# Leonhard111/M3L

Hardware: AMD Instinct MI355X
Metric: MAE fwd+bwd samples/sec (image+tactile) (higher is better)
Workload: dtype bf16; 1 GPU; BASELINE configs[1]: VTT vision+tactile MAE, 64x64 RGB + 2x32x32 tactile, ViT-Tiny 192/12/3/768 + decoder 192/4/3/768, mask 0.75; batch_per_gpu=256, global_batch=256, parallelism=dp1, grad_allreduce=none (one rank), rccl_ranks=0, step=zero_grad + mask + fwd + bwd + grad all-reduce + Adam

## Files before the change

### include/m3l_amd.h

```cpp
#ifndef M3L_AMD_H
#define M3L_AMD_H
#include <stddef.h>
#include <stdint.h>

#ifdef __cplusplus
extern "C" {
#endif

#define M3L_MAX_TACTILES 8

typedef struct m3l_geom {
    int image_h, image_w, image_patch, image_channels;
    int tactile_h, tactile_w, tactile_patch, tactile_channels;
    int num_tactiles;
    int use_vision;
    int use_tactile;
} m3l_geom;

typedef struct m3l_tf_cfg {
    int dim, depth, heads, mlp_dim;
    int project_out;
    int dtype;
    int dim_head;
} m3l_tf_cfg;

typedef struct m3l_dropout {
    float p;
    uint64_t seed;
} m3l_dropout;

int m3l_version(void);
int m3l_last_error(char* buf, size_t n);
int m3l_set_rowln(int enable);
int m3l_set_attn_block(int mode);
int m3l_set_enc_mega(int mode);
void m3l_set_attn_phase_buffer(void* dev_buf);
int m3l_set_defer_join(int on);
int m3l_set_wgrad_inline(int on);
int m3l_side_join(void* stream);
int m3l_comm_available(void);
int m3l_comm_unique_id(void* out128);
int m3l_comm_init(const void* id128, int rank, int world);
int m3l_comm_world(void);
int m3l_comm_allreduce(float* buf, size_t count, void* after_stream);
int m3l_comm_destroy(void);
int m3l_side_fork(void* after_stream, void** side_out);
int m3l_side_mark_pending(void);
void* m3l_side_stream(void);
int m3l_side_pending(void);
int m3l_set_drop_h(int on);
int m3l_set_t192(int on);
int m3l_set_t192_tt(int tt);
int m3l_set_residual_bf16(int on);
int m3l_set_t192_stagger(int lead_mask, int prio_mask);

int m3l_mask_counts(const m3l_geom* g, double ratio, int* counts_host);
int m3l_mask_sample(const m3l_geom* g, double ratio, int B, const float* const* noise, int64_t* masked, int64_t* unmasked,
                    void* stream);

int m3l_mask_sample_counts(const m3l_geom* g, int nm_img, int nm_tac, int B, const float* const* noise, int64_t* masked,
                           int64_t* unmasked, void* stream);

size_t m3l_embed_ws_bytes(const m3l_geom* g, int D, int dtype, int B, int L);
int m3l_embed_fwd(const m3l_geom* g, int D, int dtype, int B, int L, int cnt_img, const int64_t* idx, const float* image,
                  const float* const* tactiles, const void* const* tensors, void* ws, float* tokens, void* stream);
int m3l_embed_bwd(const m3l_geom* g, int D, int dtype, int B, int L, int cnt_img, const int64_t* idx, const float* image,
                  const float* const* tactiles, const void* const* tensors, void* ws, const float* dtokens, float* const* grads,
                  void* stream);

size_t m3l_transformer_ws_bytes(const m3l_tf_cfg* c, int B, int n);
int m3l_transformer_fwd(const m3l_tf_cfg* c, int B, int n, const float* x_in, const void* const* tensors, void* ws, void* y_t,
                        float* y32, void* stream);
int m3l_transformer_bwd(const m3l_tf_cfg* c, int B, int n, const float* x_in, const void* const* tensors, void* ws, const void* dy,
                        int dy_dtype, float* dx_in, float* const* grads, void* stream);

int m3l_transformer_bwd_range(const m3l_tf_cfg* c, int B, int n, const float* x_in, const void* const* tensors, void* ws,
                              const void* dy, int dy_dtype, float* dx_in, float* const* grads, int layer_hi, int layer_lo, void* stream);

size_t m3l_transformer_ws_bytes_dropout(const m3l_tf_cfg* c, int B, int n, const m3l_dropout* drop);
int m3l_transformer_fwd_dropout(const m3l_tf_cfg* c, int B, int n, const float* x_in, const void* const* tensors, void* ws, void* y_t,
                                float* y32, const m3l_dropout* drop, void* stream);
int m3l_transformer_bwd_dropout(const m3l_tf_cfg* c, int B, int n, const float* x_in, const void* const* tensors, void* ws, const void* dy,
                                int dy_dtype, float* dx_in, float* const* grads, const m3l_dropout* drop, void* stream);
int m3l_transformer_bwd_range_dropout(const m3l_tf_cfg* c, int B, int n, const float* x_in, const void* const* tensors, void* ws,
                                      const void* dy, int dy_dtype, float* dx_in, float* const* grads, int layer_hi, int layer_lo,
                                      const m3l_dropout* drop, void* stream);

size_t m3l_frozen_vit_ws_bytes(const m3l_tf_cfg* c, int B, int n);
int m3l_frozen_vit_fwd(const m3l_tf_cfg* c, float ln_eps, int B, int n, const float* x, const void* const* tensors, void* ws,
                       float* y32, void* stream);

size_t m3l_unshuffle_ws_bytes(const m3l_geom* g, int D, int dd, int dtype, int B, int nvis, int nmask);
int m3l_unshuffle_fwd(const m3l_geom* g, int D, int dd, int dtype, int B, int nvis, int nmask, const int64_t* unmasked,
                      const int64_t* masked, const float* enc32, const void* enc_t, const void* const* tensors, void* ws,
                      float* dec_in, void* stream);
int m3l_unshuffle_bwd(const m3l_geom* g, int D, int dd, int dtype, int B, int nvis, int nmask, const int64_t* unmasked,
                      const int64_t* masked, const void* enc_t, const void* const* tensors, void* ws, const float* d_dec_in,
                      void* d_enc, int* d_enc_dtype, float* const* grads, void* stream);

size_t m3l_heads_ws_bytes(const m3l_geom* g, int dd, int dtype, int B, int nmask);
int m3l_heads_loss_fwd(const m3l_geom* g, int dd, int dtype, int B, int N, int nmask, int nm_img, const int64_t* masked,
                       const float* image, const float* const* tactiles, const void* dec_t, const void* const* tensors, void* ws,
                       float* loss, float* pred_img, float* tgt_img, float* pred_tac, float* tgt_tac, void* stream);
// ... 137 lines not shown
```

### m3l_amd/_lib.py

```python
import ctypes as C
import os

_HERE = os.path.dirname(os.path.abspath(__file__))
LIB_PATH = os.environ.get("M3L_LIB_PATH") or os.path.join(_HERE, "lib", "libm3l_amd.so")

c_p = C.c_void_p
c_i = C.c_int
c_sz = C.c_size_t


class Geom(C.Structure):
    _fields_ = [(n, c_i) for n in ("image_h", "image_w", "image_patch", "image_channels", "tactile_h", "tactile_w",
                                   "tactile_patch", "tactile_channels", "num_tactiles", "use_vision", "use_tactile")]


class CnnCfg(C.Structure):
    _fields_ = [(n, c_i) for n in ("in_channels", "height", "width", "dim", "tactile", "dtype")]


class TfCfg(C.Structure):
    _fields_ = [(n, c_i) for n in ("dim", "depth", "heads", "mlp_dim", "project_out", "dtype", "dim_head")]


class MaeCfg(C.Structure):
    _fields_ = [("geom", Geom), ("enc", TfCfg), ("dec", TfCfg), ("masking_ratio", C.c_double), ("early_conv", c_i), ("learned_pos", c_i)]


class Dropout(C.Structure):
    _fields_ = [("p", C.c_float), ("seed", C.c_uint64)]


class CommPlan(C.Structure):
    _fields_ = [("flat", c_p), ("total", C.c_long), ("min_bucket", C.c_long), ("layers_per_chunk", c_i), ("n_stages", c_i),
                ("stage_end", C.POINTER(C.c_long)), ("sent_out", C.POINTER(C.c_long))]


_SIGS = {
    "m3l_version": (c_i, []),
    "m3l_last_error": (c_i, [C.c_char_p, c_sz]),
    "m3l_set_rowln": (c_i, [c_i]),
    "m3l_set_attn_block": (c_i, [c_i]),
    "m3l_set_attn_phase_buffer": (None, [c_p]),
    "m3l_set_enc_mega": (c_i, [c_i]),
    "m3l_set_drop_h": (c_i, [c_i]),
    "m3l_set_direct_conv": (c_i, [c_i]),
    "m3l_set_t192": (c_i, [c_i]),
    "m3l_set_t192_tt": (c_i, [c_i]),
    "m3l_set_t192_stagger": (c_i, [c_i, c_i]),
    "m3l_set_residual_bf16": (c_i, [c_i]),
    "m3l_set_defer_join": (c_i, [c_i]),
    "m3l_set_wgrad_inline": (c_i, [c_i]),
    "m3l_side_join": (c_i, [c_p]),
    "m3l_side_stream": (c_p, []),
    "m3l_side_fork": (c_i, [c_p, C.POINTER(c_p)]),
    "m3l_side_mark_pending": (c_i, []),
    "m3l_comm_available": (c_i, []),
    "m3l_comm_unique_id": (c_i, [c_p]),
    "m3l_comm_init": (c_i, [c_p, c_i, c_i]),
    "m3l_comm_world": (c_i, []),
    "m3l_comm_allreduce": (c_i, [c_p, c_sz, c_p]),
    "m3l_comm_destroy": (c_i, []),
    "m3l_side_pending": (c_i, []),
    "m3l_mask_counts": (c_i, [C.POINTER(Geom), C.c_double, C.POINTER(c_i)]),
    "m3l_mask_sample": (c_i, [C.POINTER(Geom), C.c_double, c_i, c_p, c_p, c_p, c_p]),
    "m3l_mask_sample_counts": (c_i, [C.POINTER(Geom), c_i, c_i, c_i, c_p, c_p, c_p, c_p]),
    "m3l_embed_ws_bytes": (c_sz, [C.POINTER(Geom), c_i, c_i, c_i, c_i]),
    "m3l_embed_fwd": (c_i, [C.POINTER(Geom), c_i, c_i, c_i, c_i, c_i, c_p, c_p, c_p, c_p, c_p, c_p, c_p]),
    "m3l_embed_bwd": (c_i, [C.POINTER(Geom), c_i, c_i, c_i, c_i, c_i, c_p, c_p, c_p, c_p, c_p, c_p, c_p, c_p]),
    "m3l_transformer_ws_bytes": (c_sz, [C.POINTER(TfCfg), c_i, c_i]),
    "m3l_transformer_fwd": (c_i, [C.POINTER(TfCfg), c_i, c_i, c_p, c_p, c_p, c_p, c_p, c_p]),
    "m3l_transformer_bwd": (c_i, [C.POINTER(TfCfg), c_i, c_i, c_p, c_p, c_p, c_p, c_i, c_p, c_p, c_p]),
    "m3l_transformer_bwd_range": (c_i, [C.POINTER(TfCfg), c_i, c_i, c_p, c_p, c_p, c_p, c_i, c_p, c_p, c_i, c_i, c_p]),
    "m3l_transformer_ws_bytes_dropout": (c_sz, [C.POINTER(TfCfg), c_i, c_i, C.POINTER(Dropout)]),
    "m3l_transformer_fwd_dropout": (c_i, [C.POINTER(TfCfg), c_i, c_i, c_p, c_p, c_p, c_p, c_p, C.POINTER(Dropout), c_p]),
    "m3l_transformer_bwd_dropout": (c_i, [C.POINTER(TfCfg), c_i, c_i, c_p, c_p, c_p, c_p, c_i, c_p, c_p, C.POINTER(Dropout), c_p]),
    "m3l_transformer_bwd_range_dropout": (c_i, [C.POINTER(TfCfg), c_i, c_i, c_p, c_p, c_p, c_p, c_i, c_p, c_p, c_i, c_i, C.POINTER(Dropout), c_p]),
    "m3l_frozen_vit_ws_bytes": (c_sz, [C.POINTER(TfCfg), c_i, c_i]),
    "m3l_frozen_vit_fwd": (c_i, [C.POINTER(TfCfg), C.c_float, c_i, c_i, c_p, c_p, c_p, c_p, c_p]),
    "m3l_unshuffle_ws_bytes": (c_sz, [C.POINTER(Geom), c_i, c_i, c_i, c_i, c_i, c_i]),
    "m3l_unshuffle_fwd": (c_i, [C.POINTER(Geom), c_i, c_i, c_i, c_i, c_i, c_i, c_p, c_p, c_p, c_p, c_p, c_p, c_p, c_p]),
    "m3l_unshuffle_bwd": (c_i, [C.POINTER(Geom), c_i, c_i, c_i, c_i, c_i, c_i, c_p, c_p, c_p, c_p, c_p, c_p, c_p,
                                C.POINTER(c_i), c_p, c_p]),
    "m3l_heads_ws_bytes": (c_sz, [C.POINTER(Geom), c_i, c_i, c_i, c_i]),
    "m3l_heads_loss_fwd": (c_i, [C.POINTER(Geom), c_i, c_i, c_i, c_i, c_i, c_i, c_p, c_p, c_p, c_p, c_p, c_p, c_p, c_p, c_p,
                                 c_p, c_p, c_p]),
    "m3l_heads_loss_fwd2": (c_i, [C.POINTER(Geom), c_i, c_i, c_i, c_i, c_i, c_i, c_p, c_p, c_p, c_p, c_p, c_p, c_p, c_p, c_p,
                                  c_p, c_p, c_p, c_p]),
    "m3l_heads_loss_bwd": (c_i, [C.POINTER(Geom), c_i, c_i, c_i, c_i, c_i, c_i, c_p, c_p, c_p, c_p, c_p, c_p, c_p]),
    "m3l_mae_step_num_tensors": (c_i, [C.POINTER(MaeCfg)]),
    "m3l_mae_step_ws_bytes": (c_sz, [C.POINTER(MaeCfg), c_i]),
    "m3l_mae_step_fwd": (c_i, [C.POINTER(MaeCfg), c_i, c_p, c_p, c_p, c_p, c_p, c_p, c_p, c_p, c_p]),
    "m3l_mae_step_bwd": (c_i, [C.POINTER(MaeCfg), c_i, c_p, c_p, c_p, c_p, c_p, c_p, c_p, c_p, C.POINTER(CommPlan), c_p]),
    "m3l_mae_step_ws_bytes_dropout": (c_sz, [C.POINTER(MaeCfg), c_i, C.POINTER(Dropout)]),
    "m3l_mae_step_fwd_dropout": (c_i, [C.POINTER(MaeCfg), c_i, c_p, c_p, c_p, c_p, c_p, c_p, c_p, c_p, C.POINTER(Dropout), c_p]),
    "m3l_mae_step_bwd_dropout": (c_i, [C.POINTER(MaeCfg), c_i, c_p, c_p, c_p, c_p, c_p, c_p, c_p, c_p, C.POINTER(CommPlan), C.POINTER(Dropout), c_p]),
    "m3l_extractor_num_tensors": (c_i, [C.POINTER(MaeCfg), C.POINTER(TfCfg)]),
    "m3l_extractor_ws_bytes": (c_sz, [C.POINTER(MaeCfg), C.POINTER(TfCfg), c_i]),
# ... 104 lines not shown
```

### m3l_amd/csrc/elementwise.hip

```cpp
#include "common.cuh"
#include "kernels.h"
#include <cstring>
#include <vector>

namespace {

constexpr int MAXV = 16;
constexpr int WPB = 4;

__device__ __forceinline__ void store_val(float* p, float v) { *p = v; }
__device__ __forceinline__ void store_val(bf16* p, float v) { *p = (bf16)v; }


template <typename TO> __device__ __forceinline__ void store4(TO* p, f32x4 v);
template <> __device__ __forceinline__ void store4<float>(float* p, f32x4 v) { *reinterpret_cast<f32x4*>(p) = v; }
template <> __device__ __forceinline__ void store4<bf16>(bf16* p, f32x4 v) {
    bf16x4 o;
    o[0] = (bf16)v[0]; o[1] = (bf16)v[1]; o[2] = (bf16)v[2]; o[3] = (bf16)v[3];
    *reinterpret_cast<bf16x4*>(p) = o;
}
__device__ __forceinline__ f32x4 load4(const float* p) { return *reinterpret_cast<const f32x4*>(p); }
__device__ __forceinline__ f32x4 load4(const bf16* p) {
    const bf16x4 v = *reinterpret_cast<const bf16x4*>(p);
    return f32x4{(float)v[0], (float)v[1], (float)v[2], (float)v[3]};
// ... 127 lines not shown
    float s = 0.f;
    if (valid) {
        float a[8] = {0.f, 0.f, 0.f, 0.f, 0.f, 0.f, 0.f, 0.f};
        int g = sl;
        for (; g + 224 < G; g += 256) {
#pragma unroll
            for (int u = 0; u < 8; ++u) a[u] += p[(long)(g + 32 * u) * stride + j];
        }
        for (; g < G; g += 32) a[0] += p[(long)g * stride + j];
        s = ((a[0] + a[1]) + (a[2] + a[3])) + ((a[4] + a[5]) + (a[6] + a[7]));
    }
    red[sl][cl] = s;
    __syncthreads();
    if (sl == 0 && valid) {
        float t = red[0][cl];
#pragma unroll
        for (int i = 1; i < 32; ++i) t += red[i][cl];
        out[j] = accumulate ? out[j] + t : t;
    }
}

__global__ __launch_bounds__(1024) void reduce_rows_kernel(const float* __restrict__ part, int G, int stride, int count,
                                                             float* __restrict__ out, int accumulate) {
    const int j = blockIdx.x * 32 + (threadIdx.x & 31);
    reduce_cols_32x32(part, G, stride, j, j < count, out, accumulate);
}

__global__ __launch_bounds__(1024) void reduce_vec_kernel(const float* __restrict__ v, int G, float* __restrict__ out, int accumulate) {
    __shared__ float red[16];
    float a0 = 0.f, a1 = 0.f, a2 = 0.f, a3 = 0.f;
    int i = threadIdx.x;
    for (; i + 3072 < G; i += 4096) { a0 += v[i]; a1 += v[i + 1024]; a2 += v[i + 2048]; a3 += v[i + 3072]; }
    for (; i < G; i += 1024) a0 += v[i];
    float s = wave_sum((a0 + a1) + (a2 + a3));
    if ((threadIdx.x & 63) == 0) red[threadIdx.x >> 6] = s;
    __syncthreads();
    if (threadIdx.x == 0) {
        float t = 0.f;
#pragma unroll
        for (int w = 0; w < 16; ++w) t += red[w];
        out[0] = accumulate ? out[0] + t : t;
    }
}

struct ReduceSegs { float* out[4]; };
__global__ __launch_bounds__(1024) void reduce_rows_seg_kernel(const float* __restrict__ part, int G, int stride, int width,
                                                                 ReduceSegs segs, int accumulate) {
    float* out = segs.out[blockIdx.y];
    if (!out) return;
    const int j = blockIdx.x * 32 + (threadIdx.x & 31);
    reduce_cols_32x32(part + (long)blockIdx.y * width, G, stride, j, j < width, out, accumulate);
}

__global__ __launch_bounds__(1024) void reduce_rows_batch_kernel(ReduceBatch b, int accumulate) {
    const ReduceBatchItem it = b.it[blockIdx.z];
    float* out = it.out[blockIdx.y];
    if (!out) return;
    const int j = blockIdx.x * 32 + (threadIdx.x & 31);
    reduce_cols_32x32(it.part + (long)blockIdx.y * b.D, it.G, 3 * b.D, j, j < b.D, out, accumulate);
}

template <typename T> struct Vec4;
template <> struct Vec4<bf16> { typedef bf16x4 type; };
template <> struct Vec4<float> { typedef f32x4 type; };
template <typename T>
__global__ __launch_bounds__(256) void colsum_kernel(const T* __restrict__ Y, int M, int N, int ld, int rows_per_block,
                                                       float* __restrict__ part, int vec_ok) {
    typedef typename Vec4<T>::type V4;
    const int r0 = blockIdx.x * rows_per_block, r1 = min(M, r0 + rows_per_block);
    for (int c = threadIdx.x * 4; c < N; c += 1024) {
        if (vec_ok && c + 4 <= N) {
            f32x4 s0 = f32x4{0.f, 0.f, 0.f, 0.f}, s1 = s0, s2 = s0, s3 = s0;
            auto ld4 = [&](int r) {
                const V4 v = *reinterpret_cast<const V4*>(Y + (long)r * ld + c);
                return f32x4{to_f32(v[0]), to_f32(v[1]), to_f32(v[2]), to_f32(v[3])};
            };
            int r = r0;
            for (; r + 3 < r1; r += 4) {
                s0 += ld4(r);
                s1 += ld4(r + 1);
                s2 += ld4(r + 2);
                s3 += ld4(r + 3);
            }
            for (; r < r1; ++r) s0 += ld4(r);
            *reinterpret_cast<f32x4*>(part + (long)blockIdx.x * N + c) = (s0 + s1) + (s2 + s3);
        } else {
            for (int cc = c; cc < min(N, c + 4); ++cc) {
                float s0 = 0.f, s1 = 0.f, s2 = 0.f, s3 = 0.f;
                int r = r0;
                for (; r + 3 < r1; r += 4) {
                    s0 += to_f32(Y[(long)r * ld + cc]);
                    s1 += to_f32(Y[(long)(r + 1) * ld + cc]);
                    s2 += to_f32(Y[(long)(r + 2) * ld + cc]);
                    s3 += to_f32(Y[(long)(r + 3) * ld + cc]);
                }
                for (; r < r1; ++r) s0 += to_f32(Y[(long)r * ld + cc]);
                part[(long)blockIdx.x * N + cc] = (s0 + s1) + (s2 + s3);
            }
        }
    }
}

template <typename T>
__global__ __launch_bounds__(256) void prep_weights_kernel(WeightPack pack) {
    __shared__ float tile[64][65];
    int m = 0;
    while (m + 1 < pack.count && (int)blockIdx.x >= pack.tile0[m + 1]) ++m;
    const WeightDesc d = pack.d[m];
    const int tcols = (d.cols + 63) >> 6;
    const int t = blockIdx.x - pack.tile0[m];
    const int r0 = (t / tcols) << 6, c0 = (t % tcols) << 6;
    const int tid = threadIdx.x, q = tid & 15, p = tid >> 4;
    T* dst = reinterpret_cast<T*>(d.dst);
    T* dstT = reinterpret_cast<T*>(d.dstT);
    const bool vec_in = (d.cols & 3) == 0 && (reinterpret_cast<uintptr_t>(d.src) & 15) == 0;
#pragma unroll
    for (int k = 0; k < 4; ++k) {
        const int r = r0 + p + 16 * k, c = c0 + 4 * q;
        float v[4] = {0.f, 0.f, 0.f, 0.f};
        if (r < d.rows) {
            if (vec_in && c + 3 < d.cols) {
                const float4 f = *reinterpret_cast<const float4*>(d.src + (long)r * d.cols + c);
                v[0] = f.x; v[1] = f.y; v[2] = f.z; v[3] = f.w;
            } else {
#pragma unroll
                for (int j = 0; j < 4; ++j)
                    if (c + j < d.cols) v[j] = d.src[(long)r * d.cols + c + j];
            }
        }
        if (dst && r < d.ld_dstT) {
#pragma unroll
            for (int j = 0; j < 4; ++j)
                if (c + j < d.ld_dst) dst[(long)r * d.ld_dst + c + j] = from_f32<T>(v[j]);
        }
#pragma unroll
        for (int j = 0; j < 4; ++j) tile[p + 16 * k][4 * q + j] = v[j];
    }
    if (!dstT) return;
    __syncthreads();
#pragma unroll
    for (int k = 0; k < 4; ++k) {
        const int c = c0 + p + 16 * k, r = r0 + 4 * q;
        if (c >= d.ld_dst) continue;
#pragma unroll
        for (int j = 0; j < 4; ++j)
            if (r + j < d.ld_dstT) dstT[(long)c * d.ld_dstT + r + j] = from_f32<T>(tile[4 * q + j][p + 16 * k]);
    }
}

template <typename T>
__global__ void axpy_t_kernel(const float* __restrict__ x, const T* __restrict__ o, long count, float* __restrict__ out) {
    const long i = (long)blockIdx.x * blockDim.x + threadIdx.x;
    if (i < count) out[i] = x[i] + to_f32(o[i]);
}
template <typename T>
__global__ void cast_kernel(const float* __restrict__ x, long count, T* __restrict__ out) {
    const long i = (long)blockIdx.x * blockDim.x + threadIdx.x;
    if (i < count) out[i] = from_f32<T>(x[i]);
}

template <typename T>
__global__ void scale_by_dev_kernel(const T* __restrict__ x, long count, const float* __restrict__ s, T* __restrict__ out) {
    const long i = (long)blockIdx.x * blockDim.x + threadIdx.x;
    if (i < count) out[i] = from_f32<T>(to_f32(x[i]) * s[0]);
}

template <int MODE>
__global__ void mask_scale_kernel(const float* __restrict__ src, const void* __restrict__ ref, float scale, long count, float* __restrict__ out) {
    const long i = (long)blockIdx.x * blockDim.x + threadIdx.x;
    if (i >= count) return;
    const bool on = MODE == 0 ? reinterpret_cast<const uint8_t*>(ref)[i] != 0 : reinterpret_cast<const float*>(ref)[i] > 0.f;
    out[i] = on ? src[i] * scale : 0.f;
}
__global__ void vit_tokens_kernel(const float* __restrict__ emb, const float* __restrict__ cls, const float* __restrict__ regs,
                                  const float* __restrict__ pos, int B, int npatch, int R, int D, float* __restrict__ tok) {
    const long i = (long)blockIdx.x * blockDim.x + threadIdx.x;
    const int n = 1 + R + npatch;
    if (i >= (long)B * n * D) return;
    const int d = (int)(i % D), t = (int)((i / D) % n), b = (int)(i / ((long)D * n));
    float v;
    if (t == 0) v = cls[d] + pos[d];
    else if (t <= R) v = regs[(long)(t - 1) * D + d];
    else v = emb[((long)b * npatch + (t - 1 - R)) * D + d] + pos[(long)(t - R) * D + d];
    tok[i] = v;
}
__global__ void concat2_kernel(const float* __restrict__ a, int na, const float* __restrict__ b2, int nb, int rows, float* __restrict__ dst, int split) {
    const long i = (long)blockIdx.x * blockDim.x + threadIdx.x;
    const int w = na + nb;
    if (i >= (long)rows * w) return;
    const int r = (int)(i / w), c = (int)(i % w);
    if (!split) dst[i] = c < na ? a[(long)r * na + c] : b2[(long)r * nb + c - na];
    else if (c < na) const_cast<float*>(a)[(long)r * na + c] = dst[i];
    else if (b2) const_cast<float*>(b2)[(long)r * nb + c - na] = dst[i];
}

template <typename T>
__global__ void im2col_kernel(ConvSrc cs, int Bsrc, int Ci, int H, int W, int KH, int S, int P, int OH, int OW, int Kpad,
                              long total, T* __restrict__ col) {
    const long idx = (long)blockIdx.x * blockDim.x + threadIdx.x;
    if (idx >= total) return;
    const int k = (int)(idx % Kpad);
    const long r = idx / Kpad;
    const int ow = (int)(r % OW), oh = (int)((r / OW) % OH);
    const int b = (int)(r / ((long)OW * OH));
    float v = 0.f;
    if (k < Ci * KH * KH) {
        const int kw = k % KH, kh = (k / KH) % KH, ci = k / (KH * KH);
        const int ih = oh * S + kh - P, iw = ow * S + kw - P;
        if (ih >= 0 && ih < H && iw >= 0 && iw < W) {
            if (cs.nchw) {
                const float* src = reinterpret_cast<const float*>(cs.src[b / Bsrc]);
                v = src[(((long)(b % Bsrc) * Ci + ci) * H + ih) * W + iw];
            } else {
                v = to_f32(reinterpret_cast<const T*>(cs.src[0])[(((long)b * H + ih) * W + iw) * Ci + ci]);
            }
        }
    }
// ... 245 lines not shown
    ph = pidx / gw;
    pw = pidx % gw;
}
__device__ __forceinline__ const float* patch_base(const PatchGroup& pg, int b, int s, int ph, int pw) {
    const float* src = pg.src[0];
#pragma unroll
    for (int i = 1; i < M3L_MAX_SENSORS; ++i) src = (s == i) ? pg.src[i] : src;
    return src + ((long)b * pg.C * pg.H + ph * pg.P) * pg.W + pw * pg.P;
}
struct PatchDiv {
    unsigned m_pp, m_p;
    int pp;
};
__device__ __forceinline__ PatchDiv patch_div(const PatchGroup& pg) {
    PatchDiv d;
    d.pp = pg.P * pg.P;
    d.m_pp = 0xFFFFFFFFu / (unsigned)d.pp + 1u;
    d.m_p = 0xFFFFFFFFu / (unsigned)pg.P + 1u;
    return d;
}
__device__ __forceinline__ int patch_off_t(const PatchGroup& pg, const PatchDiv& dv, int t, int& e) {
    const int c = (int)__umulhi((unsigned)t, dv.m_pp);
    const int rem = t - c * dv.pp;
    const int p1 = (int)__umulhi((unsigned)rem, dv.m_p);
    const int p2 = rem - p1 * pg.P;
    e = rem * pg.C + c;
    return (c * pg.H + p1) * pg.W + p2;
}
template <int NV>
__device__ __forceinline__ void patch_stage_stats(const PatchGroup& pg, const PatchDiv& dv, const float* __restrict__ base, int lane, int pd,
                                                  float eps, float* __restrict__ my, float& mean, float& rstd) {
    float v[NV];
    int ei[NV];
#pragma unroll
    for (int i = 0; i < NV; ++i) v[i] = base[patch_off_t(pg, dv, min(lane + 64 * i, pd - 1), ei[i])];
    float sum = 0.f;
#pragma unroll
    for (int i = 0; i < NV; ++i) {
        if (lane + 64 * i < pd) my[ei[i]] = v[i];
        else v[i] = 0.f;
        sum += v[i];
    }
    mean = wave_sum(sum) / pd;
    float q = 0.f;
#pragma unroll
    for (int i = 0; i < NV; ++i) {
        const float d = (lane + 64 * i < pd) ? v[i] - mean : 0.f;
        q += d * d;
    }
    rstd = rsqrtf(wave_sum(q) / pd + eps);
}

template <typename T, int NV>
__global__ __launch_bounds__(256) void patch_ln_kernel(PatchGroup pg, const int64_t* __restrict__ idx, int idx_ld, int j0, int cnt,
                                                         int rows, const float* __restrict__ gamma, const float* __restrict__ beta,
                                                         float eps, T* __restrict__ xn, int pdpad, int vec) {
    __shared__ __attribute__((aligned(16))) float buf[WPB][NV * 64];
    const int lane = threadIdx.x & 63, wave = threadIdx.x >> 6, row = blockIdx.x * WPB + wave;
    const int pd = pg.C * pg.P * pg.P;
    const PatchDiv dv = patch_div(pg);
    float* my = buf[wave];
    const bool live = row < rows;
    float mean = 0.f, rstd = 0.f;
    if (live) {
        int b, s, ph, pw, local;
        patch_locate(pg, idx, idx_ld, j0, cnt, row, b, s, ph, pw, local);
        patch_stage_stats<NV>(pg, dv, patch_base(pg, b, s, ph, pw), lane, pd, eps, my, mean, rstd);
    }
    __syncthreads();
    if (!live) return;
    T* out = xn + (long)row * pdpad;
    if (vec) {
        constexpr int NC = NV / 4;
        f32x4 gm[NC], bt[NC];
#pragma unroll
        for (int k = 0; k < NC; ++k) {
            const int ec = min(4 * (lane + 64 * k), pd - 4);
            gm[k] = load4(gamma + ec);
            bt[k] = load4(beta + ec);
        }
#pragma unroll
        for (int k = 0; k < NC; ++k) {
            const int e = 4 * (lane + 64 * k);
            if (e < pdpad) {
                f32x4 r = {0.f, 0.f, 0.f, 0.f};
                if (e < pd) r = (*reinterpret_cast<const f32x4*>(my + e) - mean) * rstd * gm[k] + bt[k];
                store4<T>(out + e, r);
            }
        }
    } else {
        for (int e = lane; e < pdpad; e += 64) out[e] = from_f32<T>(e < pd ? (my[e] - mean) * rstd * gamma[e] + beta[e] : 0.f);
    }
}

template <typename T, int NV>
__global__ __launch_bounds__(256) void patch_ln_bwd_kernel(PatchGroup pg, const int64_t* __restrict__ idx, int idx_ld, int j0, int cnt,
                                                             int rows, float eps, const T* __restrict__ dxn, int pdpad,
                                                             float* __restrict__ part, int vec) {
    __shared__ __attribute__((aligned(16))) float buf[WPB][NV * 64];
    constexpr int NC = NV / 4;
    static_assert(NV % 4 == 0, "4-element pieces");
    const int lane = threadIdx.x & 63, wave = threadIdx.x >> 6;
    const int pd = pg.C * pg.P * pg.P;
    const PatchDiv dv = patch_div(pg);
    float* my = buf[wave];
    f32x4 dg[NC], db[NC];
#pragma unroll
    for (int k = 0; k < NC; ++k) dg[k] = db[k] = f32x4{0.f, 0.f, 0.f, 0.f};
    for (int r0 = blockIdx.x * WPB; r0 < rows; r0 += gridDim.x * WPB) {
        const int row = r0 + wave;
        const bool live = row < rows;
        float mean = 0.f, rstd = 0.f;
        if (live) {
            int b, s, ph, pw, local;
            patch_locate(pg, idx, idx_ld, j0, cnt, row, b, s, ph, pw, local);
            patch_stage_stats<NV>(pg, dv, patch_base(pg, b, s, ph, pw), lane, pd, eps, my, mean, rstd);
        }
        __syncthreads();
        if (live) {
            const T* dr = dxn + (long)row * pdpad;
            f32x4 d[NC];
#pragma unroll
            for (int k = 0; k < NC; ++k) {
                const int e = 4 * (lane + 64 * k);
                if (vec) {
                    d[k] = load4(dr + min(e, pd - 4));
                } else {
#pragma unroll
                    for (int q = 0; q < 4; ++q) d[k][q] = to_f32(dr[min(e + q, pd - 1)]);
                }
            }
#pragma unroll
            for (int k = 0; k < NC; ++k) {
                const int e = 4 * (lane + 64 * k);
                f32x4 a = {0.f, 0.f, 0.f, 0.f};
                if (vec) {
                    if (e < pd) a = *reinterpret_cast<const f32x4*>(my + e);
                    else d[k] = f32x4{0.f, 0.f, 0.f, 0.f};
                } else {
#pragma unroll
                    for (int q = 0; q < 4; ++q) {
                        if (e + q < pd) a[q] = my[e + q];
                        else d[k][q] = 0.f;
                    }
                }
                dg[k] += d[k] * (a - mean) * rstd;
                db[k] += d[k];
            }
        }
        __syncthreads();
    }
    float* out = part + (long)blockIdx.x * 2 * pd;
#pragma unroll
    for (int pass = 0; pass < 2; ++pass) {
#pragma unroll
        for (int k = 0; k < NC; ++k) *reinterpret_cast<f32x4*>(my + 4 * (lane + 64 * k)) = pass ? db[k] : dg[k];
        __syncthreads();
        for (int e = threadIdx.x; e < pd; e += 256) out[pass * pd + e] = buf[0][e] + buf[1][e] + buf[2][e] + buf[3][e];
        __syncthreads();
    }
}

__global__ __launch_bounds__(256) void embed_finalize_kernel(const float* __restrict__ E, int rows, int D, PatchGroup pg,
                                                               const int64_t* __restrict__ idx, int idx_ld, int j0, int cnt,
                                                               const float* __restrict__ gamma, const float* __restrict__ beta,
                                                               float eps, const float* __restrict__ mod, int mod0,
                                                               const float* __restrict__ pos, float* __restrict__ tokens, int L) {
    const int lane = threadIdx.x & 63, row = blockIdx.x * WPB + (threadIdx.x >> 6);
    if (row >= rows) return;
    int b, s, ph, pw, local;
    patch_locate(pg, idx, idx_ld, j0, cnt, row, b, s, ph, pw, local);
    const float* xr = E + (long)row * D;
    float v[MAXV];
    float sum = 0.f;
#pragma unroll
    for (int i = 0; i < MAXV; ++i) {
        const int e = lane + 64 * i;
        v[i] = (e < D) ? xr[e] : 0.f;
        sum += v[i];
    }
    const float mean = wave_sum(sum) / D;
    float q = 0.f;
#pragma unroll
    for (int i = 0; i < MAXV; ++i) {
        const int e = lane + 64 * i;
        const float d = (e < D) ? v[i] - mean : 0.f;
        q += d * d;
    }
    const float rstd = rsqrtf(wave_sum(q) / D + eps);
    const int jj = row % cnt;
    float* out = tokens + ((long)b * L + j0 + jj) * D;
    const float* mrow = mod + (long)(mod0 + s) * D;
    const float* prow = pos + (long)local * D;
#pragma unroll
    for (int i = 0; i < MAXV; ++i) {
        const int e = lane + 64 * i;
        if (e < D) out[e] = (v[i] - mean) * rstd * gamma[e] + beta[e] + mrow[e] + prow[e];
    }
}

template <typename T>
__global__ __launch_bounds__(256) void embed_finalize_bwd_kernel(const float* __restrict__ dtok, int L, const float* __restrict__ E,
                                                                   int rows, int D, PatchGroup pg, const int64_t* __restrict__ idx,
                                                                   int idx_ld, int j0, int cnt, const float* __restrict__ gamma,
                                                                   float eps, T* __restrict__ dE, float* __restrict__ part, int nslot) {
    extern __shared__ float sm[];
    const int lane = threadIdx.x & 63, wave = threadIdx.x >> 6;
    const int PL = (2 + nslot) * D;
    for (int i = threadIdx.x; i < WPB * PL; i += 256) sm[i] = 0.f;
    __syncthreads();
    float* my = sm + wave * PL;
    for (int row = blockIdx.x * WPB + wave; row < rows; row += gridDim.x * WPB) {
        int b, s, ph, pw, local;
        patch_locate(pg, idx, idx_ld, j0, cnt, row, b, s, ph, pw, local);
        const int jj = row % cnt;
        const float* xr = E + (long)row * D;
        const float* dyr = dtok + ((long)b * L + j0 + jj) * D;
        float v[MAXV], gdy[MAXV];
        float sum = 0.f;
#pragma unroll
        for (int i = 0; i < MAXV; ++i) {
            const int e = lane + 64 * i;
            v[i] = (e < D) ? xr[e] : 0.f;
            sum += v[i];
        }
        const float mean = wave_sum(sum) / D;
        float q = 0.f;
#pragma unroll
        for (int i = 0; i < MAXV; ++i) {
            const int e = lane + 64 * i;
            const float d = (e < D) ? v[i] - mean : 0.f;
            q += d * d;
        }
        const float rstd = rsqrtf(wave_sum(q) / D + eps);
        float s1 = 0.f, s2 = 0.f;
#pragma unroll
        for (int i = 0; i < MAXV; ++i) {
            const int e = lane + 64 * i;
            if (e < D) {
                const float xh = (v[i] - mean) * rstd;
                const float d = dyr[e];
                my[e] += d * xh;
                my[D + e] += d;
                my[(2 + s) * D + e] += d;
                const float gd = d * gamma[e];
                gdy[i] = gd;
                v[i] = xh;
                s1 += gd;
                s2 += gd * xh;
            } else {
                gdy[i] = 0.f;
                v[i] = 0.f;
            }
        }
        s1 = wave_sum(s1) / D;
        s2 = wave_sum(s2) / D;
#pragma unroll
        for (int i = 0; i < MAXV; ++i) {
            const int e = lane + 64 * i;
            if (e < D) dE[(long)row * D + e] = from_f32<T>(rstd * (gdy[i] - s1 - v[i] * s2));
        }
    }
    __syncthreads();
    for (int i = threadIdx.x; i < PL; i += 256)
        part[(long)blockIdx.x * PL + i] = sm[i] + sm[PL + i] + sm[2 * PL + i] + sm[3 * PL + i];
}

template <typename TO>
__global__ __launch_bounds__(256) void unshuffle_fwd_kernel(const float* __restrict__ src, const float* __restrict__ mask_token,
                                                              const int64_t* __restrict__ unmasked, int nvis,
                                                              const int64_t* __restrict__ masked, int nmask, int B, int dd,
                                                              int n_img, int n_tac, const float* __restrict__ dmod,
                                                              const float* __restrict__ pos_img, const float* __restrict__ pos_tac,
                                                              TO* __restrict__ dec_in) {
    const int lane = threadIdx.x & 63;
    const long r = (long)blockIdx.x * WPB + (threadIdx.x >> 6);
    const int N = nvis + nmask;
    if (r >= (long)B * N) return;
    const int b = (int)(r / N), j = (int)(r % N);
    const bool vis = j < nvis;
    const int pos = (int)(vis ? unmasked[(long)b * nvis + j] : masked[(long)b * nmask + j - nvis]);
    const float* s = vis ? src + ((long)b * nvis + j) * dd : mask_token;
    const int m = pos < n_img ? 0 : 1 + (pos - n_img) / n_tac;
    const float* prow = pos < n_img ? pos_img + (long)pos * dd : pos_tac + (long)(pos - n_img) * dd;
    TO* out = dec_in + ((long)b * N + pos) * dd;
    const float* mrow = dmod + (long)m * dd;
    for (int e = 4 * lane; e < dd; e += 256) store4<TO>(out + e, load4(s + e) + load4(mrow + e) + load4(prow + e));
}

template <int MAXC, typename TI>
__global__ __launch_bounds__(256) void unshuffle_bwd_kernel(const TI* __restrict__ dY, const int64_t* __restrict__ unmasked, int nvis,
                                                              int B, int N, int dd, int n_img, int n_tac, int nmod, int rows_per_wave,
                                                              int vis_per_wave, float* __restrict__ dsrc, float* __restrict__ part) {
    extern __shared__ float sm[];
    const int lane = threadIdx.x & 63, wave = threadIdx.x >> 6;
    const int PL = (1 + nmod) * dd;
    for (int i = threadIdx.x; i < WPB * PL; i += 256) sm[i] = 0.f;
    __syncthreads();
    float* my = sm + wave * PL;
    const long gw = (long)blockIdx.x * WPB + wave;
    f32x4 acc[MAXC];
#pragma unroll
    for (int c = 0; c < MAXC; ++c) acc[c] = f32x4{0.f, 0.f, 0.f, 0.f};
#define UNSH_FLUSH(slot, sign)                                                      \
    _Pragma("unroll") for (int c = 0; c < MAXC; ++c) {                              \
        const int e4 = (lane + 64 * c) * 4;                                         \
        if (e4 < dd) {                                                              \
            _Pragma("unroll") for (int q = 0; q < 4; ++q) {                         \
                my[e4 + q] += (sign) * acc[c][q];                                   \
                if ((slot) >= 0) my[(1 + (slot)) * dd + e4 + q] += acc[c][q];       \
            }                                                                       \
        }                                                                           \
        acc[c] = f32x4{0.f, 0.f, 0.f, 0.f};                                         \
    }
    const long total = (long)B * N;
    const long r0 = gw * rows_per_wave, r1 = r0 + rows_per_wave < total ? r0 + rows_per_wave : total;
    for (long r = r0; r < r1;) {
        const int pos = (int)(r % N);
// ... 76 lines not shown
    const T* s = src + ((long)b * N + pos) * D;
    T* d = dst + (long)row * D;
    for (int e = lane; e < D; e += 64) d[e] = s[e];
}
template <typename T>
__global__ __launch_bounds__(256) void scatter_rows_kernel(const T* __restrict__ src, int N, int D, const int64_t* __restrict__ idx,
                                                             int idx_ld, int j0, int cnt, int rows, T* __restrict__ dst) {
    const int lane = threadIdx.x & 63, row = blockIdx.x * WPB + (threadIdx.x >> 6);
    if (row >= rows) return;
    const int b = row / cnt, jj = row % cnt;
    const long pos = idx[(long)b * idx_ld + j0 + jj];
    const T* s = src + (long)row * D;
    T* d = dst + ((long)b * N + pos) * D;
    for (int e = lane; e < D; e += 64) d[e] = s[e];
}

template <typename T>
__global__ __launch_bounds__(256) void gather_rows2_kernel(const T* __restrict__ src, int N, int D, const int64_t* __restrict__ idx, int idx_ld,
                                                             int cnt0, int cnt1, int rows, T* __restrict__ dst0, T* __restrict__ dst1) {
    const int lane = threadIdx.x & 63, row = blockIdx.x * WPB + (threadIdx.x >> 6);
    if (row >= rows) return;
    const int b = row / (cnt0 + cnt1), j = row % (cnt0 + cnt1);
    const long pos = idx[(long)b * idx_ld + j];
    const uint4* s = reinterpret_cast<const uint4*>(src + ((long)b * N + pos) * D);
    uint4* d = reinterpret_cast<uint4*>(j < cnt0 ? dst0 + ((long)b * cnt0 + j) * D : dst1 + ((long)b * cnt1 + (j - cnt0)) * D);
    const int pieces = D * (int)sizeof(T) / 16;
    for (int p = lane; p < pieces; p += 64) d[p] = s[p];
}
template <typename T>
__global__ __launch_bounds__(256) void scatter_rows2_kernel(const T* __restrict__ src0, const T* __restrict__ src1, int N, int D,
                                                              const int64_t* __restrict__ idx, int idx_ld, int cnt0, int cnt1, int rows,
                                                              const float* __restrict__ scale, T* __restrict__ dst) {
    const int lane = threadIdx.x & 63, row = blockIdx.x * WPB + (threadIdx.x >> 6);
    if (row >= rows) return;
    const int b = row / (cnt0 + cnt1), j = row % (cnt0 + cnt1);
    const long pos = idx[(long)b * idx_ld + j];
    const T* s = j < cnt0 ? src0 + ((long)b * cnt0 + j) * D : src1 + ((long)b * cnt1 + (j - cnt0)) * D;
    T* d = dst + ((long)b * N + pos) * D;
    const float sc = scale ? *scale : 1.f;
    constexpr int E = 16 / (int)sizeof(T);
    const int pieces = D / E;
    for (int p = lane; p < pieces; p += 64) {
        uint4 v = reinterpret_cast<const uint4*>(s)[p];
        if (scale) {
            T* e = reinterpret_cast<T*>(&v);
#pragma unroll
            for (int k = 0; k < E; ++k) e[k] = from_f32<T>(to_f32(e[k]) * sc);
        }
        reinterpret_cast<uint4*>(d)[p] = v;
    }
}

template <typename T>
__global__ __launch_bounds__(256) void mse_kernel(const float* __restrict__ pred, int pdpad, PatchGroup pg,
                                                    const int64_t* __restrict__ idx, int idx_ld, int j0, int cnt, int rows, float w,
                                                    float* __restrict__ part, T* __restrict__ dpred, float* __restrict__ target_out, int vec) {
    extern __shared__ __attribute__((aligned(16))) float mbuf[];
    __shared__ float red[WPB];
    const int lane = threadIdx.x & 63, wave = threadIdx.x >> 6;
    const int pd = pg.C * pg.P * pg.P;
    const PatchDiv dv = patch_div(pg);
    float* my = mbuf + (long)wave * pdpad;
    float acc = 0.f;
    for (int r0 = blockIdx.x * WPB; r0 < rows; r0 += gridDim.x * WPB) {
        const int row = r0 + wave;
        const bool live = row < rows;
        if (live) {
            int b, s, ph, pw, local;
            patch_locate(pg, idx, idx_ld, j0, cnt, row, b, s, ph, pw, local);
            const float* base = patch_base(pg, b, s, ph, pw);
            for (int tb = 0; tb < pd; tb += 512) {
                const int t0 = tb + lane;
                float tv[8];
                int e[8];
#pragma unroll
                for (int u = 0; u < 8; ++u) {
                    if (tb + 64 * u >= pd) break;
                    const int t = t0 + 64 * u;
                    tv[u] = base[patch_off_t(pg, dv, min(t, pd - 1), e[u])];
                }
#pragma unroll
                for (int u = 0; u < 8; ++u) {
                    if (tb + 64 * u >= pd) break;
                    if (t0 + 64 * u < pd) my[e[u]] = tv[u];
                }
            }
        }
        __syncthreads();
        if (live) {
            const float* pr = pred + (long)row * pdpad;
            T* dp = dpred + (long)row * pdpad;
            if (vec) {
#pragma unroll 4
                for (int e = 4 * lane; e < pdpad; e += 256) {
                    f32x4 d = {0.f, 0.f, 0.f, 0.f};
                    if (e < pd) {
                        const f32x4 t = *reinterpret_cast<const f32x4*>(my + e);
                        d = load4(pr + e) - t;
                        if (target_out) store4<float>(target_out + (long)row * pd + e, t);
                    }
                    acc += d[0] * d[0];
                    acc += d[1] * d[1];
                    acc += d[2] * d[2];
                    acc += d[3] * d[3];
                    store4<T>(dp + e, d * (2.f * w));
                }
            } else {
                for (int e = lane; e < pdpad; e += 64) {
                    const float d = e < pd ? pr[e] - my[e] : 0.f;
                    if (e < pd && target_out) target_out[(long)row * pd + e] = my[e];
                    acc += d * d;
                    dp[e] = from_f32<T>(2.f * w * d);
                }
            }
        }
        __syncthreads();
    }
    acc = wave_sum(acc);
    if (lane == 0) red[wave] = acc;
    __syncthreads();
    if (threadIdx.x == 0) part[blockIdx.x] = w * (red[0] + red[1] + red[2] + red[3]);
}

}

static int ln_grid(int M) { return cdiv(M, WPB); }
static bool aligned_to(const void* p, size_t a) { return ((uintptr_t)p & (a - 1)) == 0; }
int m3l_part_blocks(void) {
    static const int nb = [] {
        const char* e = getenv("M3L_PART_BLOCKS");
        const int v = e ? atoi(e) : 1024;
        return v < 64 ? 64 : (v > M3L_MAX_PARTIAL_BLOCKS ? M3L_MAX_PARTIAL_BLOCKS : v);
    }();
    return nb;
}
static int part_grid(long rows) {
    long g = (rows + WPB - 1) / WPB;
    if (g > m3l_part_blocks()) g = m3l_part_blocks();
    return (int)(g < 1 ? 1 : g);
}

int m3l_ln_fwd(int out_dtype, const float* x, int M, int D, const float* gamma, const float* beta, float eps, void* y, float* y32,
               hipStream_t st) {
    M3L_CHECK(M > 0 && D > 0 && D % 4 == 0 && D <= 1024, "ln_fwd: bad shape M=%d D=%d (D must be a multiple of 4, <= 1024)", M, D);
    ProfScope prof("ln_fwd", M, D, out_dtype, (double)M * D * (4.0 + (y ? (out_dtype ? 2 : 4) : 0) + (y32 ? 4 : 0)), st);
#define LN_FWD(TO, C, TX) ln_fwd_kernel<TO, C, TX><<<ln_grid(M), 256, 0, st>>>((const TX*)x, M, D, gamma, beta, eps, (TO*)y, y32)
    if (m3l_call_rb()) {
        if (out_dtype == 1) { if (D <= 256) LN_FWD(bf16, 1, bf16); else if (D <= 512) LN_FWD(bf16, 2, bf16); else LN_FWD(bf16, 4, bf16); }
        else { if (D <= 256) LN_FWD(float, 1, bf16); else if (D <= 512) LN_FWD(float, 2, bf16); else LN_FWD(float, 4, bf16); }
    } else if (out_dtype == 1) {
        if (D <= 256) LN_FWD(bf16, 1, float); else if (D <= 512) LN_FWD(bf16, 2, float); else LN_FWD(bf16, 4, float);
    } else {
        if (D <= 256) LN_FWD(float, 1, float); else if (D <= 512) LN_FWD(float, 2, float); else LN_FWD(float, 4, float);
    }
#undef LN_FWD
    M3L_LAUNCH_CHECK();
    return 0;
}

int m3l_reduce_rows(const float* part, int G, int stride, int count, float* out, int accumulate, hipStream_t st) {
    if (count == 1 && stride == 1)
        reduce_vec_kernel<<<1, 1024, 0, st>>>(part, G, out, accumulate);
    else
        reduce_rows_kernel<<<cdiv(count, 32), 1024, 0, st>>>(part, G, stride, count, out, accumulate);
    M3L_LAUNCH_CHECK();
    return 0;
}

int m3l_ln_bwd_blocks(int M) {
    static const int forced = getenv("M3L_LN_ROWS_PER_WAVE") ? atoi(getenv("M3L_LN_ROWS_PER_WAVE")) : 0;
    const int rpw = forced > 0 ? forced : (M >= 12288 ? 4 : std::max(1, M / 4096));
    int G = cdiv(M, rpw * WPB);
    if (G > 2048) G = 2048;
    return G < 1 ? 1 : G;
}

int m3l_ln_bwd(int dy_dtype, const void* dy, const float* x, int M, int D, const float* gamma, float eps, const float* dres,
               float* dx_out, void* dx_t_out, int ct_dtype, float* part_ws, float* dgamma, float* dbeta, float* dbias,
               int accumulate, hipStream_t st) {
    M3L_CHECK(M > 0 && D > 0 && D % 4 == 0 && D <= 1024, "ln_bwd: bad shape M=%d D=%d (D must be a multiple of 4, <= 1024)", M, D);
    const int G = m3l_ln_bwd_blocks(M);
    {
        ProfScope prof("ln_bwd", M, D, dy_dtype,
                       (double)M * D * ((m3l_call_rb() ? 2.0 : 4.0) + (dy_dtype ? 2 : 4) + (dres ? (m3l_call_rb() ? 2 : 4) : 0) + (dx_out ? 4 : 0) + (dx_t_out ? (ct_dtype ? 2 : 4) : 0)), st);
#define LN_BWD(TD, TC, C, TX) ln_bwd_kernel<TD, TC, C, TX><<<G, 256, 0, st>>>((const TD*)dy, (const TX*)x, M, D, gamma, eps, dres, dx_out, (TC*)dx_t_out, part_ws)
#define LN_BWD_C(TD, TC, TX) { if (D <= 256) LN_BWD(TD, TC, 1, TX); else if (D <= 512) LN_BWD(TD, TC, 2, TX); else LN_BWD(TD, TC, 4, TX); }
        if (m3l_call_rb()) {
            M3L_CHECK(!dx_out && dx_t_out && ct_dtype == 1, "ln_bwd: bf16 residual mode writes the compute-type gradient only");
            if (dy_dtype == 1) LN_BWD_C(bf16, bf16, bf16) else LN_BWD_C(float, bf16, bf16)
        }
        else if (dy_dtype == 1) LN_BWD_C(bf16, bf16, float)
        else if (ct_dtype == 1) LN_BWD_C(float, bf16, float)
        else LN_BWD_C(float, float, float)
#undef LN_BWD_C
#undef LN_BWD
    }
    M3L_LAUNCH_CHECK();
    if (!dgamma && !dbeta && !dbias) return 0;
    ReduceSegs segs = {{dgamma, dbeta, dbias, nullptr}};
    reduce_rows_seg_kernel<<<dim3(cdiv(D, 32), 3), 1024, 0, st>>>(part_ws, G, 3 * D, D, segs, accumulate);
    M3L_LAUNCH_CHECK();
    return 0;
}

int m3l_reduce_rows_batch(const ReduceBatch* b, int accumulate, hipStream_t st) {
    if (b->count <= 0) return 0;
    M3L_CHECK(b->count <= M3L_REDUCE_BATCH_MAX && b->D > 0, "reduce_rows_batch: count=%d D=%d", b->count, b->D);
    ProfScope prof("reduce_batch", b->count, b->D, 0, 0.0, st);
    reduce_rows_batch_kernel<<<dim3(cdiv(b->D, 32), 3, b->count), 1024, 0, st>>>(*b, accumulate);
    M3L_LAUNCH_CHECK();
    return 0;
}

int m3l_reduce_rows_seg3(const float* part, int G, int D, float* out0, float* out1, float* out2, int accumulate, hipStream_t st) {
    ReduceSegs segs = {{out0, out1, out2, nullptr}};
    reduce_rows_seg_kernel<<<dim3(cdiv(D, 32), 3), 1024, 0, st>>>(part, G, 3 * D, D, segs, accumulate);
    M3L_LAUNCH_CHECK();
    return 0;
}

int m3l_colsum(int dtype, const void* Y, int M, int N, int ld, float* part_ws, float* out, int accumulate, hipStream_t st) {
    M3L_CHECK(M > 0 && N > 0, "colsum: bad shape");
    int G = cdiv(M, N > 512 ? 16 : 64);
    if (G > m3l_part_blocks()) G = m3l_part_blocks();
    const int rpb = cdiv(M, G);
    G = cdiv(M, rpb);
    ProfScope prof("colsum", M, N, dtype, (double)M * N * (dtype ? 2 : 4), st);
    const int vec_ok = (ld % 4 == 0) && (N % 4 == 0) && (((unsigned long)Y) % 16 == 0) && (((unsigned long)part_ws) % 16 == 0);
    if (dtype == 1)
        colsum_kernel<bf16><<<G, 256, 0, st>>>((const bf16*)Y, M, N, ld, rpb, part_ws, vec_ok);
    else
        colsum_kernel<float><<<G, 256, 0, st>>>((const float*)Y, M, N, ld, rpb, part_ws, vec_ok);
    M3L_LAUNCH_CHECK();
    return m3l_reduce_rows(part_ws, G, N, N, out, accumulate, st);
}

static thread_local int g_prep_mode = 0;
static thread_local int g_prep_dtype = -1;
static thread_local std::vector<WeightDesc>* g_prep_list = nullptr;
int m3l_prep_mode(void) { return g_prep_mode; }
void m3l_prep_set_mode(int mode) {
    g_prep_mode = mode;
    if (mode == 1) {
        if (!g_prep_list) g_prep_list = new std::vector<WeightDesc>();
        g_prep_list->clear();
        g_prep_dtype = -1;
    }
}
int m3l_prep_flush(hipStream_t st) {
    const int saved = g_prep_mode;
    g_prep_mode = 0;
    int rc = 0;
    if (g_prep_list && !g_prep_list->empty()) {
        for (size_t i = 0; i < g_prep_list->size() && !rc; i += M3L_WPACK) {
            WeightPack pk;
            memset(&pk, 0, sizeof(pk));
            for (size_t k = i; k < g_prep_list->size() && k < i + M3L_WPACK; ++k) pk.d[pk.count++] = (*g_prep_list)[k];
            rc = m3l_prep_weights(g_prep_dtype, &pk, st);
        }
        g_prep_list->clear();
    }
    g_prep_mode = saved;
    return rc;
}

int m3l_prep_weights(int dtype, const WeightPack* pack_in, hipStream_t st) {
    if (pack_in->count <= 0) return 0;
    M3L_CHECK(pack_in->count <= M3L_WPACK, "prep_weights: %d matrices in one pack (max %d)", pack_in->count, M3L_WPACK);
    if (g_prep_mode == 2) return 0;
    if (g_prep_mode == 1) {
        M3L_CHECK(g_prep_dtype < 0 || g_prep_dtype == dtype, "prep_weights: modules of one chain disagree on the compute type");
        g_prep_dtype = dtype;
        for (int i = 0; i < pack_in->count; ++i) g_prep_list->push_back(pack_in->d[i]);
        return 0;
    }
    WeightPack pack = *pack_in;
    int tiles = 0;
    for (int i = 0; i < pack.count; ++i) {
        const WeightDesc& d = pack.d[i];
        M3L_CHECK(d.ld_dst >= d.cols && d.ld_dstT >= d.rows && d.ld_dst <= ((d.cols + 63) / 64) * 64 && d.ld_dstT <= ((d.rows + 63) / 64) * 64,
                  "prep_weights: padding of matrix %d ([%d, %d] -> [%d, %d]) must stay inside its last 64 x 64 tiles", i, d.rows, d.cols, d.ld_dstT, d.ld_dst);
        pack.tile0[i] = tiles;
        tiles += ((d.rows + 63) / 64) * ((d.cols + 63) / 64);
    }
    pack.tile0[pack.count] = tiles;
    if (tiles == 0) return 0;
    ProfScope prof("prep_weights", pack.count, dtype, 0, 0.0, st);
// ... 40 lines not shown
int m3l_cast_f32(int dtype, const float* x, long count, void* out, hipStream_t st) {
    ProfScope prof("cast", count, dtype, 0, (double)count * (4.0 + (dtype ? 2 : 4)), st);
    if (dtype == 1 && count % 8 == 0 && ((uintptr_t)x & 15) == 0 && ((uintptr_t)out & 15) == 0)
        cast8_f32_bf16_kernel<<<cdiv(count / 8, 256), 256, 0, st>>>(x, count / 8, (bf16*)out);
    else if (dtype == 1)
        cast_kernel<bf16><<<cdiv(count, 256), 256, 0, st>>>(x, count, (bf16*)out);
    else
        cast_kernel<float><<<cdiv(count, 256), 256, 0, st>>>(x, count, (float*)out);
    M3L_LAUNCH_CHECK();
    return 0;
}

int m3l_im2col(int dtype, const ConvSrc* src, int Bsrc, int Ci, int H, int W, int KH, int S, int P, int OH, int OW, int Kpad, void* col,
               hipStream_t st) {
    const int Btot = src->nchw ? Bsrc * src->nsrc : Bsrc;
    const long total = (long)Btot * OH * OW * Kpad;
    if (dtype == 1 && KH == 4 && Kpad == Ci * 16) {
        const long pairs = (long)Btot * OH * OW * Ci;
        im2col4_bf16_kernel<<<cdiv(pairs, 256), 256, 0, st>>>(*src, Bsrc, Ci, H, W, S, P, OH, OW, pairs, (bf16*)col);
        M3L_LAUNCH_CHECK();
        return 0;
    }
    if (dtype == 1)
        im2col_kernel<bf16><<<cdiv(total, 256), 256, 0, st>>>(*src, Bsrc, Ci, H, W, KH, S, P, OH, OW, Kpad, total, (bf16*)col);
    else
        im2col_kernel<float><<<cdiv(total, 256), 256, 0, st>>>(*src, Bsrc, Ci, H, W, KH, S, P, OH, OW, Kpad, total, (float*)col);
    M3L_LAUNCH_CHECK();
    return 0;
}

int m3l_col2im_relu(int dtype, const void* dcol, int Btot, int Ci, int H, int W, int KH, int S, int P, int OH, int OW, int Kpad,
                    const void* act, void* dX, hipStream_t st) {
    const long total = (long)Btot * H * W * Ci;
    if (dtype == 1)
        col2im_relu_kernel<bf16><<<cdiv(total, 256), 256, 0, st>>>((const bf16*)dcol, Btot, Ci, H, W, KH, S, P, OH, OW, Kpad, (const bf16*)act, (bf16*)dX);
    else
        col2im_relu_kernel<float><<<cdiv(total, 256), 256, 0, st>>>((const float*)dcol, Btot, Ci, H, W, KH, S, P, OH, OW, Kpad, (const float*)act, (float*)dX);
    M3L_LAUNCH_CHECK();
    return 0;
}

int k_tokens_assemble(const float* img_tok, const float* tac_tok, int B, int D, int n_img, int n_tac, int k, const float* mod,
                        const float* pos_img, const float* pos_tac, float* tokens, hipStream_t st) {
    const long rows = (long)B * (n_img + k * n_tac);
    tokens_assemble_kernel<<<cdiv(rows, WPB), 256, 0, st>>>(img_tok, tac_tok, B, D, n_img, n_tac > 0 ? n_tac : 1, k, mod, pos_img, pos_tac, tokens);
    M3L_LAUNCH_CHECK();
    return 0;
}

int k_tokens_assemble_bwd(const float* dtok, int B, int D, int n_img, int n_tac, int k, float* d_img, float* d_tac, float* part_ws,
                            float* dmod, int accumulate, hipStream_t st) {
    const long rows = (long)B * (n_img + k * n_tac);
    const int PL = (1 + k) * D;
    const int G = part_grid(rows);
    tokens_assemble_bwd_kernel<<<G, 256, WPB * PL * sizeof(float), st>>>(dtok, B, D, n_img, n_tac > 0 ? n_tac : 1, k, d_img, d_tac, part_ws);
    M3L_LAUNCH_CHECK();
    reduce_rows_kernel<<<cdiv(PL, 32), 1024, 0, st>>>(part_ws, G, PL, PL, dmod, accumulate);
    M3L_LAUNCH_CHECK();
    return 0;
}

int m3l_adam_flat(float* p, const float* g, float* m, float* v, long n, float lr, float b1, float b2, float eps, float wd, int step,
                  float gscale, hipStream_t st) {
    M3L_CHECK(n > 0 && step >= 1, "adam: n=%ld step=%d", n, step);
    const float bc1 = 1.0f - powf(b1, (float)step);
    const float bc2_sqrt = sqrtf(1.0f - powf(b2, (float)step));
    adam_flat_kernel<0><<<cdiv(cdiv(n, 4), 256), 256, 0, st>>>(p, const_cast<float*>(g), m, v, n, lr, b1, b2, eps, wd, bc1, bc2_sqrt, nullptr, gscale, nullptr, 0);
    M3L_LAUNCH_CHECK();
    return 0;
}

int m3l_adamw_flat(float* p, float* g, float* m, float* v, long n, float lr, float b1, float b2, float eps, float wd, int step, float gscale,
                   float max_norm, float* norm_ws, int scale_grads, hipStream_t st) {
    M3L_CHECK(n > 0 && step >= 1, "adamw: n=%ld step=%d", n, step);
    M3L_CHECK(max_norm <= 0.f || norm_ws, "adamw: clipping needs the norm workspace");
    const float bc1 = 1.0f - powf(b1, (float)step);
    const float bc2_sqrt = sqrtf(1.0f - powf(b2, (float)step));
    const float* clip = nullptr;
    if (max_norm > 0.f) {
        const int G = (int)std::min<long>(1024, cdiv(cdiv(n, 4), 256));
        gradnorm_part_kernel<<<G, 256, 0, st>>>(g, n, norm_ws);
        M3L_LAUNCH_CHECK();
        gradnorm_final_kernel<<<1, 64, 0, st>>>(norm_ws, G, gscale, max_norm, norm_ws + 1024);
        M3L_LAUNCH_CHECK();
        clip = norm_ws + 1024;
    }
    const float decay = (float)(1.0 - (double)lr * (double)wd);
    adam_flat_kernel<1><<<cdiv(cdiv(n, 4), 256), 256, 0, st>>>(p, g, m, v, n, lr, b1, b2, eps, decay, bc1, bc2_sqrt, nullptr, gscale, clip,
                                                              scale_grads && (clip || gscale != 1.0f));
    M3L_LAUNCH_CHECK();
    return 0;
}

int m3l_adam_flat_dev(float* p, const float* g, float* m, float* v, long n, float lr, float b1, float b2, float eps, float wd,
                      int* step_dev, float* bc_dev, hipStream_t st) {
    M3L_CHECK(n > 0 && step_dev && bc_dev, "adam (device step): n=%ld", n);
    adam_bias_kernel<<<1, 1, 0, st>>>(step_dev, b1, b2, bc_dev);
    M3L_LAUNCH_CHECK();
    adam_flat_kernel<0><<<cdiv(cdiv(n, 4), 256), 256, 0, st>>>(p, const_cast<float*>(g), m, v, n, lr, b1, b2, eps, wd, 1.0f, 1.0f, bc_dev, 1.0f, nullptr, 0);
    M3L_LAUNCH_CHECK();
    return 0;
}

int m3l_scale_by_dev(int dtype, const void* x, long count, const float* scale_dev, void* out, hipStream_t st) {
    if (dtype == 1)
        scale_by_dev_kernel<bf16><<<cdiv(count, 256), 256, 0, st>>>((const bf16*)x, count, scale_dev, (bf16*)out);
    else
        scale_by_dev_kernel<float><<<cdiv(count, 256), 256, 0, st>>>((const float*)x, count, scale_dev, (float*)out);
    M3L_LAUNCH_CHECK();
    return 0;
}

int m3l_mask_scale(int mode, const float* src, const void* ref, float scale, long count, float* out, hipStream_t st) {
    M3L_CHECK((mode == 0 || mode == 1) && count > 0 && src && ref && out, "mask_scale: bad arguments");
    if (mode == 0) mask_scale_kernel<0><<<cdiv(count, 256), 256, 0, st>>>(src, ref, scale, count, out);
    else mask_scale_kernel<1><<<cdiv(count, 256), 256, 0, st>>>(src, ref, scale, count, out);
    M3L_LAUNCH_CHECK();
    return 0;
}
int m3l_vit_tokens(const float* emb, const float* cls, const float* regs, const float* pos, int B, int npatch, int R, int D, float* tok,
                   hipStream_t st) {
    M3L_CHECK(B > 0 && npatch > 0 && R >= 0 && D > 0 && emb && cls && pos && tok && (R == 0 || regs), "vit_tokens: bad arguments");
    vit_tokens_kernel<<<cdiv((long)B * (1 + R + npatch) * D, 256), 256, 0, st>>>(emb, cls, regs, pos, B, npatch, R, D, tok);
    M3L_LAUNCH_CHECK();
    return 0;
}
int m3l_concat2(float* a, int na, float* b2, int nb, int rows, float* cat, int split, hipStream_t st) {
    M3L_CHECK(rows > 0 && na > 0 && nb > 0 && a && cat && (split || b2), "concat2: bad arguments");
    concat2_kernel<<<cdiv((long)rows * (na + nb), 256), 256, 0, st>>>(a, na, b2, nb, rows, cat, split);
    M3L_LAUNCH_CHECK();
    return 0;
}

int m3l_vt_load_launch(const void* image_nhwc, int image_u8, int B, int H, int W, int C, float img_lo, float img_span, float* image_nchw,
                       const void* tactile, int tactile_u8, int th, int tw, int n_sensors, int frame_stack, float tac_lo, float tac_span,
                       float* const* tactile_out, hipStream_t st) {
    if (image_nhwc) {
        M3L_CHECK(img_span != 0.f, "vt_load: empty image normalisation range");
        const long total = (long)B * C * H * W;
        if (image_u8)
            vt_image_kernel<uint8_t><<<cdiv(total, 256), 256, 0, st>>>((const uint8_t*)image_nhwc, B, H, W, C, img_lo, img_span, image_nchw);
        else
            vt_image_kernel<float><<<cdiv(total, 256), 256, 0, st>>>((const float*)image_nhwc, B, H, W, C, img_lo, img_span, image_nchw);
        M3L_LAUNCH_CHECK();
    }
    if (tactile) {
        M3L_CHECK(n_sensors >= 1 && n_sensors <= M3L_MAX_SENSORS, "vt_load: n_sensors=%d", n_sensors);
        M3L_CHECK(tac_span != 0.f, "vt_load: empty tactile normalisation range");
        VtTactileOut o;
        for (int s = 0; s < n_sensors; ++s) o.p[s] = tactile_out[s];
        const long total = (long)B * 3 * n_sensors * frame_stack * th * tw;
        if (tactile_u8)
            vt_tactile_kernel<uint8_t><<<cdiv(total, 256), 256, 0, st>>>((const uint8_t*)tactile, B, th, tw, n_sensors, frame_stack, tac_lo,
                                                                         tac_span, o);
        else
            vt_tactile_kernel<float><<<cdiv(total, 256), 256, 0, st>>>((const float*)tactile, B, th, tw, n_sensors, frame_stack, tac_lo,
                                                                       tac_span, o);
        M3L_LAUNCH_CHECK();
    }
    return 0;
}

int m3l_mask_rank_groups(const MaskRankArgs* args, int B, int64_t* masked, int masked_ld, int64_t* unmasked, int unmasked_ld, hipStream_t st) {
    M3L_CHECK(B > 0 && args->count >= 1 && args->count <= M3L_MAX_SENSORS + 1, "mask_rank: B=%d groups=%d", B, args->count);
    int nmax = 0;
    for (int i = 0; i < args->count; ++i) {
        const MaskRankGroup& g = args->g[i];
        M3L_CHECK(g.n > 0 && g.nm >= 0 && g.nm <= g.n, "mask_rank: bad shape n=%d nm=%d", g.n, g.nm);
        M3L_CHECK(g.n <= 8192, "mask_rank: n=%d too large", g.n);
        nmax = std::max(nmax, g.n);
    }
    const int threads = nmax <= 64 ? 64 : (nmax <= 128 ? 128 : 256);
    mask_rank_kernel<<<dim3(B, args->count), threads, nmax * sizeof(float), st>>>(*args, masked, masked_ld, unmasked, unmasked_ld);
    M3L_LAUNCH_CHECK();
    return 0;
}
int m3l_mask_rank(const float* noise, int B, int n, int nm, int token_offset, int64_t* masked, int masked_ld, int masked_off,
                  int64_t* unmasked, int unmasked_ld, int unmasked_off, hipStream_t st) {
    MaskRankArgs a;
    memset(&a, 0, sizeof(a));
    a.count = 1;
    a.g[0] = MaskRankGroup{noise, n, nm, token_offset, masked_off, unmasked_off};
    return m3l_mask_rank_groups(&a, B, masked, masked_ld, unmasked, unmasked_ld, st);
}

constexpr int PATCH_NV_MAX = 40;
static int check_pg(const PatchGroup& pg) {
    const int pd = pg.C * pg.P * pg.P;
    M3L_CHECK(pg.nsrc >= 1 && pg.nsrc <= M3L_MAX_SENSORS, "patch group: nsrc=%d", pg.nsrc);
    M3L_CHECK(pd <= 64 * PATCH_NV_MAX, "patch dim %d > %d unsupported", pd, 64 * PATCH_NV_MAX);
    M3L_CHECK(pg.H % pg.P == 0 && pg.W % pg.P == 0, "image dims must be divisible by the patch size");
    return 0;
}

int m3l_patch_ln(int dtype, const PatchGroup* pg, const int64_t* idx, int idx_ld, int j0, int cnt, int B, const float* gamma,
                 const float* beta, float eps, void* xn, int pdpad, hipStream_t st) {
    if (check_pg(*pg)) return 1;
    const int rows = B * cnt;
    if (rows == 0) return 0;
    const int pd_ = pg->C * pg->P * pg->P, esz = dtype == 1 ? 2 : 4;
    const bool wide = pd_ > 64 * MAXV, tiny = pd_ <= 256;
    const int vec = pd_ % 4 == 0 && pdpad % 4 == 0 && aligned_to(gamma, 16) && aligned_to(beta, 16) && aligned_to(xn, 4 * esz);
#define PATCH_LN(T, NV) patch_ln_kernel<T, NV><<<ln_grid(rows), 256, 0, st>>>(*pg, idx, idx_ld, j0, cnt, rows, gamma, beta, eps, (T*)xn, pdpad, vec)
    if (dtype == 1) {
        if (wide) PATCH_LN(bf16, PATCH_NV_MAX); else if (tiny) PATCH_LN(bf16, 4); else PATCH_LN(bf16, MAXV);
    } else {
        if (wide) PATCH_LN(float, PATCH_NV_MAX); else if (tiny) PATCH_LN(float, 4); else PATCH_LN(float, MAXV);
    }
#undef PATCH_LN
    M3L_LAUNCH_CHECK();
    return 0;
}

int m3l_patch_ln_bwd(int dtype, const PatchGroup* pg, const int64_t* idx, int idx_ld, int j0, int cnt, int B, float eps,
                     const void* dxn, int pdpad, float* part_ws, float* dgamma, float* dbeta, int accumulate, hipStream_t st) {
    if (check_pg(*pg)) return 1;
    const int rows = B * cnt;
    if (rows == 0) return 0;
    const int pd = pg->C * pg->P * pg->P;
    const int G = part_grid(rows);
    const bool wide = pd > 64 * MAXV, tiny = pd <= 256;
    const int vec = pd % 4 == 0 && pdpad % 4 == 0 && aligned_to(dxn, 4 * (dtype == 1 ? 2 : 4));
#define PATCH_LN_BWD(T, NV) patch_ln_bwd_kernel<T, NV><<<G, 256, 0, st>>>(*pg, idx, idx_ld, j0, cnt, rows, eps, (const T*)dxn, pdpad, part_ws, vec)
    if (dtype == 1) {
        if (wide) PATCH_LN_BWD(bf16, PATCH_NV_MAX); else if (tiny) PATCH_LN_BWD(bf16, 4); else PATCH_LN_BWD(bf16, MAXV);
    } else {
        if (wide) PATCH_LN_BWD(float, PATCH_NV_MAX); else if (tiny) PATCH_LN_BWD(float, 4); else PATCH_LN_BWD(float, MAXV);
    }
#undef PATCH_LN_BWD
    M3L_LAUNCH_CHECK();
    ReduceSegs segs = {{dgamma, dbeta, nullptr, nullptr}};
    reduce_rows_seg_kernel<<<dim3(cdiv(pd, 32), 2), 1024, 0, st>>>(part_ws, G, 2 * pd, pd, segs, accumulate);
    M3L_LAUNCH_CHECK();
    return 0;
}

int m3l_embed_finalize(const float* E, int D, const PatchGroup* pg, const int64_t* idx, int idx_ld, int j0, int cnt, int B,
                       const float* gamma, const float* beta, float eps, const float* mod, int mod0, const float* pos,
                       float* tokens, int L, hipStream_t st) {
    const int rows = B * cnt;
    if (rows == 0) return 0;
    M3L_CHECK(D <= 64 * MAXV, "embed_finalize: D=%d too large", D);
    embed_finalize_kernel<<<ln_grid(rows), 256, 0, st>>>(E, rows, D, *pg, idx, idx_ld, j0, cnt, gamma, beta, eps, mod, mod0, pos, tokens, L);
    M3L_LAUNCH_CHECK();
    return 0;
}

int m3l_embed_finalize_bwd(int dtype, const float* dtok, int L, const float* E, int D, const PatchGroup* pg, const int64_t* idx,
                           int idx_ld, int j0, int cnt, int B, const float* gamma, float eps, void* dE, float* part_ws,
                           float* dgamma, float* dbeta, float* dmod, int mod0, int accumulate, hipStream_t st) {
    const int rows = B * cnt;
    if (rows == 0) return 0;
    const int nslot = pg->nsrc;
    const int PL = (2 + nslot) * D;
    const int G = part_grid(rows);
    if (dtype == 1)
        embed_finalize_bwd_kernel<bf16><<<G, 256, WPB * PL * sizeof(float), st>>>(dtok, L, E, rows, D, *pg, idx, idx_ld, j0, cnt, gamma, eps, (bf16*)dE, part_ws, nslot);
    else
        embed_finalize_bwd_kernel<float><<<G, 256, WPB * PL * sizeof(float), st>>>(dtok, L, E, rows, D, *pg, idx, idx_ld, j0, cnt, gamma, eps, (float*)dE, part_ws, nslot);
    M3L_LAUNCH_CHECK();
    if (nslot <= 2) {
        float* dm = dmod + (long)mod0 * D;
        ReduceSegs segs = {{dgamma, dbeta, dm, nslot > 1 ? dm + D : nullptr}};
        reduce_rows_seg_kernel<<<dim3(cdiv(D, 32), 2 + nslot), 1024, 0, st>>>(part_ws, G, PL, D, segs, accumulate);
    } else {
        reduce_rows_kernel<<<cdiv(D, 32), 1024, 0, st>>>(part_ws, G, PL, D, dgamma, accumulate);
        reduce_rows_kernel<<<cdiv(D, 32), 1024, 0, st>>>(part_ws + D, G, PL, D, dbeta, accumulate);
        reduce_rows_kernel<<<cdiv(nslot * D, 32), 1024, 0, st>>>(part_ws + 2 * D, G, PL, nslot * D, dmod + (long)mod0 * D, accumulate);
    }
    M3L_LAUNCH_CHECK();
    return 0;
}

int k_unshuffle_fwd(const float* src, const float* mask_token, const int64_t* unmasked, int nvis, const int64_t* masked,
                      int nmask, int B, int dd, int n_img, int n_tac, const float* dmod, const float* pos_img, const float* pos_tac,
                      float* dec_in, hipStream_t st) {
    const long rows = (long)B * (nvis + nmask);
    M3L_CHECK(dd % 4 == 0, "unshuffle_fwd: dd=%d must be a multiple of 4", dd);
    if (m3l_call_io())
        unshuffle_fwd_kernel<bf16><<<cdiv(rows, WPB), 256, 0, st>>>(src, mask_token, unmasked, nvis, masked, nmask, B, dd, n_img, n_tac > 0 ? n_tac : 1, dmod,
                                                                     pos_img, pos_tac, reinterpret_cast<bf16*>(dec_in));
    else
        unshuffle_fwd_kernel<float><<<cdiv(rows, WPB), 256, 0, st>>>(src, mask_token, unmasked, nvis, masked, nmask, B, dd, n_img, n_tac > 0 ? n_tac : 1, dmod,
                                                                      pos_img, pos_tac, dec_in);
    M3L_LAUNCH_CHECK();
    return 0;
}

int k_unshuffle_bwd(const float* dY, const int64_t* unmasked, int nvis, const int64_t* masked, int nmask, int B, int dd, int n_img,
                      int n_tac, int nmod, float* dsrc, float* part_ws, float* dmask_token, float* ddmod, int accumulate,
                      hipStream_t st) {
    const long rows = (long)B * (nvis + nmask);
    const int PL = (1 + nmod) * dd;
    M3L_CHECK(dd % 4 == 0 && dd <= 1024, "unshuffle_bwd: dd=%d must be a multiple of 4, <= 1024", dd);
    (void)masked;
    int rpw = 16;
    while (cdiv(cdiv(rows, rpw), WPB) > m3l_part_blocks()) rpw *= 2;
    const int G = cdiv(cdiv(rows, rpw), WPB);
    const int vpw = cdiv((long)B * nvis, (long)G * WPB);
    const int N = nvis + nmask, nt = n_tac > 0 ? n_tac : 1;
    const size_t lds = WPB * PL * sizeof(float);
#define UNSH_BWD(C, TI) unshuffle_bwd_kernel<C, TI><<<G, 256, lds, st>>>((const TI*)dY, unmasked, nvis, B, N, dd, n_img, nt, nmod, rpw, vpw, dsrc, part_ws)
    if (m3l_call_io()) {
        if (dd <= 256) UNSH_BWD(1, bf16); else if (dd <= 512) UNSH_BWD(2, bf16); else UNSH_BWD(4, bf16);
    } else {
        if (dd <= 256) UNSH_BWD(1, float); else if (dd <= 512) UNSH_BWD(2, float); else UNSH_BWD(4, float);
    }
#undef UNSH_BWD
    M3L_LAUNCH_CHECK();
    if (nmod <= 3) {
        ReduceSegs segs = {{dmask_token, ddmod, nmod > 1 ? ddmod + dd : nullptr, nmod > 2 ? ddmod + 2 * dd : nullptr}};
        reduce_rows_seg_kernel<<<dim3(cdiv(dd, 32), 1 + nmod), 1024, 0, st>>>(part_ws, G, PL, dd, segs, accumulate);
    } else {
        reduce_rows_kernel<<<cdiv(dd, 32), 1024, 0, st>>>(part_ws, G, PL, dd, dmask_token, accumulate);
        reduce_rows_kernel<<<cdiv(nmod * dd, 32), 1024, 0, st>>>(part_ws + dd, G, PL, nmod * dd, ddmod, accumulate);
    }
    M3L_LAUNCH_CHECK();
    return 0;
}

int m3l_gather_rows(int dtype, const void* src, int N, int D, const int64_t* idx, int idx_ld, int j0, int cnt, int B, void* dst,
                    hipStream_t st) {
    const int rows = B * cnt;
    if (rows == 0) return 0;
    if (dtype == 1)
        gather_rows_kernel<bf16><<<ln_grid(rows), 256, 0, st>>>((const bf16*)src, N, D, idx, idx_ld, j0, cnt, rows, (bf16*)dst);
    else
        gather_rows_kernel<float><<<ln_grid(rows), 256, 0, st>>>((const float*)src, N, D, idx, idx_ld, j0, cnt, rows, (float*)dst);
    M3L_LAUNCH_CHECK();
    return 0;
}

int m3l_gather_rows2(int dtype, const void* src, int N, int D, const int64_t* idx, int idx_ld, int cnt0, int cnt1, int B, void* dst0, void* dst1,
                     hipStream_t st) {
    const int rows = B * (cnt0 + cnt1);
    if (rows == 0) return 0;
    M3L_CHECK((D * (dtype ? 2 : 4)) % 16 == 0, "gather_rows2: rows of %d elements are not 16-byte pieces", D);
    if (dtype == 1)
        gather_rows2_kernel<bf16><<<ln_grid(rows), 256, 0, st>>>((const bf16*)src, N, D, idx, idx_ld, cnt0, cnt1, rows, (bf16*)dst0, (bf16*)dst1);
    else
        gather_rows2_kernel<float><<<ln_grid(rows), 256, 0, st>>>((const float*)src, N, D, idx, idx_ld, cnt0, cnt1, rows, (float*)dst0, (float*)dst1);
    M3L_LAUNCH_CHECK();
    return 0;
}
int m3l_scatter_rows2(int dtype, const void* src0, const void* src1, int N, int D, const int64_t* idx, int idx_ld, int cnt0, int cnt1, int B,
                      const float* scale_dev, void* dst, hipStream_t st) {
    const int rows = B * (cnt0 + cnt1);
    if (rows == 0) return 0;
    M3L_CHECK((D * (dtype ? 2 : 4)) % 16 == 0, "scatter_rows2: rows of %d elements are not 16-byte pieces", D);
    if (dtype == 1)
        scatter_rows2_kernel<bf16><<<ln_grid(rows), 256, 0, st>>>((const bf16*)src0, (const bf16*)src1, N, D, idx, idx_ld, cnt0, cnt1, rows, scale_dev,
                                                                  (bf16*)dst);
    else
        scatter_rows2_kernel<float><<<ln_grid(rows), 256, 0, st>>>((const float*)src0, (const float*)src1, N, D, idx, idx_ld, cnt0, cnt1, rows,
                                                                   scale_dev, (float*)dst);
    M3L_LAUNCH_CHECK();
    return 0;
}

int m3l_scatter_rows(int dtype, const void* src, int N, int D, const int64_t* idx, int idx_ld, int j0, int cnt, int B, void* dst,
                     hipStream_t st) {
    const int rows = B * cnt;
    if (rows == 0) return 0;
    if (dtype == 1)
        scatter_rows_kernel<bf16><<<ln_grid(rows), 256, 0, st>>>((const bf16*)src, N, D, idx, idx_ld, j0, cnt, rows, (bf16*)dst);
    else
        scatter_rows_kernel<float><<<ln_grid(rows), 256, 0, st>>>((const float*)src, N, D, idx, idx_ld, j0, cnt, rows, (float*)dst);
    M3L_LAUNCH_CHECK();
    return 0;
}

int m3l_mse(int dtype, const float* pred, int pdpad, const PatchGroup* pg, const int64_t* idx, int idx_ld, int j0, int cnt, int B,
            float weight, float* part_ws, int* nblocks_out, void* dpred, float* target_out, hipStream_t st) {
    if (check_pg(*pg)) return 1;
    const int rows = B * cnt;
    if (nblocks_out) *nblocks_out = 0;
    if (rows == 0) return 0;
    const int pd = pg->C * pg->P * pg->P;
    const float w = weight / ((float)rows * (float)pd);
    const int G = part_grid(rows);
    M3L_CHECK(pdpad >= pd, "mse: pdpad %d < patch dim %d", pdpad, pd);
    const int vec = pd % 4 == 0 && pdpad % 4 == 0 && aligned_to(pred, 16) && aligned_to(dpred, 4 * (dtype == 1 ? 2 : 4)) &&
                    (!target_out || aligned_to(target_out, 16));
    const size_t lds = (size_t)WPB * pdpad * sizeof(float);
    M3L_CHECK(lds <= 64 * 1024, "mse: padded patch dim %d too wide", pdpad);
    if (dtype == 1)
        mse_kernel<bf16><<<G, 256, lds, st>>>(pred, pdpad, *pg, idx, idx_ld, j0, cnt, rows, w, part_ws, (bf16*)dpred, target_out, vec);
    else
        mse_kernel<float><<<G, 256, lds, st>>>(pred, pdpad, *pg, idx, idx_ld, j0, cnt, rows, w, part_ws, (float*)dpred, target_out, vec);
    M3L_LAUNCH_CHECK();
    if (nblocks_out) *nblocks_out = G;
    return 0;
}

DropCtx m3l_drop_ctx(float p, uint64_t seed, int layer, int site) {
    DropCtx d;
    memset(&d, 0, sizeof(d));
    d.on = p > 0.f ? 1 : 0;
    const double pd = p;
    const double t = floor(pd * 4294967296.0);
    d.thr = t >= 4294967295.0 ? 0xFFFFFFFFu : (uint32_t)t;
    d.scale = pd >= 1.0 ? 0.f : (float)(1.0 / (1.0 - pd));
    d.k0 = (uint32_t)seed;
    d.k1 = (uint32_t)(seed >> 32);
    d.ctr2 = (uint32_t)(4 * layer + site);
    return d;
}

namespace {
template <typename T>
__global__ __launch_bounds__(256) void dropout_bwd_kernel(const T* __restrict__ dy, T* __restrict__ out, float* __restrict__ part, int M, int N,
                                                           int rpb, DropCtx dr) {
    __shared__ float red[1024];
    const int NQ = N >> 2, RY = blockDim.y, tx = threadIdx.x, ty = threadIdx.y;
    const int r0 = blockIdx.x * rpb, r1 = min(M, r0 + rpb);
    float cs[4] = {0.f, 0.f, 0.f, 0.f};
    for (int r = r0 + ty; r < r1; r += RY) {
        const long o = (long)r * N + 4 * tx;
        const uint4 wd = drop_words(dr.k0, dr.k1, dr.ctr2, (uint64_t)r * NQ + tx);
        const uint32_t w[4] = {wd.x, wd.y, wd.z, wd.w};
#pragma unroll
        for (int j = 0; j < 4; ++j) {
            const T v = from_f32<T>(to_f32(dy[o + j]) * (w[j] >= dr.thr ? dr.scale : 0.f));
            out[o + j] = v;
            cs[j] += to_f32(v);
        }
    }
#pragma unroll
    for (int j = 0; j < 4; ++j) red[ty * N + 4 * tx + j] = cs[j];
    __syncthreads();
    if (ty == 0) {
#pragma unroll
        for (int j = 0; j < 4; ++j) {
            float s = 0.f;
            for (int y = 0; y < RY; ++y) s += red[y * N + 4 * tx + j];
            part[(long)blockIdx.x * N + 4 * tx + j] = s;
        }
    }
}

__global__ void dropout_mask_kernel(DropCtx dr, long rows, int N, uint8_t* __restrict__ out) {
    const int NQ = (N + 3) >> 2;
    const long i = (long)blockIdx.x * blockDim.x + threadIdx.x;
    if (i >= rows * NQ) return;
// ... 35 lines not shown
```

### m3l_amd/csrc/gemm.hip

```cpp
#include <stdlib.h>
#include <string.h>

#include <algorithm>

#include "common.cuh"
#include "kernels.h"

namespace {

constexpr int BM = 128, BN = 128;

template <typename T> struct NtCfg;
template <> struct NtCfg<bf16> { static constexpr int BK = 64, KSTEPS = 2, ROW = 72; };
template <> struct NtCfg<float> { static constexpr int BK = 32, KSTEPS = 1, ROW = 36; };

constexpr int NT_STAGE_BYTES = 128 * 144;
constexpr int NT_LDS_BYTES = 4 * NT_STAGE_BYTES;
constexpr int CS_LD = 132;

template <typename T>
__global__ __launch_bounds__(256) void gemm_nt_kernel(const T* __restrict__ A, int lda, const T* __restrict__ W, int ldw,
                                                        int M, int N, int K, GemmEpi epi) {
    extern __shared__ __attribute__((aligned(16))) char smem[];
    using C = NtCfg<T>;
// ... 78 lines not shown
    const T* gelu_u = reinterpret_cast<const T*>(epi.gelu_u);
#pragma unroll
    for (int i = 0; i < 8; ++i) {
        const int rl = r0 + 16 * i, row = m0 + rl;
        if (row >= M) continue;
        float v[8];
        const f32x4 p0 = *reinterpret_cast<const f32x4*>(Cs + rl * CS_LD + cchunk * 8);
        const f32x4 p1 = *reinterpret_cast<const f32x4*>(Cs + rl * CS_LD + cchunk * 8 + 4);
        v[0] = p0[0]; v[1] = p0[1]; v[2] = p0[2]; v[3] = p0[3];
        v[4] = p1[0]; v[5] = p1[1]; v[6] = p1[2]; v[7] = p1[3];
        const long o = (long)row * epi.ldc + col;
#pragma unroll
        for (int j = 0; j < 8; ++j) v[j] = v[j] * epi.alpha + bias[j];
        if (gelu_u) {
#pragma unroll
            for (int j = 0; j < 8; ++j) v[j] *= gelu_grad_t<T>(to_f32(gelu_u[o + j]));
        }
        if (out_pre) {
#pragma unroll
            for (int j = 0; j < 8; ++j) {
                const T u = from_f32<T>(v[j]);
                out_pre[o + j] = u;
                v[j] = to_f32(u);
            }
        }
        if (epi.act == 1) {
#pragma unroll
            for (int j = 0; j < 8; ++j) v[j] = gelu_t<T>(v[j]);
        } else if (epi.act == 2) {
#pragma unroll
            for (int j = 0; j < 8; ++j) v[j] = fmaxf(v[j], 0.f);
        }
        if (epi.relu_ref) {
            const T* rr = reinterpret_cast<const T*>(epi.relu_ref);
#pragma unroll
            for (int j = 0; j < 8; ++j) v[j] = to_f32(rr[o + j]) > 0.f ? v[j] : 0.f;
        }
        if (epi.res) {
#pragma unroll
            for (int j = 0; j < 8; ++j) v[j] += epi.res[o + j];
        }
        if (epi.out_f32) {
            *reinterpret_cast<f32x4*>(epi.out_f32 + o) = f32x4{v[0], v[1], v[2], v[3]};
            *reinterpret_cast<f32x4*>(epi.out_f32 + o + 4) = f32x4{v[4], v[5], v[6], v[7]};
        }
        if (out_t) {
#pragma unroll
            for (int j = 0; j < 8; ++j) out_t[o + j] = from_f32<T>(v[j]);
        }
    }
}

enum { EPI_GENERIC = 0, EPI_FC1 = 1, EPI_DGELU = 2, EPI_PLAIN = 3, EPI_RES32 = 4, EPI_RES16 = 5, EPI_DROP = 6 };
template <typename T, int BN, int R, int BM = 128, int EPI = 0>
__global__ __launch_bounds__(256) void gemm_nt_glds_kernel(const T* __restrict__ A, int lda, const T* __restrict__ W, int ldw,
                                                             int M, int N, int K, GemmEpi epi) {
    extern __shared__ __attribute__((aligned(16))) char smem[];
    constexpr int EPC = Chunk<T>::N;
    constexpr int BKE = 8 * EPC;
    constexpr int KSTEPS = BKE / 32;
    constexpr int A_BYTES = BM * 128, B_BYTES = BN * 128, STAGE = A_BYTES + B_BYTES;
    constexpr int WM = (BN == 128) ? BM / 2 : BM / 4;
    constexpr int ASEG = BM / 32;
    constexpr int TM = WM / 16;
    constexpr int CSLD = BN + 4;
    typedef __attribute__((address_space(3))) void* lds_vp;
    typedef __attribute__((address_space(1))) const void* gl_vp;

    const int tid = threadIdx.x, lane = tid & 63, wave = __builtin_amdgcn_readfirstlane(tid >> 6);
    const int g = lane >> 4, li = lane & 15;
    const int wr = (BN == 128) ? (wave >> 1) : wave, wc = (BN == 128) ? (wave & 1) : 0;
    const int gx = (N + BN - 1) / BN, gy = (M + BM - 1) / BM;
    const int bid = blockIdx.x, rest = bid >> 3;
    const int bx = rest % gx, by = (rest / gx) * 8 + (bid & 7);
    if (by >= gy) return;
    const int m0 = by * BM, n0 = bx * BN;

    const int srow = lane >> 3, spc = lane & 7;
    const T* asrc[ASEG];
#pragma unroll
    for (int i = 0; i < ASEG; ++i) {
        const int row = (wave * ASEG + i) * 8 + srow;
        asrc[i] = A + (long)min(m0 + row, M - 1) * lda + (spc ^ (row & 7)) * EPC;
    }
    constexpr int BSEG = BN / 32;
    const T* bsrc[BSEG];
#pragma unroll
    for (int i = 0; i < BSEG; ++i) {
        const int row = (wave * BSEG + i) * 8 + srow;
        bsrc[i] = W + (long)min(n0 + row, N - 1) * ldw + (spc ^ (row & 7)) * EPC;
    }
    auto stage = [&](int st, int k0) {
        char* base = smem + st * STAGE;
#pragma unroll
        for (int i = 0; i < ASEG; ++i)
            __builtin_amdgcn_global_load_lds((gl_vp)(asrc[i] + k0), (lds_vp)(base + (wave * ASEG + i) * 1024), 16, 0, 0);
#pragma unroll
        for (int i = 0; i < BSEG; ++i)
            __builtin_amdgcn_global_load_lds((gl_vp)(bsrc[i] + k0), (lds_vp)(base + A_BYTES + (wave * BSEG + i) * 1024), 16, 0, 0);
    };
    auto frag = [&](const char* base, int row, int ks) {
        Frag<T> f;
        if constexpr (sizeof(T) == 2) {
            f.v = *reinterpret_cast<const bf16x8*>(base + row * 128 + (((ks * 4 + g) ^ (row & 7)) << 4));
        } else {
            const f32x4 a = *reinterpret_cast<const f32x4*>(base + row * 128 + (((2 * g) ^ (row & 7)) << 4));
            const f32x4 b = *reinterpret_cast<const f32x4*>(base + row * 128 + (((2 * g + 1) ^ (row & 7)) << 4));
            f.v[0] = a[0]; f.v[1] = a[1]; f.v[2] = a[2]; f.v[3] = a[3];
            f.v[4] = b[0]; f.v[5] = b[1]; f.v[6] = b[2]; f.v[7] = b[3];
        }
        return f;
    };

    f32x4 acc[TM][4];
#pragma unroll
    for (int a = 0; a < TM; ++a)
#pragma unroll
        for (int b = 0; b < 4; ++b) acc[a][b] = f32x4{0.f, 0.f, 0.f, 0.f};

    constexpr int DMA_PER_STAGE = ASEG + BSEG;
    static_assert(R != 3 || DMA_PER_STAGE == 6 || DMA_PER_STAGE == 8, "counted vmcnt immediates exist for 6 / 8 DMA per stage");
    const int nk = K / BKE;
    if (R != 1) stage(0, 0);
    if (R == 3 && nk > 1) stage(1, BKE);
    if (R == 2) __syncthreads();
    for (int t = 0; t < nk; ++t) {
// ... 142 lines not shown
                const T* rr = reinterpret_cast<const T*>(epi.relu_ref);
#pragma unroll
                for (int j = 0; j < 8; ++j) v[j] = to_f32(rr[o + j]) > 0.f ? v[j] : 0.f;
            }
            if constexpr (EPI == EPI_DROP) {
                const uint64_t qb = (uint64_t)row * (uint64_t)(N >> 2) + (col >> 2);
                const uint4 w0 = drop_words(epi.drop.k0, epi.drop.k1, epi.drop.ctr2, qb);
                const uint4 w1 = drop_words(epi.drop.k0, epi.drop.k1, epi.drop.ctr2, qb + 1);
                const uint32_t wd[8] = {w0.x, w0.y, w0.z, w0.w, w1.x, w1.y, w1.z, w1.w};
#pragma unroll
                for (int j = 0; j < 8; ++j) v[j] *= wd[j] >= epi.drop.thr ? epi.drop.scale : 0.f;
            }
            if (f_res) {
                const f32x4 q0 = rq0[i], q1 = rq1[i];
                v[0] += q0[0]; v[1] += q0[1]; v[2] += q0[2]; v[3] += q0[3];
                v[4] += q1[0]; v[5] += q1[1]; v[6] += q1[2]; v[7] += q1[3];
            }
            if (f_res16) {
#pragma unroll
                for (int j = 0; j < 8; ++j) v[j] += to_f32(ruu[i].v[j]);
            }
            if (f_out32) {
                *reinterpret_cast<f32x4*>(epi.out_f32 + o) = f32x4{v[0], v[1], v[2], v[3]};
                *reinterpret_cast<f32x4*>(epi.out_f32 + o + 4) = f32x4{v[4], v[5], v[6], v[7]};
            }
            if (f_out_t) {
                Frag<T> pk;
#pragma unroll
                for (int j = 0; j < 8; ++j) {
                    pk.v[j] = from_f32<T>(v[j]);
                    csum[j] += to_f32(pk.v[j]);
                }
                if constexpr (sizeof(T) == 2) {
                    *reinterpret_cast<bf16x8*>(out_t + o) = pk.v;
                } else {
#pragma unroll
                    for (int j = 0; j < 8; ++j) out_t[o + j] = pk.v[j];
                }
            }
        }
    }
    if (f_colsum) {
        float* red = reinterpret_cast<float*>(smem) + BM * CSLD;
#pragma unroll
        for (int j = 0; j < 8; ++j) red[r0 * BN + cchunk * 8 + j] = csum[j];
        __syncthreads();
        if (tid < BN && n0 + tid < N) {
            float s = 0.f;
            for (int r = 0; r < RSTEP; ++r) s += red[r * BN + tid];
            epi.colsum_part[(long)by * N + n0 + tid] = s;
        }
    }
}

template <typename T> struct TnSwz;
template <> struct TnSwz<bf16> {
    static constexpr int ROWB = 256, CPR = 16, RPI = 4, BMT = 64;
    static __device__ __forceinline__ int swz(int row) { return 2 * (row & 7); }
};
template <> struct TnSwz<float> {
    static constexpr int ROWB = 512, CPR = 32, RPI = 2, BMT = 32;
    static __device__ __forceinline__ int swz(int row) { return 4 * ((row >> 2) & 1); }
};
__device__ __forceinline__ Frag<bf16> load_ks_swz(const char* tile, int k0, int c0, int lane, bf16) {
    const int g = lane >> 4, i = lane & 15, q = i >> 2, p = i & 3;
    const int r0 = k0 + 4 * g + q;
    const int chunk = (c0 >> 3) + (p >> 1);
    const int x = ((chunk ^ (2 * (r0 & 7))) << 4) + (p & 1) * 8;
    typedef __attribute__((address_space(3))) bf16x4* lds_p;
    const bf16x4 lo = __builtin_amdgcn_ds_read_tr16_b64_v4bf16((lds_p)(tile + r0 * 256 + x));
    const bf16x4 hi = __builtin_amdgcn_ds_read_tr16_b64_v4bf16((lds_p)(tile + (r0 + 16) * 256 + x));
    Frag<bf16> f;
    f.v[0] = lo[0]; f.v[1] = lo[1]; f.v[2] = lo[2]; f.v[3] = lo[3];
    f.v[4] = hi[0]; f.v[5] = hi[1]; f.v[6] = hi[2]; f.v[7] = hi[3];
    return f;
}
__device__ __forceinline__ Frag<float> load_ks_swz(const char* tile, int k0, int c0, int lane, float) {
    const int g = lane >> 4, i = lane & 15;
    const int col = c0 + i, chunk = col >> 2, off = (col & 3) * 4;
    Frag<float> f;
#pragma unroll
    for (int j = 0; j < 8; ++j) {
        const int r = k0 + 4 * g + (j & 3) + 16 * (j >> 2);
        f.v[j] = *reinterpret_cast<const float*>(tile + r * 512 + ((chunk ^ (4 * ((r >> 2) & 1))) << 4) + off);
    }
    return f;
}

template <typename T>
__global__ __launch_bounds__(256) void gemm_tn_glds_kernel(TnGroup grp, int M, int m_per_split, int nsplit,
                                                             float* __restrict__ partial_base) {
    extern __shared__ __attribute__((aligned(16))) char smem[];
    using S = TnSwz<T>;
    constexpr int ES = (int)sizeof(T), EPC = Chunk<T>::N;
    constexpr int TILE_B = S::BMT * S::ROWB;
    constexpr int STAGE = 2 * TILE_B;
    constexpr int MS = S::BMT / 32;
    typedef __attribute__((address_space(3))) void* lds_vp;
    const int tid = threadIdx.x, lane = tid & 63, wave = __builtin_amdgcn_readfirstlane(tid >> 6);
    const int wr = wave >> 1, wc = wave & 1, g = lane >> 4, li = lane & 15;
    const int bid = blockIdx.x, rest = bid >> 3;
    const int gtile = rest % grp.tiles_total, sp = (rest / grp.tiles_total) * 8 + (bid & 7);
    if (sp >= nsplit) return;
    int pi = 0;
#pragma unroll
    for (int i = 1; i < 4; ++i)
// ... 81 lines not shown
    for (int i = 0; i < S; ++i) s += partial[(long)i * N * K + idx];
    float* o = out + (long)n * ldo + k;
    *o = accumulate ? (*o + s) : s;
}

__global__ void reduce_splits_grouped_kernel(TnGroup grp, const float* __restrict__ partial_base, int S, int accumulate) {
    const long idx = (long)blockIdx.x * blockDim.x + threadIdx.x;
    if ((int)blockIdx.y == grp.count) {
        if (idx >= grp.extra_width) return;
        float s0 = 0.f, s1 = 0.f;
        int g = 0;
        for (; g + 1 < grp.extra_G; g += 2) {
            s0 += grp.extra_part[(long)g * grp.extra_width + idx];
            s1 += grp.extra_part[(long)(g + 1) * grp.extra_width + idx];
        }
        if (g < grp.extra_G) s0 += grp.extra_part[(long)g * grp.extra_width + idx];
        grp.extra_out[idx] = accumulate ? grp.extra_out[idx] + (s0 + s1) : (s0 + s1);
        return;
    }
    const TnProblem& pb = grp.p[blockIdx.y];
    const long cnt = (long)pb.N * pb.K;
    if (idx >= cnt) return;
    const int n = (int)(idx / pb.K), k = (int)(idx % pb.K);
    if (k >= pb.kvalid || n >= pb.nvalid) return;
    const float* P = partial_base + pb.part_off + idx;
    float s0 = 0.f, s1 = 0.f;
    int i = 0;
    for (; i + 1 < S; i += 2) {
        s0 += P[(long)i * cnt];
        s1 += P[(long)(i + 1) * cnt];
    }
    if (i < S) s0 += P[(long)i * cnt];
    float* o = pb.out + (long)n * pb.ldo + k;
    *o = accumulate ? (*o + (s0 + s1)) : (s0 + s1);
}

}

static constexpr int glds_lds_bytes(int bn, int r = 2, int bm = 128) {
    const int stages = r * (bm * 128 + bn * 128), cs = bm * (bn + 4) * 4 + (256 / (bn / 8)) * bn * 4;
    return stages > cs ? stages : cs;
}
static int nt_tile_rows(int M, int N) { return ((long)cdiv(M, 128) * cdiv(N, 64) < 1024) ? 64 : 128; }
static int g_gemm_inited = 0;
int m3l_gemm_init() {
    if (g_gemm_inited) return 0;
    M3L_HIP(hipFuncSetAttribute((const void*)gemm_nt_kernel<bf16>, hipFuncAttributeMaxDynamicSharedMemorySize, NT_LDS_BYTES));
    M3L_HIP(hipFuncSetAttribute((const void*)gemm_nt_kernel<float>, hipFuncAttributeMaxDynamicSharedMemorySize, NT_LDS_BYTES));
#define NT_ATTR(T, BMv, E) M3L_HIP(hipFuncSetAttribute((const void*)gemm_nt_glds_kernel<T, 64, 2, BMv, E>, hipFuncAttributeMaxDynamicSharedMemorySize, glds_lds_bytes(64, 2, BMv)))
#define NT_ATTR5(T, BMv) NT_ATTR(T, BMv, 0); NT_ATTR(T, BMv, 1); NT_ATTR(T, BMv, 2); NT_ATTR(T, BMv, 3); NT_ATTR(T, BMv, 4); NT_ATTR(T, BMv, 5); NT_ATTR(T, BMv, 6)
    NT_ATTR5(bf16, 128); NT_ATTR5(float, 128); NT_ATTR5(bf16, 64); NT_ATTR5(float, 64);
#undef NT_ATTR5
#undef NT_ATTR
    M3L_HIP(hipFuncSetAttribute((const void*)gemm_tn_glds_kernel<float>, hipFuncAttributeMaxDynamicSharedMemorySize, 65536));
    g_gemm_inited = 1;
    return 0;
}

int m3l_gemm_nt(int dtype, const void* A, int lda, const void* W, int ldw, int M, int N, int K, const GemmEpi* epi_in,
                hipStream_t st) {
    if (m3l_gemm_init()) return 2;
    GemmEpi e = *epi_in;
    if (e.n_bias <= 0) e.n_bias = N;
    const GemmEpi* epi = &e;
    M3L_CHECK(dtype == 0 || dtype == 1, "gemm_nt: bad dtype %d", dtype);
    M3L_CHECK(M > 0 && N > 0 && K > 0, "gemm_nt: empty problem %d %d %d", M, N, K);
    M3L_CHECK(K % 8 == 0 && N % 8 == 0 && lda % 8 == 0 && ldw % 8 == 0 && epi->ldc % 8 == 0,
              "gemm_nt: K,N,lda,ldw,ldc must be multiples of 8 (got K=%d N=%d lda=%d ldw=%d ldc=%d)", K, N, lda, ldw, epi->ldc);
    const int bke = dtype == 1 ? 64 : 32;
    M3L_CHECK(!epi->res_t || (dtype == 1 && K % bke == 0 && epi->out_t && !epi->res && !epi->gelu_u),
              "gemm_nt: a bf16 residual needs bf16 operands, K %% 64 == 0, a compute-type output, and neither an fp32 residual nor gelu_u");
    const double es = dtype ? 2.0 : 4.0;
    const double bytes = (double)M * K * es + (double)N * K * es +
                         (double)M * N * ((epi->res ? 4.0 : 0.0) + (epi->res_t ? 2.0 : 0.0) + (epi->out_f32 ? 4.0 : 0.0) + (epi->out_t ? es : 0.0) +
                                          (epi->out_pre ? es : 0.0) + (epi->gelu_u ? es : 0.0));
    const char* kind = (K % bke != 0) ? "gemm_nt_generic" : "gemm_nt_glds64";
    ProfScope prof(kind, M, N, K, 2.0 * M * N * K, st, bytes);
    if (K % bke == 0) {
        const bool plain_alpha = epi->alpha == 1.0f && !epi->relu_ref;
        int mode = EPI_GENERIC;
        if (epi->drop.on)
            mode = EPI_DROP;
        else if (plain_alpha && epi->out_t && epi->out_pre && epi->act == 1 && !epi->gelu_u && !epi->res && !epi->res_t && !epi->out_f32 && !epi->colsum_part)
            mode = EPI_FC1;
        else if (plain_alpha && epi->out_t && epi->gelu_u && !epi->out_pre && epi->act == 0 && !epi->res && !epi->res_t && !epi->out_f32)
            mode = EPI_DGELU;
        else if (plain_alpha && epi->out_t && !epi->gelu_u && !epi->out_pre && epi->act == 0 && !epi->res && !epi->res_t && !epi->out_f32 && !epi->colsum_part)
            mode = EPI_PLAIN;
        else if (plain_alpha && !epi->out_t && !epi->gelu_u && !epi->out_pre && epi->act == 0 && epi->res && epi->out_f32 && !epi->colsum_part)
            mode = EPI_RES32;
        else if (plain_alpha && epi->out_t && epi->res_t && !epi->gelu_u && !epi->out_pre && epi->act == 0 && !epi->res && !epi->out_f32 && !epi->colsum_part)
            mode = EPI_RES16;
        const bool small = nt_tile_rows(M, N) == 64;
        const dim3 grid(8 * cdiv(N, 64) * cdiv(cdiv(M, small ? 64 : 128), 8));
#define NT_LAUNCH(T, BMv, E) gemm_nt_glds_kernel<T, 64, 2, BMv, E><<<grid, 256, glds_lds_bytes(64, 2, BMv), st>>>((const T*)A, lda, (const T*)W, ldw, M, N, K, *epi)
#define NT_MODES(T, BMv)                                       \
    switch (mode) {                                            \
        case EPI_FC1: NT_LAUNCH(T, BMv, EPI_FC1); break;       \
        case EPI_DGELU: NT_LAUNCH(T, BMv, EPI_DGELU); break;   \
        case EPI_PLAIN: NT_LAUNCH(T, BMv, EPI_PLAIN); break;   \
        case EPI_RES32: NT_LAUNCH(T, BMv, EPI_RES32); break;   \
        case EPI_RES16: NT_LAUNCH(T, BMv, EPI_RES16); break;   \
        case EPI_DROP: NT_LAUNCH(T, BMv, EPI_DROP); break;     \
        default: NT_LAUNCH(T, BMv, EPI_GENERIC); break;        \
    }
        if (dtype == 1) {
            if (small) { NT_MODES(bf16, 64) } else { NT_MODES(bf16, 128) }
        } else {
            if (small) { NT_MODES(float, 64) } else { NT_MODES(float, 128) }
        }
#undef NT_MODES
#undef NT_LAUNCH
    } else {
        M3L_CHECK(epi->colsum_part == nullptr, "gemm_nt: colsum epilogue needs K %% %d == 0", bke);
        M3L_CHECK(!epi->drop.on, "gemm_nt: the dropout epilogue needs K %% %d == 0 (got K=%d)", bke, K);
        dim3 grid(cdiv(N, BN), cdiv(M, BM));
        if (dtype == 1)
            gemm_nt_kernel<bf16><<<grid, 256, NT_LDS_BYTES, st>>>((const bf16*)A, lda, (const bf16*)W, ldw, M, N, K, *epi);
        else
            gemm_nt_kernel<float><<<grid, 256, NT_LDS_BYTES, st>>>((const float*)A, lda, (const float*)W, ldw, M, N, K, *epi);
    }
    M3L_LAUNCH_CHECK();
    return 0;
}

int m3l_gemm_nt_colsum_rows(int M, int N) { return cdiv(M, nt_tile_rows(M, N)); }

static int tn_splits(int M, int tiles) {
    int S = cdiv(512, tiles);
    const int max_s = cdiv(M, 256);
    if (S > max_s) S = max_s;
    if (S < 1) S = 1;
    return S;
}

size_t m3l_gemm_tn_ws_bytes(int M, int N, int K, int* splits_out) {
    const int S = tn_splits(M, cdiv(N, 128) * cdiv(K, 128));
    if (splits_out) *splits_out = S;
    TnProblem p;
    memset(&p, 0, sizeof(p));
    p.N = N; p.K = K;
    return std::max((size_t)S * N * K * sizeof(float), m3l_wgrad_ws_bytes(M, &p, 1));
}

size_t m3l_gemm_tn_grouped_ws_bytes(int M, const TnProblem* probs, int count) {
    size_t f32 = 0;
    for (int c0 = 0; c0 < count; c0 += 4) {
        int tiles = 0;
        size_t elems = 0;
        for (int i = c0; i < std::min(count, c0 + 4); ++i) {
            tiles += cdiv(probs[i].N, 128) * cdiv(probs[i].K, 128);
            elems += (size_t)probs[i].N * probs[i].K;
        }
        f32 = std::max(f32, (size_t)tn_splits(M, tiles > 0 ? tiles : 1) * elems * sizeof(float));
    }
    return std::max(f32, m3l_wgrad_ws_bytes(M, probs, count));
}

static int tn_grouped_f32(TnProblem* probs, int count, int M, float* partial_ws, size_t ws_bytes, int accumulate, hipStream_t st,
                          const float* extra_part, int extra_G, int extra_width, float* extra_out) {
    const int dtype = 0;
    TnGroup grp;
    memset(&grp, 0, sizeof(grp));
    int tiles = 0, maxnk = 0;
    long off = 0;
    double flops = 0, bytes = 0;
    for (int i = 0; i < count; ++i) {
        TnProblem& p = probs[i];
        M3L_CHECK(p.N > 0 && p.K > 0 && p.K % 8 == 0 && p.N % 8 == 0 && p.ldy % 8 == 0 && p.ldx % 8 == 0,
                  "gemm_tn: N,K,ldy,ldx must be positive multiples of 8");
        M3L_CHECK((long)M * p.ldy * 4 < 2147483647L && (long)M * p.ldx * 4 < 2147483647L, "gemm_tn: operand larger than 2 GiB");
        p.tile0 = tiles;
        tiles += cdiv(p.N, 128) * cdiv(p.K, 128);
        if (p.N * p.K > maxnk) maxnk = p.N * p.K;
        flops += 2.0 * M * p.N * p.K;
        bytes += (double)M * (p.N + p.K) * 4;
    }
    const int unit = 32;
    int S = tn_splits(M, tiles);
// ... 61 lines not shown
```

### m3l_amd/csrc/kernels.h

```cpp
#pragma once
#include <hip/hip_runtime.h>
#include <stddef.h>
#include <stdint.h>

#define M3L_MAX_SENSORS 8
#define M3L_MAX_PARTIAL_BLOCKS 2048


struct DropCtx {
    uint32_t thr;
    float scale;
    uint32_t k0, k1;
    uint32_t ctr2;
    int on;
};
DropCtx m3l_drop_ctx(float p, uint64_t seed, int layer, int site);

struct ProfScope {
    int idx;
    hipStream_t stream;
    ProfScope(const char* kind, long a, long b, long c, double work, hipStream_t st, double bytes = 0.0);
    ~ProfScope();
};

// ... 54 lines not shown
    float* part;
    float eps;
};
bool m3l_gemm_nt_rowln_supported(int dtype, int N, int K);
int m3l_gemm_nt_rowln(int dtype, int mode, const void* A, int lda, const void* W, int ldw, int M, int N, int K, const RowLnEpi* ep,
                      hipStream_t st);
constexpr int M3L_REDUCE_BATCH_MAX = 56;
struct ReduceBatchItem {
    const float* part;
    float* out[3];
    int G;
};
struct ReduceBatch {
    ReduceBatchItem it[M3L_REDUCE_BATCH_MAX];
    int count, D;
};
int m3l_reduce_rows_batch(const ReduceBatch* b, int accumulate, hipStream_t st);
int m3l_ln_bwd_blocks(int M);
int m3l_reduce_rows_seg3(const float* part, int G, int D, float* out0, float* out1, float* out2, int accumulate, hipStream_t st);

struct TnProblem {
    const void* Y;
    const void* X;
    int ldy, ldx, N, K;
    float* out;
    int ldo, nvalid, kvalid;
    int tile0;
    long part_off;
    int gelu_x;
};
struct TnGroup {
    TnProblem p[4];
    int count, tiles_total;
    const float* extra_part;
    float* extra_out;
    int extra_G, extra_width;
};
#define M3L_TN_MAX_PROBLEMS 16
#define M3L_TN_MAX_EXTRAS 4
struct TnExtra {
    const float* part;
    float* out;
    int G, width;
};
size_t m3l_gemm_tn_grouped_ws_bytes(int M, const TnProblem* probs, int count);
int m3l_gemm_tn_grouped(int dtype, TnProblem* probs, int count, int M, float* partial_ws, size_t ws_bytes, int accumulate,
                        hipStream_t st, const TnExtra* extras = nullptr, int extra_count = 0);
size_t m3l_wgrad_ws_bytes(int M, const TnProblem* probs, int count);
int m3l_wgrad_layers_per_launch(int M, const TnProblem* layer_probs, int count);
int m3l_wgrad_bf16(TnProblem* probs, int count, int M, float* ws, size_t ws_bytes, int accumulate, hipStream_t st, const TnExtra* extras,
                   int extra_count);
int m3l_gemm_init();
int m3l_gemm_nt_colsum_rows(int M, int N);

int m3l_attn_block_supported(int dtype, int D, int heads, int n, int project_out, int dim_head);
int m3l_attn_block_bwd_enabled(void);
int m3l_attn_block_fwd(int D, int B, int n, const float* x, const float* ln1_w, const float* ln1_b, const void* wqkv, const void* wo,
                       const float* bo, const float* ln2_w, const float* ln2_b, float eps, void* xn1, void* qkv, void* o, float* lse,
                       float* x1, void* xn2, hipStream_t st);
int m3l_mlp_block_supported(int dtype, int D, int mlp, int n);
int m3l_mlp_block_fwd(int D, int mlp, int B, int n, const void* xn2, const float* x1, const void* w1, const float* b1, const void* w2,
                      const float* b2, void* u, void* h, float* xout, hipStream_t st);
int m3l_mlp_block_bwd_supported(int dtype, int D, int mlp, int n);
int m3l_mlp_block_bwd(int D, int mlp, int B, int n, const void* dxt, float* dx, const float* x1, const float* ln2_w, const void* u,
                      const void* w2T, const void* w1T, float eps, void* du, void* dx1t, float* cs_part, float* ln_part, hipStream_t st);
int m3l_attn_block_bwd(int D, int B, int n, const void* dx1t, const float* dres, const float* x, const float* ln1_w, const void* qkv,
                       const void* o, const float* lse, const void* woT, const void* wqkvT, float eps, void* dqkv, float* dx_out, void* dxt_out,
                       float* ln_part, hipStream_t st);
#define M3L_MEGA_MAX_LAYERS 16
#define M3L_MEGA_BWD_MAX_LAYERS 4
int m3l_enc_mega_enabled(void);
int m3l_enc_fwd_mega(int D, int mlp, int B, int n, const float* x0, const void* const* layers, int count, float eps, hipStream_t st);
int m3l_enc_bwd_mega(int D, int mlp, int B, int n, float* dx, const void* const* layers, int count, float eps, hipStream_t st);
unsigned long long* m3l_attn_phase_buffer(void);
int m3l_mlp_t192_supported(int dtype, int D, int mlp, int M);
int m3l_mlp_t192_fwd(int D, int M, int mlp, const void* xn2, const float* x1, const void* w1, const float* b1, const void* w2, const float* b2,
                     void* u, void* h, float* xout, hipStream_t st);
int m3l_attn_t192_fwd_supported(int dtype, int D, int heads, int n, int B, int dim_head);
int m3l_attn_t192_fwd(int D, int B, int n, const float* x, const float* ln_w, const float* ln_b, const void* wqkv, float eps, void* xn1, void* qkv,
                      void* o, float* lse, hipStream_t st);
int m3l_attn_t192_bwd(int D, int B, int n, const void* dx1t, const void* qkv, const void* o, const float* lse, const void* woT, void* dqkv,
                      hipStream_t st);
int m3l_attn_tail_mlp_t192_supported(int dtype, int D, int HD, int mlp, int M, int dim_head);
int m3l_attn_tail_mlp_t192_fwd(int D, int M, int mlp, const void* o, const float* x, const void* wo, const float* bo, const float* ln2_w,
                               const float* ln2_b, float eps, float* x1, void* xn2, const void* w1, const float* b1, const void* w2,
                               const float* b2, void* u, void* h, float* xout, hipStream_t st);
int m3l_mlp_t192_short(void);
int m3l_mlp_t192_tiles(int D, int M);
int m3l_mlp_t192_cs_rows(int D, int M);
int m3l_mlp_t192_bwd(int D, int M, int mlp, const void* dxt, float* dx, const float* x1, const float* ln2_w, const void* u, const void* w2T,
                     const void* w1T, float eps, void* du, void* dx1t, float* cs_part, float* ln_part, hipStream_t st);
int m3l_qkv_bwd_t192_supported(int dtype, int D, int K, int M);
int m3l_qkv_bwd_t192_tiles(int D, int M);
int m3l_qkv_bwd_t192(int D, int M, int K, const void* dqkv, const float* x, const float* ln1_w, const void* wqkvT, const float* dres, float eps,
                     float* dx_out, void* dxt_out, float* ln_part, hipStream_t st);
int m3l_attn_fwd(int dtype, const void* qkv, void* o, float* lse, int B, int n, int H, int DH, hipStream_t st, const DropCtx* drop = nullptr);
int m3l_attn_bwd(int dtype, const void* qkv, const void* o, const void* dO, const float* lse, float* dsum, void* dqkv, int B, int n,
                 int H, int DH, hipStream_t st, const DropCtx* drop = nullptr);
int m3l_dropout_bwd_blocks(int M);
int m3l_dropout_bwd(int dtype, const void* dy, int M, int N, const DropCtx* drop, void* out, float* part, hipStream_t st);
int m3l_dropout_mask(const DropCtx* drop, long rows, int N, uint8_t* out, hipStream_t st);

int m3l_ln_fwd(int out_dtype, const float* x, int M, int D, const float* gamma, const float* beta, float eps, void* y, float* y32,
               hipStream_t st);
int m3l_ln_bwd(int dy_dtype, const void* dy, const float* x, int M, int D, const float* gamma, float eps, const float* dres,
               float* dx_out, void* dx_t_out, int ct_dtype, float* part_ws, float* dgamma, float* dbeta, float* dbias, int accumulate,
// ... 11 lines not shown
int m3l_cast_bf16_f32(const void* x, long count, float* out, hipStream_t st);
int m3l_scale_by_dev(int dtype, const void* x, long count, const float* scale_dev, void* out, hipStream_t st);
int m3l_mask_scale(int mode, const float* src, const void* ref, float scale, long count, float* out, hipStream_t st);
int m3l_vit_tokens(const float* emb, const float* cls, const float* regs, const float* pos, int B, int npatch, int R, int D, float* tok,
                   hipStream_t st);
int m3l_concat2(float* a, int na, float* b2, int nb, int rows, float* cat, int split, hipStream_t st);
int m3l_vt_load_launch(const void* image_nhwc, int image_u8, int B, int H, int W, int C, float img_lo, float img_span, float* image_nchw,
                       const void* tactile, int tactile_u8, int th, int tw, int n_sensors, int frame_stack, float tac_lo, float tac_span,
                       float* const* tactile_out, hipStream_t st);
struct ConvSrc {
    const void* src[M3L_MAX_SENSORS];
    int nsrc, nchw;
};
int m3l_im2col(int dtype, const ConvSrc* src, int Bsrc, int Ci, int H, int W, int KH, int S, int P, int OH, int OW, int Kpad, void* col,
               hipStream_t st);
int m3l_conv_direct_supported(int dtype, int Ci, int Co, int KH, int S, int P, int first_layer);
size_t m3l_conv_wf_elems(int Ci, int Co, int KH);
size_t m3l_conv_wd_elems(int Ci, int Co, int KH, int S);
size_t m3l_conv_wgrad_slab_elems(int B, int Ci, int H, int W, int Co, int KH, int S, int P);
int m3l_conv_prep(const float* W, int Ci, int Co, int KH, int S, void* Wf, void* Wd, hipStream_t st);
int m3l_conv_fwd(const ConvSrc* src, int Bsrc, int B, int Ci, int H, int W, int Co, int KH, int S, int P, const void* Wf, const float* bias,
                 void* out, hipStream_t st);
int m3l_conv_wgrad(const ConvSrc* src, int Bsrc, int B, int Ci, int H, int W, int Co, int KH, int S, int P, const void* dY, float* slab,
                   float* dW, hipStream_t st);
int m3l_conv_dgrad(const void* dY, int B, int Ci, int H, int W, int Co, int KH, int S, int P, const void* Wd, const void* act, void* dX,
                   hipStream_t st);
int m3l_col2im_relu(int dtype, const void* dcol, int Btot, int Ci, int H, int W, int KH, int S, int P, int OH, int OW, int Kpad,
                    const void* act, void* dX, hipStream_t st);
int k_tokens_assemble(const float* img_tok, const float* tac_tok, int B, int D, int n_img, int n_tac, int k, const float* mod,
                        const float* pos_img, const float* pos_tac, float* tokens, hipStream_t st);
int k_tokens_assemble_bwd(const float* dtok, int B, int D, int n_img, int n_tac, int k, float* d_img, float* d_tac, float* part_ws,
                            float* dmod, int accumulate, hipStream_t st);
int m3l_adam_flat(float* p, const float* g, float* m, float* v, long n, float lr, float b1, float b2, float eps, float wd, int step,
                  float gscale, hipStream_t st);
int m3l_adamw_flat(float* p, float* g, float* m, float* v, long n, float lr, float b1, float b2, float eps, float wd, int step, float gscale,
                   float max_norm, float* norm_ws, int scale_grads, hipStream_t st);
int m3l_adam_flat_dev(float* p, const float* g, float* m, float* v, long n, float lr, float b1, float b2, float eps, float wd,
                      int* step_dev, float* bc_dev, hipStream_t st);
struct MaskRankGroup { const float* noise; int n, nm, token_offset, masked_off, unmasked_off; };
struct MaskRankArgs { MaskRankGroup g[M3L_MAX_SENSORS + 1]; int count; };
int m3l_mask_rank_groups(const MaskRankArgs* args, int B, int64_t* masked, int masked_ld, int64_t* unmasked, int unmasked_ld, hipStream_t st);
int m3l_mask_rank(const float* noise, int B, int n, int nm, int token_offset, int64_t* masked, int masked_ld, int masked_off,
                  int64_t* unmasked, int unmasked_ld, int unmasked_off, hipStream_t st);
int m3l_patch_ln(int dtype, const PatchGroup* pg, const int64_t* idx, int idx_ld, int j0, int cnt, int B, const float* gamma,
                 const float* beta, float eps, void* xn, int pdpad, hipStream_t st);
int m3l_patch_ln_bwd(int dtype, const PatchGroup* pg, const int64_t* idx, int idx_ld, int j0, int cnt, int B, float eps,
                     const void* dxn, int pdpad, float* part_ws, float* dgamma, float* dbeta, int accumulate, hipStream_t st);
int m3l_embed_finalize(const float* E, int D, const PatchGroup* pg, const int64_t* idx, int idx_ld, int j0, int cnt, int B,
                       const float* gamma, const float* beta, float eps, const float* mod, int mod0, const float* pos, float* tokens,
                       int L, hipStream_t st);
int m3l_embed_finalize_bwd(int dtype, const float* dtok, int L, const float* E, int D, const PatchGroup* pg, const int64_t* idx,
                           int idx_ld, int j0, int cnt, int B, const float* gamma, float eps, void* dE, float* part_ws, float* dgamma,
                           float* dbeta, float* dmod, int mod0, int accumulate, hipStream_t st);
int k_unshuffle_fwd(const float* src, const float* mask_token, const int64_t* unmasked, int nvis, const int64_t* masked, int nmask,
                      int B, int dd, int n_img, int n_tac, const float* dmod, const float* pos_img, const float* pos_tac, float* dec_in,
                      hipStream_t st);
int k_unshuffle_bwd(const float* dY, const int64_t* unmasked, int nvis, const int64_t* masked, int nmask, int B, int dd, int n_img,
                      int n_tac, int nmod, float* dsrc, float* part_ws, float* dmask_token, float* ddmod, int accumulate, hipStream_t st);
int m3l_gather_rows(int dtype, const void* src, int N, int D, const int64_t* idx, int idx_ld, int j0, int cnt, int B, void* dst,
                    hipStream_t st);
int m3l_gather_rows2(int dtype, const void* src, int N, int D, const int64_t* idx, int idx_ld, int cnt0, int cnt1, int B, void* dst0, void* dst1,
                     hipStream_t st);
int m3l_scatter_rows2(int dtype, const void* src0, const void* src1, int N, int D, const int64_t* idx, int idx_ld, int cnt0, int cnt1, int B,
                      const float* scale_dev, void* dst, hipStream_t st);
int m3l_scatter_rows(int dtype, const void* src, int N, int D, const int64_t* idx, int idx_ld, int j0, int cnt, int B, void* dst,
                     hipStream_t st);
int m3l_mse(int dtype, const float* pred, int pdpad, const PatchGroup* pg, const int64_t* idx, int idx_ld, int j0, int cnt, int B,
            float weight, float* part_ws, int* nblocks_out, void* dpred, float* target_out, hipStream_t st);
```

### m3l_amd/csrc/mae_plan.hip

```cpp
#include <stdarg.h>
#include <stdio.h>
#include <stdlib.h>
#include <string.h>

#include <algorithm>
#include <map>
#include <mutex>
#include <vector>

#include "../../include/m3l_amd.h"
#include "common.cuh"
#include "kernels.h"


namespace {

constexpr float LN_EPS = 1e-5f;

struct SideStream {
    hipStream_t s = nullptr;
    std::vector<hipEvent_t> ev;
    int next = 0;
};
std::mutex g_side_mu;
// ... 45 lines not shown
    bool on = false;
    int fork(hipStream_t st, hipStream_t* s) {
        *s = st;
        if (!g_defer_join || wgrad_inline()) return 0;
        if (side_init()) return 2;
        hipEvent_t ready = side_event();
        M3L_HIP(hipEventRecord(ready, st));
        M3L_HIP(hipStreamWaitEvent(g_side.s, ready, 0));
        *s = g_side.s;
        on = true;
        return 0;
    }
    int end() {
        if (!on) return 0;
        hipEvent_t tail = tail_event();
        M3L_HIP(hipEventRecord(tail, g_side.s));
        std::lock_guard<std::mutex> lock(g_side_mu);
        g_pending.push_back(tail);
        on = false;
        return 0;
    }
};

struct Arena {
    char* base;
    size_t off = 0;
    explicit Arena(void* b) : base(reinterpret_cast<char*>(b)) {}
    void* take(size_t bytes) {
        off = (off + 255) & ~size_t(255);
        void* p = base ? base + off : nullptr;
        off += bytes;
        return p;
    }
    template <typename T> T* take_n(size_t n) { return reinterpret_cast<T*>(take(n * sizeof(T))); }
};

inline int pad8(int x) { return (x + 7) & ~7; }
inline int pad64(int x) { return (x + 63) & ~63; }
int g_rowln = -1;
inline bool use_rowln() {
    if (g_rowln < 0) g_rowln = getenv("M3L_ROWLN") != nullptr ? 1 : 0;
    return g_rowln == 1;
}
inline size_t esz(int dtype) { return dtype ? 2 : 4; }
int g_drop_h = -1;
inline bool drop_h() {
    if (g_drop_h < 0) g_drop_h = getenv("M3L_DROP_H") ? (atoi(getenv("M3L_DROP_H")) > 0 ? 1 : 0) : 0;
    return g_drop_h == 1;
}
int g_res_bf16 = -1;
inline bool res_bf16_mode() {
    if (g_res_bf16 < 0) g_res_bf16 = getenv("M3L_RES_BF16") ? (atoi(getenv("M3L_RES_BF16")) > 0 ? 1 : 0) : 1;
    return g_res_bf16 == 1;
}
struct RbScope {
    explicit RbScope(bool on) { m3l_set_call_rb(on ? 1 : 0); }
    ~RbScope() { m3l_set_call_rb(0); }
};
inline int tf_dh(const m3l_tf_cfg* c) { return c->dim_head ? c->dim_head : 64; }
bool tf_rb(const m3l_tf_cfg* c, int B, int n, bool fuse) {
    if (!res_bf16_mode() || c->dtype != 1 || fuse || !c->project_out || c->depth < 1) return false;
    if (c->mlp_dim % 64 != 0 || (c->heads * tf_dh(c)) % 64 != 0) return false;
    if ((m3l_enc_mega_enabled() & 2) && m3l_attn_block_supported(1, c->dim, c->heads, n, c->project_out, tf_dh(c))) return false;
    (void)B;
    return true;
}
int fused_mlp_kind(const m3l_tf_cfg* c, int B, int n, bool fuse) {
    const int M = B * n, D = c->dim, mlp = c->mlp_dim, dt = c->dtype;
    if (fuse || dt != 1 || tf_dh(c) != 64) return 0;
    const bool block = m3l_attn_block_supported(dt, D, c->heads, n, c->project_out, 64);
    const bool t192 = m3l_mlp_t192_supported(dt, D, mlp, M);
    if (block && !(m3l_mlp_t192_short() && t192) && m3l_mlp_block_supported(dt, D, mlp, n)) return 1;
    return t192 ? 2 : 0;
}

size_t scratch_bytes(int M, const std::vector<std::pair<int, int>>& wshapes, int maxcols) {
    size_t s = (size_t)2048 * 4 * (size_t)maxcols * sizeof(float);
    for (auto& nk : wshapes) s = std::max(s, m3l_gemm_tn_ws_bytes(M, nk.first, nk.second, nullptr));
    return s;
}

GemmEpi epi0(int ldc) {
    GemmEpi e;
    memset(&e, 0, sizeof(e));
    e.ldc = ldc;
    e.alpha = 1.f;
    return e;
}

struct Geo {
    int n_img, n_tac, k;
    int pd_img, pd_tac, pdp_img, pdp_tac;
};
Geo geo_of(const m3l_geom* g) {
    Geo o;
    o.n_img = g->use_vision ? (g->image_h / g->image_patch) * (g->image_w / g->image_patch) : 0;
    o.k = (g->use_tactile && g->num_tactiles > 0) ? g->num_tactiles : 0;
    o.n_tac = o.k ? (g->tactile_h / g->tactile_patch) * (g->tactile_w / g->tactile_patch) : 0;
    o.pd_img = g->image_channels * g->image_patch * g->image_patch;
    o.pd_tac = g->tactile_channels * g->tactile_patch * g->tactile_patch;
    o.pdp_img = pad64(o.pd_img);
    o.pdp_tac = pad64(o.pd_tac);
    return o;
}
PatchGroup group_img(const m3l_geom* g, const Geo& ge, const float* image) {
    PatchGroup pg;
// ... 174 lines not shown
    if (side_init()) return 2;
    hipEvent_t ready = side_event();
    M3L_HIP(hipEventRecord(ready, (hipStream_t)after_stream));
    M3L_HIP(hipStreamWaitEvent(g_side.s, ready, 0));
    *side_out = (void*)g_side.s;
    return 0;
}
int m3l_side_mark_pending(void) {
    if (side_init()) return 2;
    hipEvent_t tail = tail_event();
    M3L_HIP(hipEventRecord(tail, g_side.s));
    std::lock_guard<std::mutex> lock(g_side_mu);
    g_pending.push_back(tail);
    return 0;
}

int m3l_set_defer_join(int on) {
    const int old = g_defer_join;
    g_defer_join = on ? 1 : 0;
    return old;
}

int m3l_side_join(void* stream) {
    std::vector<hipEvent_t> evs;
    {
        std::lock_guard<std::mutex> lock(g_side_mu);
        evs.swap(g_pending);
    }
    for (hipEvent_t ev : evs) M3L_HIP(hipStreamWaitEvent((hipStream_t)stream, ev, 0));
    return (int)0;
}
int m3l_side_pending(void) {
    std::lock_guard<std::mutex> lock(g_side_mu);
    return (int)g_pending.size();
}

int m3l_transformer_rb(const m3l_tf_cfg* c, int B, int n) {
    const int D = c->dim, HD = c->heads * tf_dh(c), mlp = c->mlp_dim;
    return tf_rb(c, B, n, use_rowln() && m3l_gemm_nt_rowln_supported(c->dtype, D, HD) && m3l_gemm_nt_rowln_supported(c->dtype, D, mlp)) ? 1 : 0;
}

int m3l_set_residual_bf16(int on) {
    const int old = res_bf16_mode() ? 1 : 0;
    g_res_bf16 = on ? 1 : 0;
    return old;
}

int m3l_set_drop_h(int on) {
    const int old = drop_h() ? 1 : 0;
    g_drop_h = on ? 1 : 0;
    return old;
}

int m3l_set_rowln(int enable) {
    const int old = use_rowln() ? 1 : 0;
    g_rowln = enable ? 1 : 0;
    return old;
}

int m3l_mask_counts(const m3l_geom* g, double ratio, int* counts_host) {
    if (check_geom(g)) return 1;
    M3L_CHECK(ratio > 0.0 && ratio < 1.0, "masking ratio must be kept between 0 and 1");
    mask_counts(geo_of(g), ratio, counts_host);
    return 0;
}

int m3l_mask_sample(const m3l_geom* g, double ratio, int B, const float* const* noise, int64_t* masked, int64_t* unmasked,
                    void* stream) {
    if (check_geom(g)) return 1;
    M3L_CHECK(ratio > 0.0 && ratio < 1.0, "masking ratio must be kept between 0 and 1");
    int c[6];
    mask_counts(geo_of(g), ratio, c);
    return m3l_mask_sample_counts(g, c[2], c[3], B, noise, masked, unmasked, stream);
}

int m3l_mask_sample_counts(const m3l_geom* g, int nm_img, int nm_tac, int B, const float* const* noise, int64_t* masked,
                           int64_t* unmasked, void* stream) {
    if (check_geom(g)) return 1;
    hipStream_t st = (hipStream_t)stream;
    const Geo ge = geo_of(g);
    M3L_CHECK(nm_img >= 0 && nm_img <= ge.n_img && nm_tac >= 0 && nm_tac <= ge.n_tac, "mask_sample: bad counts %d %d", nm_img, nm_tac);
    const int nmask = nm_img + ge.k * nm_tac, nvis = ge.n_img + ge.k * ge.n_tac - nmask;
    MaskRankArgs a;
    memset(&a, 0, sizeof(a));
    int ni = 0;
    if (ge.n_img > 0) a.g[a.count++] = MaskRankGroup{noise[ni++], ge.n_img, nm_img, 0, 0, 0};
    for (int s = 0; s < ge.k; ++s)
        a.g[a.count++] = MaskRankGroup{noise[ni++], ge.n_tac, nm_tac, ge.n_img + s * ge.n_tac, nm_img + s * nm_tac,
                                       (ge.n_img - nm_img) + s * (ge.n_tac - nm_tac)};
    if (a.count == 0) return 0;
    return m3l_mask_rank_groups(&a, B, masked, nmask, unmasked, nvis, st);
}

namespace {
struct EmbGroupWs {
    void *w, *wT, *xn, *dE, *dxn;
    float* E;
};
struct EmbWs {
    EmbGroupWs g[2];
    float* scratch;
    float* scratch_side;
    size_t scratch_b, total;
};
EmbWs emb_layout(const Geo& ge, int D, int dtype, int B, void* ws) {
    Arena a(ws);
    EmbWs w;
    const size_t e = esz(dtype);
    const int pdp[2] = {ge.pdp_img, ge.pdp_tac};
    const int maxrows[2] = {B * ge.n_img, B * ge.k * ge.n_tac};
    for (int i = 0; i < 2; ++i) {
        w.g[i].w = a.take((size_t)D * pdp[i] * e);
        w.g[i].wT = a.take((size_t)pdp[i] * D * e);
        w.g[i].xn = a.take((size_t)maxrows[i] * pdp[i] * e);
        w.g[i].E = a.take_n<float>((size_t)maxrows[i] * D);
        w.g[i].dE = a.take((size_t)maxrows[i] * D * e);
        w.g[i].dxn = a.take((size_t)maxrows[i] * pdp[i] * e);
    }
    const int Mmax = std::max(maxrows[0], maxrows[1]);
    std::vector<std::pair<int, int>> shapes = {{D, ge.pdp_img}, {D, ge.pdp_tac}};
    w.scratch_b = scratch_bytes(std::max(Mmax, 1), shapes, std::max(D * (2 + M3L_MAX_TACTILES), std::max(ge.pdp_img, ge.pdp_tac)));
    w.scratch = reinterpret_cast<float*>(a.take(w.scratch_b));
    w.scratch_side = reinterpret_cast<float*>(a.take(w.scratch_b));
    w.total = a.off + 256;
    return w;
}
}

size_t m3l_embed_ws_bytes(const m3l_geom* g, int D, int dtype, int B, int L) {
    if (check_geom(g)) return 0;
    const Geo ge = geo_of(g);
    (void)L;
    return emb_layout(ge, D, dtype, B, nullptr).total;
}

namespace {
int embed_run(bool backward, const m3l_geom* g, int D, int dtype, int B, int L, int cnt_img, const int64_t* idx, const float* image,
              const float* const* tactiles, const void* const* tensors, void* ws, float* tokens, const float* dtokens,
              float* const* grads, hipStream_t st) {
    if (check_geom(g)) return 1;
    M3L_CHECK(D % 8 == 0 && D <= 1024, "embed: dim=%d must be a multiple of 8, <= 1024", D);
    const Geo ge = geo_of(g);
    EmbWs w = emb_layout(ge, D, dtype, B, ws);
    M3L_CHECK(idx || L == ge.n_img + ge.k * ge.n_tac, "embed: L=%d must equal the number of patches when idx is NULL", L);
    const int cnt[2] = {cnt_img, L - cnt_img};
    const int j0[2] = {0, cnt_img};
    M3L_CHECK(cnt[0] >= 0 && cnt[1] >= 0 && cnt[0] <= ge.n_img && cnt[1] <= ge.k * ge.n_tac, "embed: inconsistent list split %d/%d", cnt[0], cnt[1]);
    const PatchGroup pgs[2] = {group_img(g, ge, image), group_tac(g, ge, tactiles)};
    const int pd[2] = {ge.pd_img, ge.pd_tac}, pdp[2] = {ge.pdp_img, ge.pdp_tac};
    const float* mod = (const float*)tensors[12];
    const float* pos[2] = {(const float*)tensors[13], (const float*)tensors[14]};
    const int mod0[2] = {0, 1};
    SideSection side;
    if (!backward) {
        WeightPack pk;
        memset(&pk, 0, sizeof(pk));
        for (int i = 0; i < 2; ++i) {
            if (cnt[i] == 0) continue;
            pk.d[pk.count++] = WeightDesc{(const float*)tensors[6 * i + 2], w.g[i].w, w.g[i].wT, D, pd[i], pdp[i], D};
        }
        if (m3l_prep_weights(dtype, &pk, st)) return 1;
        if (m3l_prep_mode() == 1) return 0;
    }
    for (int i = 0; i < 2; ++i) {
        if (cnt[i] == 0) continue;
        const int rows = B * cnt[i];
        const void* const* t = tensors + 6 * i;
        const float *ln1_w = (const float*)t[0], *ln1_b = (const float*)t[1], *W = (const float*)t[2], *bias = (const float*)t[3];
        const float *ln2_w = (const float*)t[4], *ln2_b = (const float*)t[5];
        if (!backward) {
            if (m3l_patch_ln(dtype, &pgs[i], idx, L, j0[i], cnt[i], B, ln1_w, ln1_b, LN_EPS, w.g[i].xn, pdp[i], st)) return 1;
            GemmEpi e = epi0(D);
            e.bias = bias;
            e.out_f32 = w.g[i].E;
            if (m3l_gemm_nt(dtype, w.g[i].xn, pdp[i], w.g[i].w, pdp[i], rows, D, pdp[i], &e, st)) return 1;
            if (m3l_embed_finalize(w.g[i].E, D, &pgs[i], idx, L, j0[i], cnt[i], B, ln2_w, ln2_b, LN_EPS, mod, mod0[i], pos[i], tokens, L, st))
                return 1;
        } else {
            float* const* gr = grads + 6 * i;
            if (m3l_embed_finalize_bwd(dtype, dtokens, L, w.g[i].E, D, &pgs[i], idx, L, j0[i], cnt[i], B, ln2_w, LN_EPS, w.g[i].dE,
                                       w.scratch, gr[4], gr[5], grads[12], mod0[i], 0, st))
                return 1;
            hipStream_t s2;
            if (side.fork(st, &s2)) return 2;
            float* sc = side.on ? w.scratch_side : w.scratch;
            if (m3l_gemm_tn(dtype, w.g[i].dE, D, w.g[i].xn, pdp[i], rows, D, pdp[i], sc, w.scratch_b, gr[2], pd[i], D, pd[i], 0, s2)) return 1;
            if (m3l_colsum(dtype, w.g[i].dE, rows, D, D, sc, gr[3], 0, s2)) return 1;
            GemmEpi e = epi0(pdp[i]);
            e.out_t = w.g[i].dxn;
            if (m3l_gemm_nt(dtype, w.g[i].dE, D, w.g[i].wT, D, rows, pdp[i], D, &e, st)) return 1;
            if (m3l_patch_ln_bwd(dtype, &pgs[i], idx, L, j0[i], cnt[i], B, LN_EPS, w.g[i].dxn, pdp[i], w.scratch, gr[0], gr[1], 0, st))
                return 1;
        }
    }
    return side.end();
}
}

int m3l_embed_fwd(const m3l_geom* g, int D, int dtype, int B, int L, int cnt_img, const int64_t* idx, const float* image,
                  const float* const* tactiles, const void* const* tensors, void* ws, float* tokens, void* stream) {
    return embed_run(false, g, D, dtype, B, L, cnt_img, idx, image, tactiles, tensors, ws, tokens, nullptr, nullptr, (hipStream_t)stream);
}
int m3l_embed_bwd(const m3l_geom* g, int D, int dtype, int B, int L, int cnt_img, const int64_t* idx, const float* image,
                  const float* const* tactiles, const void* const* tensors, void* ws, const float* dtokens, float* const* grads,
                  void* stream) {
    return embed_run(true, g, D, dtype, B, L, cnt_img, idx, image, tactiles, tensors, ws, nullptr, dtokens, grads, (hipStream_t)stream);
}

size_t m3l_transformer_ws_bytes(const m3l_tf_cfg* c, int B, int n) { return m3l_transformer_ws_bytes_dropout(c, B, n, nullptr); }

size_t m3l_transformer_ws_bytes_dropout(const m3l_tf_cfg* c, int B, int n, const m3l_dropout* drop) {
    if (check_tf(c, B, n)) return 0;
    return tf_layout(c, B, n, nullptr, drop_active(drop)).total;
}

// ... 642 lines not shown
        w.g[i].pred = a.take_n<float>(rows * pdp[i]);
        w.g[i].dpred = a.take(rows * pdp[i] * e);
        w.g[i].dpred_s = a.take(rows * pdp[i] * e);
        w.g[i].ddg = a.take(rows * dd * e);
    }
    w.loss_part = a.take_n<float>(2 * M3L_MAX_PARTIAL_BLOCKS);
    std::vector<std::pair<int, int>> shapes = {{ge.pdp_img, dd}, {ge.pdp_tac, dd}};
    w.scratch_b = scratch_bytes((int)std::max(rows, (size_t)1), shapes, std::max(dd, std::max(ge.pdp_img, ge.pdp_tac)));
    w.scratch = reinterpret_cast<float*>(a.take(w.scratch_b));
    w.scratch_side = reinterpret_cast<float*>(a.take(w.scratch_b));
    w.total = a.off + 256;
    return w;
}
}

size_t m3l_heads_ws_bytes(const m3l_geom* g, int dd, int dtype, int B, int nmask) {
    if (check_geom(g)) return 0;
    return head_layout(geo_of(g), dd, dtype, B, nmask, nullptr).total;
}

int m3l_heads_loss_fwd(const m3l_geom* g, int dd, int dtype, int B, int N, int nmask, int nm_img, const int64_t* masked,
                       const float* image, const float* const* tactiles, const void* dec_t, const void* const* tensors, void* ws,
                       float* loss, float* pred_img, float* tgt_img, float* pred_tac, float* tgt_tac, void* stream) {
    return m3l_heads_loss_fwd2(g, dd, dtype, B, N, nmask, nm_img, masked, image, tactiles, dec_t, tensors, ws, loss, nullptr, pred_img,
                               tgt_img, pred_tac, tgt_tac, stream);
}

int m3l_heads_loss_fwd2(const m3l_geom* g, int dd, int dtype, int B, int N, int nmask, int nm_img, const int64_t* masked,
                        const float* image, const float* const* tactiles, const void* dec_t, const void* const* tensors, void* ws,
                        float* loss, float* loss_parts, float* pred_img, float* tgt_img, float* pred_tac, float* tgt_tac, void* stream) {
    if (check_geom(g)) return 1;
    hipStream_t st = (hipStream_t)stream;
    const Geo ge = geo_of(g);
    HeadWs w = head_layout(ge, dd, dtype, B, nmask, ws);
    const int cnt[2] = {nm_img, nmask - nm_img}, j0[2] = {0, nm_img};
    const int pd[2] = {ge.pd_img, ge.pd_tac}, pdp[2] = {ge.pdp_img, ge.pdp_tac};
    const float weight[2] = {1.f, 10.f};
    const PatchGroup pgs[2] = {group_img(g, ge, image), group_tac(g, ge, tactiles)};
    float* tgt[2] = {tgt_img, tgt_tac};
    float* pred_out[2] = {pred_img, pred_tac};
    int nparts = 0;
    int part_beg[2] = {0, 0}, part_cnt[2] = {0, 0};
    {
        WeightPack pk;
        memset(&pk, 0, sizeof(pk));
        for (int i = 0; i < 2; ++i) {
            if (cnt[i] == 0) continue;
            pk.d[pk.count++] = WeightDesc{(const float*)tensors[2 * i], w.g[i].w, w.g[i].wT, pd[i], dd, dd, pdp[i]};
        }
        if (m3l_prep_weights(dtype, &pk, st)) return 1;
        if (m3l_prep_mode() == 1) return 0;
    }
    if (m3l_gather_rows2(dtype, dec_t, N, dd, masked, nmask, cnt[0], cnt[1], B, w.g[0].dg, w.g[1].dg, st)) return 1;
    for (int i = 0; i < 2; ++i) {
        if (cnt[i] == 0) continue;
        const int rows = B * cnt[i];
        GemmEpi e = epi0(pdp[i]);
        e.bias = (const float*)tensors[2 * i + 1];
        e.n_bias = pd[i];
        e.out_f32 = w.g[i].pred;
        if (m3l_gemm_nt(dtype, w.g[i].dg, dd, w.g[i].w, dd, rows, pdp[i], dd, &e, st)) return 1;
        int nb = 0;
        if (m3l_mse(dtype, w.g[i].pred, pdp[i], &pgs[i], masked, nmask, j0[i], cnt[i], B, weight[i], w.loss_part + nparts, &nb,
                    w.g[i].dpred, tgt[i], st))
            return 1;
        part_beg[i] = nparts; part_cnt[i] = nb;
        nparts += nb;
        if (pred_out[i])
            M3L_HIP(hipMemcpy2DAsync(pred_out[i], (size_t)pd[i] * 4, w.g[i].pred, (size_t)pdp[i] * 4, (size_t)pd[i] * 4, rows,
                                     hipMemcpyDeviceToDevice, st));
    }
    if (loss_parts) {
        M3L_HIP(hipMemsetAsync(loss_parts, 0, 2 * sizeof(float), st));
        for (int i = 0; i < 2; ++i)
            if (part_cnt[i] && m3l_reduce_rows(w.loss_part + part_beg[i], part_cnt[i], 1, 1, loss_parts + i, 0, st)) return 1;
    }
    return m3l_reduce_rows(w.loss_part, nparts, 1, 1, loss, 0, st);
}

int m3l_heads_loss_bwd(const m3l_geom* g, int dd, int dtype, int B, int N, int nmask, int nm_img, const int64_t* masked,
                       const void* const* tensors, void* ws, const float* dloss, void* d_dec, float* const* grads, void* stream) {
    if (check_geom(g)) return 1;
    (void)tensors;
    hipStream_t st = (hipStream_t)stream;
    const Geo ge = geo_of(g);
    HeadWs w = head_layout(ge, dd, dtype, B, nmask, ws);
    const int cnt[2] = {nm_img, nmask - nm_img}, j0[2] = {0, nm_img};
    const int pd[2] = {ge.pd_img, ge.pd_tac}, pdp[2] = {ge.pdp_img, ge.pdp_tac};
    M3L_HIP(hipMemsetAsync(d_dec, 0, (size_t)B * N * dd * esz(dtype), st));
    SideSection side;
    for (int i = 0; i < 2; ++i) {
        if (cnt[i] == 0) continue;
        const int rows = B * cnt[i];
        hipStream_t s2;
        if (side.fork(st, &s2)) return 2;
        const void* dpred = w.g[i].dpred;
        if (dloss) {
            if (m3l_scale_by_dev(dtype, w.g[i].dpred, (long)rows * pdp[i], dloss, w.g[i].dpred_s, s2)) return 1;
            dpred = w.g[i].dpred_s;
        }
        float* sc = side.on ? w.scratch_side : w.scratch;
        if (m3l_gemm_tn(dtype, dpred, pdp[i], w.g[i].dg, dd, rows, pdp[i], dd, sc, w.scratch_b, grads[2 * i], dd, pd[i], dd, 0, s2)) return 1;
        if (m3l_colsum(dtype, dpred, rows, pd[i], pdp[i], sc, grads[2 * i + 1], 0, s2)) return 1;
        GemmEpi e = epi0(dd);
        e.out_t = w.g[i].ddg;
        if (m3l_gemm_nt(dtype, w.g[i].dpred, pdp[i], w.g[i].wT, pdp[i], rows, dd, pdp[i], &e, st)) return 1;
    }
    if (m3l_scatter_rows2(dtype, w.g[0].ddg, w.g[1].ddg, N, dd, masked, nmask, cnt[0], cnt[1], B, dloss, d_dec, st)) return 1;
    return side.end();
}

namespace {
struct ConvL { int Ci, Co, KH, S, P, H, W, OH, OW, K, Kpad; long M; };
struct CnnWs {
    ConvL L[4];
    void *col[3], *act[3], *w[4], *wT[4];
    void *dout_t, *dpreA, *dpreB, *dcol;
    void *wf[3], *wd[3];
    float* slab;
    bool direct;
    float* scratch;
    size_t scratch_b, total;
};
int g_direct_conv = -1;
bool cnn_direct(const m3l_cnn_cfg* c) {
    if (g_direct_conv < 0) g_direct_conv = getenv("M3L_DIRECT_CONV") ? (atoi(getenv("M3L_DIRECT_CONV")) > 0 ? 1 : 0) : 1;
    if (!g_direct_conv || c->dtype != 1) return false;
    const int D = c->dim, co[3] = {D / 8, D / 4, D / 2};
    int ci = c->in_channels;
    for (int l = 0; l < 3; ++l) {
        const bool k3 = l == 2 && c->tactile;
        if (!m3l_conv_direct_supported(c->dtype, ci, co[l], k3 ? 3 : 4, k3 ? 1 : 2, 1, l == 0)) return false;
        ci = co[l];
    }
    return true;
}
CnnWs cnn_layout(const m3l_cnn_cfg* c, int Btot, void* ws) {
    Arena a(ws);
    CnnWs w;
    const int D = c->dim;
    const int co[4] = {D / 8, D / 4, D / 2, D};
    int ci = c->in_channels, H = c->height, W = c->width;
    for (int l = 0; l < 4; ++l) {
        ConvL& L = w.L[l];
// ... 308 lines not shown
```

Baseline: 71820 samples/s.

## Pair-launch image and tactile embed/head kernels in single grid launches

Adds paired variants of the patch LN, embed finalize, MSE, colsum, scale and NT GEMM kernels, so the image and tactile modality groups run in one launch with the block index split between them. The embed backward also batches its column reductions into one table-driven reduce kernel, replacing several per-tensor reduce launches. This targets kernel-launch overhead and the poor occupancy of the small per-modality launches at this tiny model size. It is on by default through an env and setter toggle, at the cost of more code paths and shared memory sized for the larger modality.

```diff
diff --git a/include/m3l_amd.h b/include/m3l_amd.h
--- a/include/m3l_amd.h
+++ b/include/m3l_amd.h
@@ -49,6 +49,7 @@
 void* m3l_side_stream(void);
 int m3l_side_pending(void);
 int m3l_set_drop_h(int on);
+int m3l_set_pair_launch(int on);
 int m3l_set_t192(int on);
 int m3l_set_t192_tt(int tt);
 int m3l_set_residual_bf16(int on);
diff --git a/m3l_amd/_lib.py b/m3l_amd/_lib.py
--- a/m3l_amd/_lib.py
+++ b/m3l_amd/_lib.py
@@ -43,6 +43,7 @@
     "m3l_set_attn_phase_buffer": (None, [c_p]),
     "m3l_set_enc_mega": (c_i, [c_i]),
     "m3l_set_drop_h": (c_i, [c_i]),
+    "m3l_set_pair_launch": (c_i, [c_i]),
     "m3l_set_direct_conv": (c_i, [c_i]),
     "m3l_set_t192": (c_i, [c_i]),
     "m3l_set_t192_tt": (c_i, [c_i]),
diff --git a/m3l_amd/csrc/elementwise.hip b/m3l_amd/csrc/elementwise.hip
--- a/m3l_amd/csrc/elementwise.hip
+++ b/m3l_amd/csrc/elementwise.hip
@@ -203,6 +203,13 @@
     reduce_cols_32x32(part + (long)blockIdx.y * width, G, stride, j, j < width, out, accumulate);
 }
 
+__global__ __launch_bounds__(1024) void reduce_rows_table_kernel(ReduceTable t, int accumulate) {
+    const ReduceTableItem it = t.it[blockIdx.y];
+    if (!it.out || (int)blockIdx.x * 32 >= it.width) return;
+    const int j = blockIdx.x * 32 + (threadIdx.x & 31);
+    reduce_cols_32x32(it.part, it.G, it.stride, j, j < it.width, it.out, accumulate);
+}
+
 __global__ __launch_bounds__(1024) void reduce_rows_batch_kernel(ReduceBatch b, int accumulate) {
     const ReduceBatchItem it = b.it[blockIdx.z];
     float* out = it.out[blockIdx.y];
@@ -215,10 +222,12 @@
 template <> struct Vec4<bf16> { typedef bf16x4 type; };
 template <> struct Vec4<float> { typedef f32x4 type; };
 template <typename T>
-__global__ __launch_bounds__(256) void colsum_kernel(const T* __restrict__ Y, int M, int N, int ld, int rows_per_block,
-                                                       float* __restrict__ part, int vec_ok) {
+__device__ __forceinline__ void colsum_body(const ColsumArgs& a, int bid) {
     typedef typename Vec4<T>::type V4;
-    const int r0 = blockIdx.x * rows_per_block, r1 = min(M, r0 + rows_per_block);
+    const T* __restrict__ Y = reinterpret_cast<const T*>(a.Y);
+    float* __restrict__ part = a.part;
+    const int M = a.M, N = a.N, ld = a.ld, rows_per_block = a.rows_per_block, vec_ok = a.vec_ok;
+    const int r0 = bid * rows_per_block, r1 = min(M, r0 + rows_per_block);
     for (int c = threadIdx.x * 4; c < N; c += 1024) {
         if (vec_ok && c + 4 <= N) {
             f32x4 s0 = f32x4{0.f, 0.f, 0.f, 0.f}, s1 = s0, s2 = s0, s3 = s0;
@@ -234,7 +243,7 @@
                 s3 += ld4(r + 3);
             }
             for (; r < r1; ++r) s0 += ld4(r);
-            *reinterpret_cast<f32x4*>(part + (long)blockIdx.x * N + c) = (s0 + s1) + (s2 + s3);
+            *reinterpret_cast<f32x4*>(part + (long)bid * N + c) = (s0 + s1) + (s2 + s3);
         } else {
             for (int cc = c; cc < min(N, c + 4); ++cc) {
                 float s0 = 0.f, s1 = 0.f, s2 = 0.f, s3 = 0.f;
@@ -246,10 +255,17 @@
                     s3 += to_f32(Y[(long)(r + 3) * ld + cc]);
                 }
                 for (; r < r1; ++r) s0 += to_f32(Y[(long)r * ld + cc]);
-                part[(long)blockIdx.x * N + cc] = (s0 + s1) + (s2 + s3);
+                part[(long)bid * N + cc] = (s0 + s1) + (s2 + s3);
             }
         }
     }
+}
+template <typename T>
+__global__ __launch_bounds__(256) void colsum_kernel(ColsumArgs a) { colsum_body<T>(a, blockIdx.x); }
+template <typename T>
+__global__ __launch_bounds__(256) void colsum_pair_kernel(ColsumArgs a0, ColsumArgs a1, int blocks0) {
+    if ((int)blockIdx.x < blocks0) colsum_body<T>(a0, blockIdx.x);
+    else colsum_body<T>(a1, blockIdx.x - blocks0);
 }
 
 template <typename T>
@@ -311,9 +327,19 @@
 }
 
 template <typename T>
+__device__ __forceinline__ void scale_by_dev_body(const T* __restrict__ x, long count, const float* __restrict__ s, T* __restrict__ out, int bid) {
+    const long i = (long)bid * blockDim.x + threadIdx.x;
+    if (i < count) out[i] = from_f32<T>(to_f32(x[i]) * s[0]);
+}
+template <typename T>
 __global__ void scale_by_dev_kernel(const T* __restrict__ x, long count, const float* __restrict__ s, T* __restrict__ out) {
-    const long i = (long)blockIdx.x * blockDim.x + threadIdx.x;
-    if (i < count) out[i] = from_f32<T>(to_f32(x[i]) * s[0]);
+    scale_by_dev_body<T>(x, count, s, out, blockIdx.x);
+}
+template <typename T>
+__global__ void scale_by_dev_pair_kernel(const T* __restrict__ x0, long count0, T* __restrict__ out0, const T* __restrict__ x1, long count1,
+                                         T* __restrict__ out1, const float* __restrict__ s, int blocks0) {
+    if ((int)blockIdx.x < blocks0) scale_by_dev_body<T>(x0, count0, s, out0, blockIdx.x);
+    else scale_by_dev_body<T>(x1, count1, s, out1, blockIdx.x - blocks0);
 }
 
 template <int MODE>
@@ -665,14 +691,18 @@
 }
 
 template <typename T, int NV>
-__global__ __launch_bounds__(256) void patch_ln_kernel(PatchGroup pg, const int64_t* __restrict__ idx, int idx_ld, int j0, int cnt,
-                                                         int rows, const float* __restrict__ gamma, const float* __restrict__ beta,
-                                                         float eps, T* __restrict__ xn, int pdpad, int vec) {
-    __shared__ __attribute__((aligned(16))) float buf[WPB][NV * 64];
-    const int lane = threadIdx.x & 63, wave = threadIdx.x >> 6, row = blockIdx.x * WPB + wave;
+__device__ __forceinline__ void patch_ln_body(const PatchLnArgs& a, int bid, float* buf) {
+    const PatchGroup& pg = a.pg;
+    const int64_t* __restrict__ idx = a.idx;
+    const float* __restrict__ gamma = a.gamma;
+    const float* __restrict__ beta = a.beta;
+    T* __restrict__ xn = reinterpret_cast<T*>(a.xn);
+    const int idx_ld = a.idx_ld, j0 = a.j0, cnt = a.cnt, rows = a.rows, pdpad = a.pdpad, vec = a.vec;
+    const float eps = a.eps;
+    const int lane = threadIdx.x & 63, wave = threadIdx.x >> 6, row = bid * WPB + wave;
     const int pd = pg.C * pg.P * pg.P;
     const PatchDiv dv = patch_div(pg);
-    float* my = buf[wave];
+    float* my = buf + wave * (NV * 64);
     const bool live = row < rows;
     float mean = 0.f, rstd = 0.f;
     if (live) {
@@ -705,22 +735,36 @@
         for (int e = lane; e < pdpad; e += 64) out[e] = from_f32<T>(e < pd ? (my[e] - mean) * rstd * gamma[e] + beta[e] : 0.f);
     }
 }
-
 template <typename T, int NV>
-__global__ __launch_bounds__(256) void patch_ln_bwd_kernel(PatchGroup pg, const int64_t* __restrict__ idx, int idx_ld, int j0, int cnt,
-                                                             int rows, float eps, const T* __restrict__ dxn, int pdpad,
-                                                             float* __restrict__ part, int vec) {
-    __shared__ __attribute__((aligned(16))) float buf[WPB][NV * 64];
-    constexpr int NC = NV / 4;
+__global__ __launch_bounds__(256) void patch_ln_kernel(PatchLnArgs a) {
+    __shared__ __attribute__((aligned(16))) float buf[WPB * NV * 64];
+    patch_ln_body<T, NV>(a, blockIdx.x, buf);
+}
+template <typename T, int NV0, int NV1>
+__global__ __launch_bounds__(256) void patch_ln_pair_kernel(PatchLnArgs a0, PatchLnArgs a1, int blocks0) {
+    __shared__ __attribute__((aligned(16))) float buf[WPB * (NV0 > NV1 ? NV0 : NV1) * 64];
+    if ((int)blockIdx.x < blocks0) patch_ln_body<T, NV0>(a0, blockIdx.x, buf);
+    else patch_ln_body<T, NV1>(a1, blockIdx.x - blocks0, buf);
+}
+
+template <typename T, int NV>
+__device__ __forceinline__ void patch_ln_bwd_body(const PatchLnBwdArgs& a, int bid, int nblk, float* buf) {
+    const PatchGroup& pg = a.pg;
+    const int64_t* __restrict__ idx = a.idx;
+    const T* __restrict__ dxn = reinterpret_cast<const T*>(a.dxn);
+    float* __restrict__ part = a.part;
+    const int idx_ld = a.idx_ld, j0 = a.j0, cnt = a.cnt, rows = a.rows, pdpad = a.pdpad, vec = a.vec;
+    const float eps = a.eps;
+    constexpr int NC = NV / 4, BS = NV * 64;
     static_assert(NV % 4 == 0, "4-element pieces");
     const int lane = threadIdx.x & 63, wave = threadIdx.x >> 6;
     const int pd = pg.C * pg.P * pg.P;
     const PatchDiv dv = patch_div(pg);
-    float* my = buf[wave];
+    float* my = buf + wave * BS;
     f32x4 dg[NC], db[NC];
 #pragma unroll
     for (int k = 0; k < NC; ++k) dg[k] = db[k] = f32x4{0.f, 0.f, 0.f, 0.f};
-    for (int r0 = blockIdx.x * WPB; r0 < rows; r0 += gridDim.x * WPB) {
+    for (int r0 = bid * WPB; r0 < rows; r0 += nblk * WPB) {
         const int row = r0 + wave;
         const bool live = row < rows;
         float mean = 0.f, rstd = 0.f;
@@ -763,23 +807,40 @@
         }
         __syncthreads();
     }
-    float* out = part + (long)blockIdx.x * 2 * pd;
+    float* out = part + (long)bid * 2 * pd;
 #pragma unroll
     for (int pass = 0; pass < 2; ++pass) {
 #pragma unroll
         for (int k = 0; k < NC; ++k) *reinterpret_cast<f32x4*>(my + 4 * (lane + 64 * k)) = pass ? db[k] : dg[k];
         __syncthreads();
-        for (int e = threadIdx.x; e < pd; e += 256) out[pass * pd + e] = buf[0][e] + buf[1][e] + buf[2][e] + buf[3][e];
+        for (int e = threadIdx.x; e < pd; e += 256) out[pass * pd + e] = buf[e] + buf[BS + e] + buf[2 * BS + e] + buf[3 * BS + e];
         __syncthreads();
     }
 }
-
-__global__ __launch_bounds__(256) void embed_finalize_kernel(const float* __restrict__ E, int rows, int D, PatchGroup pg,
-                                                               const int64_t* __restrict__ idx, int idx_ld, int j0, int cnt,
-                                                               const float* __restrict__ gamma, const float* __restrict__ beta,
-                                                               float eps, const float* __restrict__ mod, int mod0,
-                                                               const float* __restrict__ pos, float* __restrict__ tokens, int L) {
-    const int lane = threadIdx.x & 63, row = blockIdx.x * WPB + (threadIdx.x >> 6);
+template <typename T, int NV>
+__global__ __launch_bounds__(256) void patch_ln_bwd_kernel(PatchLnBwdArgs a) {
+    __shared__ __attribute__((aligned(16))) float buf[WPB * NV * 64];
+    patch_ln_bwd_body<T, NV>(a, blockIdx.x, gridDim.x, buf);
+}
+template <typename T, int NV0, int NV1>
+__global__ __launch_bounds__(256) void patch_ln_bwd_pair_kernel(PatchLnBwdArgs a0, PatchLnBwdArgs a1, int blocks0) {
+    __shared__ __attribute__((aligned(16))) float buf[WPB * (NV0 > NV1 ? NV0 : NV1) * 64];
+    if ((int)blockIdx.x < blocks0) patch_ln_bwd_body<T, NV0>(a0, blockIdx.x, blocks0, buf);
+    else patch_ln_bwd_body<T, NV1>(a1, blockIdx.x - blocks0, gridDim.x - blocks0, buf);
+}
+
+__device__ __forceinline__ void embed_finalize_body(const EmbedFinArgs& a, int bid) {
+    const PatchGroup& pg = a.pg;
+    const float* __restrict__ E = a.E;
+    const int64_t* __restrict__ idx = a.idx;
+    const float* __restrict__ gamma = a.gamma;
+    const float* __restrict__ beta = a.beta;
+    const float* __restrict__ mod = a.mod;
+    const float* __restrict__ pos = a.pos;
+    float* __restrict__ tokens = a.tokens;
+    const int rows = a.rows, D = a.D, idx_ld = a.idx_ld, j0 = a.j0, cnt = a.cnt, mod0 = a.mod0, L = a.L;
+    const float eps = a.eps;
+    const int lane = threadIdx.x & 63, row = bid * WPB + (threadIdx.x >> 6);
     if (row >= rows) return;
     int b, s, ph, pw, local;
     patch_locate(pg, idx, idx_ld, j0, cnt, row, b, s, ph, pw, local);
@@ -811,19 +872,29 @@
         if (e < D) out[e] = (v[i] - mean) * rstd * gamma[e] + beta[e] + mrow[e] + prow[e];
     }
 }
-
-template <typename T>
-__global__ __launch_bounds__(256) void embed_finalize_bwd_kernel(const float* __restrict__ dtok, int L, const float* __restrict__ E,
-                                                                   int rows, int D, PatchGroup pg, const int64_t* __restrict__ idx,
-                                                                   int idx_ld, int j0, int cnt, const float* __restrict__ gamma,
-                                                                   float eps, T* __restrict__ dE, float* __restrict__ part, int nslot) {
-    extern __shared__ float sm[];
+__global__ __launch_bounds__(256) void embed_finalize_kernel(EmbedFinArgs a) { embed_finalize_body(a, blockIdx.x); }
+__global__ __launch_bounds__(256) void embed_finalize_pair_kernel(EmbedFinArgs a0, EmbedFinArgs a1, int blocks0) {
+    if ((int)blockIdx.x < blocks0) embed_finalize_body(a0, blockIdx.x);
+    else embed_finalize_body(a1, blockIdx.x - blocks0);
+}
+
+template <typename T>
+__device__ __forceinline__ void embed_finalize_bwd_body(const EmbedFinBwdArgs& a, int bid, int nblk, float* sm) {
+    const PatchGroup& pg = a.pg;
+    const float* __restrict__ dtok = a.dtok;
+    const float* __restrict__ E = a.E;
+    const int64_t* __restrict__ idx = a.idx;
+    const float* __restrict__ gamma = a.gamma;
+    T* __restrict__ dE = reinterpret_cast<T*>(a.dE);
+    float* __restrict__ part = a.part;
+    const int L = a.L, rows = a.rows, D = a.D, idx_ld = a.idx_ld, j0 = a.j0, cnt = a.cnt, nslot = a.nslot;
+    const float eps = a.eps;
     const int lane = threadIdx.x & 63, wave = threadIdx.x >> 6;
     const int PL = (2 + nslot) * D;
     for (int i = threadIdx.x; i < WPB * PL; i += 256) sm[i] = 0.f;
     __syncthreads();
     float* my = sm + wave * PL;
-    for (int row = blockIdx.x * WPB + wave; row < rows; row += gridDim.x * WPB) {
+    for (int row = bid * WPB + wave; row < rows; row += nblk * WPB) {
         int b, s, ph, pw, local;
         patch_locate(pg, idx, idx_ld, j0, cnt, row, b, s, ph, pw, local);
         const int jj = row % cnt;
@@ -876,7 +947,18 @@
     }
     __syncthreads();
     for (int i = threadIdx.x; i < PL; i += 256)
-        part[(long)blockIdx.x * PL + i] = sm[i] + sm[PL + i] + sm[2 * PL + i] + sm[3 * PL + i];
+        part[(long)bid * PL + i] = sm[i] + sm[PL + i] + sm[2 * PL + i] + sm[3 * PL + i];
+}
+template <typename T>
+__global__ __launch_bounds__(256) void embed_finalize_bwd_kernel(EmbedFinBwdArgs a) {
+    extern __shared__ float sm[];
+    embed_finalize_bwd_body<T>(a, blockIdx.x, gridDim.x, sm);
+}
+template <typename T>
+__global__ __launch_bounds__(256) void embed_finalize_bwd_pair_kernel(EmbedFinBwdArgs a0, EmbedFinBwdArgs a1, int blocks0) {
+    extern __shared__ float sm[];
+    if ((int)blockIdx.x < blocks0) embed_finalize_bwd_body<T>(a0, blockIdx.x, blocks0, sm);
+    else embed_finalize_bwd_body<T>(a1, blockIdx.x - blocks0, gridDim.x - blocks0, sm);
 }
 
 template <typename TO>
@@ -1059,17 +1141,21 @@
 }
 
 template <typename T>
-__global__ __launch_bounds__(256) void mse_kernel(const float* __restrict__ pred, int pdpad, PatchGroup pg,
-                                                    const int64_t* __restrict__ idx, int idx_ld, int j0, int cnt, int rows, float w,
-                                                    float* __restrict__ part, T* __restrict__ dpred, float* __restrict__ target_out, int vec) {
-    extern __shared__ __attribute__((aligned(16))) float mbuf[];
-    __shared__ float red[WPB];
+__device__ __forceinline__ void mse_body(const MseArgs& a, int bid, int nblk, float* mbuf, float* red) {
+    const PatchGroup& pg = a.pg;
+    const float* __restrict__ pred = a.pred;
+    const int64_t* __restrict__ idx = a.idx;
+    float* __restrict__ part = a.part;
+    T* __restrict__ dpred = reinterpret_cast<T*>(a.dpred);
+    float* __restrict__ target_out = a.target_out;
+    const int pdpad = a.pdpad, idx_ld = a.idx_ld, j0 = a.j0, cnt = a.cnt, rows = a.rows, vec = a.vec;
+    const float w = a.w;
     const int lane = threadIdx.x & 63, wave = threadIdx.x >> 6;
     const int pd = pg.C * pg.P * pg.P;
     const PatchDiv dv = patch_div(pg);
     float* my = mbuf + (long)wave * pdpad;
     float acc = 0.f;
-    for (int r0 = blockIdx.x * WPB; r0 < rows; r0 += gridDim.x * WPB) {
+    for (int r0 = bid * WPB; r0 < rows; r0 += nblk * WPB) {
         const int row = r0 + wave;
         const bool live = row < rows;
         if (live) {
@@ -1126,7 +1212,20 @@
     acc = wave_sum(acc);
     if (lane == 0) red[wave] = acc;
     __syncthreads();
-    if (threadIdx.x == 0) part[blockIdx.x] = w * (red[0] + red[1] + red[2] + red[3]);
+    if (threadIdx.x == 0) part[bid] = w * (red[0] + red[1] + red[2] + red[3]);
+}
+template <typename T>
+__global__ __launch_bounds__(256) void mse_kernel(MseArgs a) {
+    extern __shared__ __attribute__((aligned(16))) float mbuf[];
+    __shared__ float red[WPB];
+    mse_body<T>(a, blockIdx.x, gridDim.x, mbuf, red);
+}
+template <typename T>
+__global__ __launch_bounds__(256) void mse_pair_kernel(MseArgs a0, MseArgs a1, int blocks0) {
+    extern __shared__ __attribute__((aligned(16))) float mbuf[];
+    __shared__ float red[WPB];
+    if ((int)blockIdx.x < blocks0) mse_body<T>(a0, blockIdx.x, blocks0, mbuf, red);
+    else mse_body<T>(a1, blockIdx.x - blocks0, gridDim.x - blocks0, mbuf, red);
 }
 
 }
@@ -1141,7 +1240,7 @@
     }();
     return nb;
 }
-static int part_grid(long rows) {
+int m3l_part_grid(long rows) {
     long g = (rows + WPB - 1) / WPB;
     if (g > m3l_part_blocks()) g = m3l_part_blocks();
     return (int)(g < 1 ? 1 : g);
@@ -1226,20 +1325,64 @@
     return 0;
 }
 
-int m3l_colsum(int dtype, const void* Y, int M, int N, int ld, float* part_ws, float* out, int accumulate, hipStream_t st) {
-    M3L_CHECK(M > 0 && N > 0, "colsum: bad shape");
+static int colsum_setup(const void* Y, int M, int N, int ld, float* part_ws, ColsumArgs* a) {
     int G = cdiv(M, N > 512 ? 16 : 64);
     if (G > m3l_part_blocks()) G = m3l_part_blocks();
     const int rpb = cdiv(M, G);
     G = cdiv(M, rpb);
+    const int vec_ok = (ld % 4 == 0) && (N % 4 == 0) && (((unsigned long)Y) % 16 == 0) && (((unsigned long)part_ws) % 16 == 0);
+    *a = ColsumArgs{Y, part_ws, M, N, ld, rpb, vec_ok};
+    return G;
+}
+
+int m3l_colsum(int dtype, const void* Y, int M, int N, int ld, float* part_ws, float* out, int accumulate, hipStream_t st) {
+    M3L_CHECK(M > 0 && N > 0, "colsum: bad shape");
+    ColsumArgs a;
+    const int G = colsum_setup(Y, M, N, ld, part_ws, &a);
     ProfScope prof("colsum", M, N, dtype, (double)M * N * (dtype ? 2 : 4), st);
-    const int vec_ok = (ld % 4 == 0) && (N % 4 == 0) && (((unsigned long)Y) % 16 == 0) && (((unsigned long)part_ws) % 16 == 0);
     if (dtype == 1)
-        colsum_kernel<bf16><<<G, 256, 0, st>>>((const bf16*)Y, M, N, ld, rpb, part_ws, vec_ok);
+        colsum_kernel<bf16><<<G, 256, 0, st>>>(a);
     else
-        colsum_kernel<float><<<G, 256, 0, st>>>((const float*)Y, M, N, ld, rpb, part_ws, vec_ok);
+        colsum_kernel<float><<<G, 256, 0, st>>>(a);
     M3L_LAUNCH_CHECK();
     return m3l_reduce_rows(part_ws, G, N, N, out, accumulate, st);
+}
+
+int m3l_reduce_rows_table(const ReduceTable* t, int accumulate, hipStream_t st) {
+    if (t->count <= 0) return 0;
+    M3L_CHECK(t->count <= M3L_REDUCE_TABLE_MAX, "reduce_rows_table: count=%d", t->count);
+    int wmax = 0;
+    for (int i = 0; i < t->count; ++i) {
+        M3L_CHECK(!t->it[i].out || (t->it[i].G > 0 && t->it[i].width > 0), "reduce_rows_table: entry %d: G=%d width=%d", i, t->it[i].G, t->it[i].width);
+        if (t->it[i].out) wmax = std::max(wmax, t->it[i].width);
+    }
+    if (wmax == 0) return 0;
+    reduce_rows_table_kernel<<<dim3(cdiv(wmax, 32), t->count), 1024, 0, st>>>(*t, accumulate);
+    M3L_LAUNCH_CHECK();
+    return 0;
+}
+
+int m3l_colsum_pair(int dtype, const void* const* Y, const int* M, const int* N, const int* ld, float* part_ws, float* const* out,
+                    int accumulate, hipStream_t st) {
+    M3L_CHECK(M[0] > 0 && N[0] > 0 && M[1] > 0 && N[1] > 0, "colsum_pair: bad shape");
+    ColsumArgs a[2];
+    const int G0 = colsum_setup(Y[0], M[0], N[0], ld[0], part_ws, &a[0]);
+    float* part1 = part_ws + (((long)G0 * N[0] + 3) & ~3L);
+    const int G1 = colsum_setup(Y[1], M[1], N[1], ld[1], part1, &a[1]);
+    {
+        ProfScope prof("colsum", M[0] + M[1], N[0], dtype, ((double)M[0] * N[0] + (double)M[1] * N[1]) * (dtype ? 2 : 4), st);
+        if (dtype == 1)
+            colsum_pair_kernel<bf16><<<G0 + G1, 256, 0, st>>>(a[0], a[1], G0);
+        else
+            colsum_pair_kernel<float><<<G0 + G1, 256, 0, st>>>(a[0], a[1], G0);
+        M3L_LAUNCH_CHECK();
+    }
+    ReduceTable t;
+    memset(&t, 0, sizeof(t));
+    t.count = 2;
+    t.it[0] = ReduceTableItem{part_ws, out[0], G0, N[0], N[0]};
+    t.it[1] = ReduceTableItem{part1, out[1], G1, N[1], N[1]};
+    return m3l_reduce_rows_table(&t, accumulate, st);
 }
 
 static thread_local int g_prep_mode = 0;
@@ -1386,7 +1529,7 @@
                             float* dmod, int accumulate, hipStream_t st) {
     const long rows = (long)B * (n_img + k * n_tac);
     const int PL = (1 + k) * D;
-    const int G = part_grid(rows);
+    const int G = m3l_part_grid(rows);
     tokens_assemble_bwd_kernel<<<G, 256, WPB * PL * sizeof(float), st>>>(dtok, B, D, n_img, n_tac > 0 ? n_tac : 1, k, d_img, d_tac, part_ws);
     M3L_LAUNCH_CHECK();
     reduce_rows_kernel<<<cdiv(PL, 32), 1024, 0, st>>>(part_ws, G, PL, PL, dmod, accumulate);
@@ -1445,6 +1588,17 @@
     return 0;
 }
 
+int m3l_scale_by_dev_pair(int dtype, const void* const* x, const long* count, const float* scale_dev, void* const* out, hipStream_t st) {
+    const int g0 = (int)cdiv(count[0], 256), g1 = (int)cdiv(count[1], 256);
+    M3L_CHECK(g0 > 0 && g1 > 0, "scale_by_dev_pair: empty group");
+    if (dtype == 1)
+        scale_by_dev_pair_kernel<bf16><<<g0 + g1, 256, 0, st>>>((const bf16*)x[0], count[0], (bf16*)out[0], (const bf16*)x[1], count[1], (bf16*)out[1], scale_dev, g0);
+    else
+        scale_by_dev_pair_kernel<float><<<g0 + g1, 256, 0, st>>>((const float*)x[0], count[0], (float*)out[0], (const float*)x[1], count[1], (float*)out[1], scale_dev, g0);
+    M3L_LAUNCH_CHECK();
+    return 0;
+}
+
 int m3l_mask_scale(int mode, const float* src, const void* ref, float scale, long count, float* out, hipStream_t st) {
     M3L_CHECK((mode == 0 || mode == 1) && count > 0 && src && ref && out, "mask_scale: bad arguments");
     if (mode == 0) mask_scale_kernel<0><<<cdiv(count, 256), 256, 0, st>>>(src, ref, scale, count, out);
@@ -1527,21 +1681,57 @@
     return 0;
 }
 
+static int patch_nvc(int pd) { return pd > 64 * MAXV ? 2 : (pd <= 256 ? 0 : 1); }
+#define PATCH_NV1(LAUNCH, T, c) \
+    { if ((c) == 2) { LAUNCH(T, PATCH_NV_MAX); } else if ((c) == 0) { LAUNCH(T, 4); } else { LAUNCH(T, MAXV); } }
+#define PATCH_NV2_(LAUNCH, T, NV0, c1) \
+    { if ((c1) == 2) { LAUNCH(T, NV0, PATCH_NV_MAX); } else if ((c1) == 0) { LAUNCH(T, NV0, 4); } else { LAUNCH(T, NV0, MAXV); } }
+#define PATCH_NV2(LAUNCH, T, c0, c1) \
+    { if ((c0) == 2) PATCH_NV2_(LAUNCH, T, PATCH_NV_MAX, c1) else if ((c0) == 0) PATCH_NV2_(LAUNCH, T, 4, c1) else PATCH_NV2_(LAUNCH, T, MAXV, c1) }
+
+int m3l_patch_ln_vec(int dtype, const PatchGroup* pg, int pdpad, const float* gamma, const float* beta, const void* xn) {
+    const int pd = pg->C * pg->P * pg->P;
+    return pd % 4 == 0 && pdpad % 4 == 0 && aligned_to(gamma, 16) && aligned_to(beta, 16) && aligned_to(xn, 4 * (dtype == 1 ? 2 : 4));
+}
+int m3l_patch_ln_bwd_vec(int dtype, const PatchGroup* pg, int pdpad, const void* dxn) {
+    const int pd = pg->C * pg->P * pg->P;
+    return pd % 4 == 0 && pdpad % 4 == 0 && aligned_to(dxn, 4 * (dtype == 1 ? 2 : 4));
+}
+int m3l_mse_vec(int dtype, const PatchGroup* pg, int pdpad, const float* pred, const void* dpred, const float* target_out) {
+    const int pd = pg->C * pg->P * pg->P;
+    return pd % 4 == 0 && pdpad % 4 == 0 && aligned_to(pred, 16) && aligned_to(dpred, 4 * (dtype == 1 ? 2 : 4)) &&
+           (!target_out || aligned_to(target_out, 16));
+}
+
 int m3l_patch_ln(int dtype, const PatchGroup* pg, const int64_t* idx, int idx_ld, int j0, int cnt, int B, const float* gamma,
                  const float* beta, float eps, void* xn, int pdpad, hipStream_t st) {
     if (check_pg(*pg)) return 1;
     const int rows = B * cnt;
     if (rows == 0) return 0;
-    const int pd_ = pg->C * pg->P * pg->P, esz = dtype == 1 ? 2 : 4;
-    const bool wide = pd_ > 64 * MAXV, tiny = pd_ <= 256;
-    const int vec = pd_ % 4 == 0 && pdpad % 4 == 0 && aligned_to(gamma, 16) && aligned_to(beta, 16) && aligned_to(xn, 4 * esz);
-#define PATCH_LN(T, NV) patch_ln_kernel<T, NV><<<ln_grid(rows), 256, 0, st>>>(*pg, idx, idx_ld, j0, cnt, rows, gamma, beta, eps, (T*)xn, pdpad, vec)
-    if (dtype == 1) {
-        if (wide) PATCH_LN(bf16, PATCH_NV_MAX); else if (tiny) PATCH_LN(bf16, 4); else PATCH_LN(bf16, MAXV);
-    } else {
-        if (wide) PATCH_LN(float, PATCH_NV_MAX); else if (tiny) PATCH_LN(float, 4); else PATCH_LN(float, MAXV);
-    }
+    const int nvc = patch_nvc(pg->C * pg->P * pg->P);
+    const PatchLnArgs a = {*pg, idx, gamma, beta, xn, idx_ld, j0, cnt, rows, pdpad, m3l_patch_ln_vec(dtype, pg, pdpad, gamma, beta, xn), eps};
+#define PATCH_LN(T, NV) patch_ln_kernel<T, NV><<<ln_grid(rows), 256, 0, st>>>(a)
+    if (dtype == 1) PATCH_NV1(PATCH_LN, bf16, nvc) else PATCH_NV1(PATCH_LN, float, nvc)
 #undef PATCH_LN
+    M3L_LAUNCH_CHECK();
+    return 0;
+}
+
+int m3l_patch_ln_pair(int dtype, const PatchGroup* pg, const int64_t* idx, int idx_ld, const int* j0, const int* cnt, int B,
+                      const float* const* gamma, const float* const* beta, float eps, void* const* xn, const int* pdpad, hipStream_t st) {
+    if (check_pg(pg[0]) || check_pg(pg[1])) return 1;
+    PatchLnArgs a[2];
+    int nvc[2];
+    for (int i = 0; i < 2; ++i) {
+        M3L_CHECK(B * cnt[i] > 0, "patch_ln_pair: group %d is empty", i);
+        M3L_CHECK(m3l_patch_ln_vec(dtype, &pg[i], pdpad[i], gamma[i], beta[i], xn[i]), "patch_ln_pair: group %d takes the element-wise walk", i);
+        nvc[i] = patch_nvc(pg[i].C * pg[i].P * pg[i].P);
+        a[i] = PatchLnArgs{pg[i], idx, gamma[i], beta[i], xn[i], idx_ld, j0[i], cnt[i], B * cnt[i], pdpad[i], 1, eps};
+    }
+    const int g0 = ln_grid(a[0].rows), g1 = ln_grid(a[1].rows);
+#define PATCH_LN2(T, NV0, NV1) patch_ln_pair_kernel<T, NV0, NV1><<<g0 + g1, 256, 0, st>>>(a[0], a[1], g0)
+    if (dtype == 1) PATCH_NV2(PATCH_LN2, bf16, nvc[0], nvc[1]) else PATCH_NV2(PATCH_LN2, float, nvc[0], nvc[1])
+#undef PATCH_LN2
     M3L_LAUNCH_CHECK();
     return 0;
 }
@@ -1552,19 +1742,34 @@
     const int rows = B * cnt;
     if (rows == 0) return 0;
     const int pd = pg->C * pg->P * pg->P;
-    const int G = part_grid(rows);
-    const bool wide = pd > 64 * MAXV, tiny = pd <= 256;
-    const int vec = pd % 4 == 0 && pdpad % 4 == 0 && aligned_to(dxn, 4 * (dtype == 1 ? 2 : 4));
-#define PATCH_LN_BWD(T, NV) patch_ln_bwd_kernel<T, NV><<<G, 256, 0, st>>>(*pg, idx, idx_ld, j0, cnt, rows, eps, (const T*)dxn, pdpad, part_ws, vec)
-    if (dtype == 1) {
-        if (wide) PATCH_LN_BWD(bf16, PATCH_NV_MAX); else if (tiny) PATCH_LN_BWD(bf16, 4); else PATCH_LN_BWD(bf16, MAXV);
-    } else {
-        if (wide) PATCH_LN_BWD(float, PATCH_NV_MAX); else if (tiny) PATCH_LN_BWD(float, 4); else PATCH_LN_BWD(float, MAXV);
-    }
+    const int G = m3l_part_grid(rows);
+    const int nvc = patch_nvc(pd);
+    const PatchLnBwdArgs a = {*pg, idx, dxn, part_ws, idx_ld, j0, cnt, rows, pdpad, m3l_patch_ln_bwd_vec(dtype, pg, pdpad, dxn), eps};
+#define PATCH_LN_BWD(T, NV) patch_ln_bwd_kernel<T, NV><<<G, 256, 0, st>>>(a)
+    if (dtype == 1) PATCH_NV1(PATCH_LN_BWD, bf16, nvc) else PATCH_NV1(PATCH_LN_BWD, float, nvc)
 #undef PATCH_LN_BWD
     M3L_LAUNCH_CHECK();
     ReduceSegs segs = {{dgamma, dbeta, nullptr, nullptr}};
     reduce_rows_seg_kernel<<<dim3(cdiv(pd, 32), 2), 1024, 0, st>>>(part_ws, G, 2 * pd, pd, segs, accumulate);
+    M3L_LAUNCH_CHECK();
+    return 0;
+}
+
+int m3l_patch_ln_bwd_pair(int dtype, const PatchGroup* pg, const int64_t* idx, int idx_ld, const int* j0, const int* cnt, int B, float eps,
+                          const void* const* dxn, const int* pdpad, float* const* part_ws, hipStream_t st) {
+    if (check_pg(pg[0]) || check_pg(pg[1])) return 1;
+    PatchLnBwdArgs a[2];
+    int nvc[2];
+    for (int i = 0; i < 2; ++i) {
+        M3L_CHECK(B * cnt[i] > 0, "patch_ln_bwd_pair: group %d is empty", i);
+        M3L_CHECK(m3l_patch_ln_bwd_vec(dtype, &pg[i], pdpad[i], dxn[i]), "patch_ln_bwd_pair: group %d takes the element-wise walk", i);
+        nvc[i] = patch_nvc(pg[i].C * pg[i].P * pg[i].P);
+        a[i] = PatchLnBwdArgs{pg[i], idx, dxn[i], part_ws[i], idx_ld, j0[i], cnt[i], B * cnt[i], pdpad[i], 1, eps};
+    }
+    const int g0 = m3l_part_grid(a[0].rows), g1 = m3l_part_grid(a[1].rows);
+#define PATCH_LN_BWD2(T, NV0, NV1) patch_ln_bwd_pair_kernel<T, NV0, NV1><<<g0 + g1, 256, 0, st>>>(a[0], a[1], g0)
+    if (dtype == 1) PATCH_NV2(PATCH_LN_BWD2, bf16, nvc[0], nvc[1]) else PATCH_NV2(PATCH_LN_BWD2, float, nvc[0], nvc[1])
+#undef PATCH_LN_BWD2
     M3L_LAUNCH_CHECK();
     return 0;
 }
@@ -1575,7 +1780,23 @@
     const int rows = B * cnt;
     if (rows == 0) return 0;
     M3L_CHECK(D <= 64 * MAXV, "embed_finalize: D=%d too large", D);
-    embed_finalize_kernel<<<ln_grid(rows), 256, 0, st>>>(E, rows, D, *pg, idx, idx_ld, j0, cnt, gamma, beta, eps, mod, mod0, pos, tokens, L);
+    const EmbedFinArgs a = {*pg, E, idx, gamma, beta, mod, pos, tokens, rows, D, idx_ld, j0, cnt, mod0, L, eps};
+    embed_finalize_kernel<<<ln_grid(rows), 256, 0, st>>>(a);
+    M3L_LAUNCH_CHECK();
+    return 0;
+}
+
+int m3l_embed_finalize_pair(const float* const* E, int D, const PatchGroup* pg, const int64_t* idx, int idx_ld, const int* j0,
+                            const int* cnt, int B, const float* const* gamma, const float* const* beta, float eps, const float* mod,
+                            const int* mod0, const float* const* pos, float* tokens, int L, hipStream_t st) {
+    M3L_CHECK(D <= 64 * MAXV, "embed_finalize: D=%d too large", D);
+    EmbedFinArgs a[2];
+    for (int i = 0; i < 2; ++i) {
+        M3L_CHECK(B * cnt[i] > 0, "embed_finalize_pair: group %d is empty", i);
+        a[i] = EmbedFinArgs{pg[i], E[i], idx, gamma[i], beta[i], mod, pos[i], tokens, B * cnt[i], D, idx_ld, j0[i], cnt[i], mod0[i], L, eps};
+    }
+    const int g0 = ln_grid(a[0].rows), g1 = ln_grid(a[1].rows);
+    embed_finalize_pair_kernel<<<g0 + g1, 256, 0, st>>>(a[0], a[1], g0);
     M3L_LAUNCH_CHECK();
     return 0;
 }
@@ -1587,11 +1808,12 @@
     if (rows == 0) return 0;
     const int nslot = pg->nsrc;
     const int PL = (2 + nslot) * D;
-    const int G = part_grid(rows);
+    const int G = m3l_part_grid(rows);
+    const EmbedFinBwdArgs a = {*pg, dtok, E, idx, gamma, dE, part_ws, L, rows, D, idx_ld, j0, cnt, nslot, eps};
     if (dtype == 1)
-        embed_finalize_bwd_kernel<bf16><<<G, 256, WPB * PL * sizeof(float), st>>>(dtok, L, E, rows, D, *pg, idx, idx_ld, j0, cnt, gamma, eps, (bf16*)dE, part_ws, nslot);
+        embed_finalize_bwd_kernel<bf16><<<G, 256, WPB * PL * sizeof(float), st>>>(a);
     else
-        embed_finalize_bwd_kernel<float><<<G, 256, WPB * PL * sizeof(float), st>>>(dtok, L, E, rows, D, *pg, idx, idx_ld, j0, cnt, gamma, eps, (float*)dE, part_ws, nslot);
+        embed_finalize_bwd_kernel<float><<<G, 256, WPB * PL * sizeof(float), st>>>(a);
     M3L_LAUNCH_CHECK();
     if (nslot <= 2) {
         float* dm = dmod + (long)mod0 * D;
@@ -1602,6 +1824,24 @@
         reduce_rows_kernel<<<cdiv(D, 32), 1024, 0, st>>>(part_ws + D, G, PL, D, dbeta, accumulate);
         reduce_rows_kernel<<<cdiv(nslot * D, 32), 1024, 0, st>>>(part_ws + 2 * D, G, PL, nslot * D, dmod + (long)mod0 * D, accumulate);
     }
+    M3L_LAUNCH_CHECK();
+    return 0;
+}
+
+int m3l_embed_finalize_bwd_pair(int dtype, const float* dtok, int L, const float* const* E, int D, const PatchGroup* pg,
+                                const int64_t* idx, int idx_ld, const int* j0, const int* cnt, int B, const float* const* gamma,
+                                float eps, void* const* dE, float* const* part_ws, hipStream_t st) {
+    EmbedFinBwdArgs a[2];
+    for (int i = 0; i < 2; ++i) {
+        M3L_CHECK(B * cnt[i] > 0, "embed_finalize_bwd_pair: group %d is empty", i);
+        a[i] = EmbedFinBwdArgs{pg[i], dtok, E[i], idx, gamma[i], dE[i], part_ws[i], L, B * cnt[i], D, idx_ld, j0[i], cnt[i], pg[i].nsrc, eps};
+    }
+    const int g0 = m3l_part_grid(a[0].rows), g1 = m3l_part_grid(a[1].rows);
+    const size_t lds = (size_t)WPB * (2 + std::max(a[0].nslot, a[1].nslot)) * D * sizeof(float);
+    if (dtype == 1)
+        embed_finalize_bwd_pair_kernel<bf16><<<g0 + g1, 256, lds, st>>>(a[0], a[1], g0);
+    else
+        embed_finalize_bwd_pair_kernel<float><<<g0 + g1, 256, lds, st>>>(a[0], a[1], g0);
     M3L_LAUNCH_CHECK();
     return 0;
 }
@@ -1704,26 +1944,57 @@
     return 0;
 }
 
+static int mse_setup(int dtype, const float* pred, int pdpad, const PatchGroup* pg, const int64_t* idx, int idx_ld, int j0, int cnt, int B,
+                     float weight, float* part_ws, void* dpred, float* target_out, MseArgs* a, size_t* lds) {
+    const int rows = B * cnt;
+    if (rows == 0) return 0;
+    const int pd = pg->C * pg->P * pg->P;
+    const float w = weight / ((float)rows * (float)pd);
+    if (pdpad < pd) { m3l_set_error("mse: pdpad %d < patch dim %d", pdpad, pd); return -1; }
+    *lds = (size_t)WPB * pdpad * sizeof(float);
+    if (*lds > 64 * 1024) { m3l_set_error("mse: padded patch dim %d too wide", pdpad); return -1; }
+    *a = MseArgs{*pg, pred, idx, part_ws, dpred, target_out, pdpad, idx_ld, j0, cnt, rows, m3l_mse_vec(dtype, pg, pdpad, pred, dpred, target_out), w};
+    return m3l_part_grid(rows);
+}
+
 int m3l_mse(int dtype, const float* pred, int pdpad, const PatchGroup* pg, const int64_t* idx, int idx_ld, int j0, int cnt, int B,
             float weight, float* part_ws, int* nblocks_out, void* dpred, float* target_out, hipStream_t st) {
     if (check_pg(*pg)) return 1;
-    const int rows = B * cnt;
     if (nblocks_out) *nblocks_out = 0;
-    if (rows == 0) return 0;
-    const int pd = pg->C * pg->P * pg->P;
-    const float w = weight / ((float)rows * (float)pd);
-    const int G = part_grid(rows);
-    M3L_CHECK(pdpad >= pd, "mse: pdpad %d < patch dim %d", pdpad, pd);
-    const int vec = pd % 4 == 0 && pdpad % 4 == 0 && aligned_to(pred, 16) && aligned_to(dpred, 4 * (dtype == 1 ? 2 : 4)) &&
-                    (!target_out || aligned_to(target_out, 16));
-    const size_t lds = (size_t)WPB * pdpad * sizeof(float);
-    M3L_CHECK(lds <= 64 * 1024, "mse: padded patch dim %d too wide", pdpad);
+    MseArgs a;
+    size_t lds = 0;
+    const int G = mse_setup(dtype, pred, pdpad, pg, idx, idx_ld, j0, cnt, B, weight, part_ws, dpred, target_out, &a, &lds);
+    if (G <= 0) return G < 0 ? 1 : 0;
     if (dtype == 1)
-        mse_kernel<bf16><<<G, 256, lds, st>>>(pred, pdpad, *pg, idx, idx_ld, j0, cnt, rows, w, part_ws, (bf16*)dpred, target_out, vec);
+        mse_kernel<bf16><<<G, 256, lds, st>>>(a);
     else
-        mse_kernel<float><<<G, 256, lds, st>>>(pred, pdpad, *pg, idx, idx_ld, j0, cnt, rows, w, part_ws, (float*)dpred, target_out, vec);
+        mse_kernel<float><<<G, 256, lds, st>>>(a);
     M3L_LAUNCH_CHECK();
     if (nblocks_out) *nblocks_out = G;
+    return 0;
+}
+
+int m3l_mse_pair(int dtype, const float* const* pred, const int* pdpad, const PatchGroup* pg, const int64_t* idx, int idx_ld,
+                 const int* j0, const int* cnt, int B, const float* weight, float* part_ws, int* nblocks_out, void* const* dpred,
+                 float* const* target_out, hipStream_t st) {
+    if (check_pg(pg[0]) || check_pg(pg[1])) return 1;
+    MseArgs a[2];
+    size_t lds[2] = {0, 0};
+    int G[2] = {0, 0};
+    for (int i = 0; i < 2; ++i) {
+        G[i] = mse_setup(dtype, pred[i], pdpad[i], &pg[i], idx, idx_ld, j0[i], cnt[i], B, weight[i], part_ws + (i ? G[0] : 0), dpred[i],
+                         target_out[i], &a[i], &lds[i]);
+        if (G[i] < 0) return 1;
+        M3L_CHECK(G[i] > 0, "mse_pair: group %d is empty", i);
+        M3L_CHECK(a[i].vec, "mse_pair: group %d takes the element-wise walk", i);
+    }
+    if (dtype == 1)
+        mse_pair_kernel<bf16><<<G[0] + G[1], 256, std::max(lds[0], lds[1]), st>>>(a[0], a[1], G[0]);
+    else
+        mse_pair_kernel<float><<<G[0] + G[1], 256, std::max(lds[0], lds[1]), st>>>(a[0], a[1], G[0]);
+    M3L_LAUNCH_CHECK();
+    nblocks_out[0] = G[0];
+    nblocks_out[1] = G[1];
     return 0;
 }
 
diff --git a/m3l_amd/csrc/gemm.hip b/m3l_amd/csrc/gemm.hip
--- a/m3l_amd/csrc/gemm.hip
+++ b/m3l_amd/csrc/gemm.hip
@@ -154,10 +154,9 @@
 }
 
 enum { EPI_GENERIC = 0, EPI_FC1 = 1, EPI_DGELU = 2, EPI_PLAIN = 3, EPI_RES32 = 4, EPI_RES16 = 5, EPI_DROP = 6 };
-template <typename T, int BN, int R, int BM = 128, int EPI = 0>
-__global__ __launch_bounds__(256) void gemm_nt_glds_kernel(const T* __restrict__ A, int lda, const T* __restrict__ W, int ldw,
-                                                             int M, int N, int K, GemmEpi epi) {
-    extern __shared__ __attribute__((aligned(16))) char smem[];
+template <typename T, int BN, int R, int BM, int EPI>
+__device__ __forceinline__ void gemm_nt_glds_body(const T* __restrict__ A, int lda, const T* __restrict__ W, int ldw, int M, int N, int K,
+                                                  const GemmEpi& epi, const int bid, char* smem) {
     constexpr int EPC = Chunk<T>::N;
     constexpr int BKE = 8 * EPC;
     constexpr int KSTEPS = BKE / 32;
@@ -173,7 +172,7 @@
     const int g = lane >> 4, li = lane & 15;
     const int wr = (BN == 128) ? (wave >> 1) : wave, wc = (BN == 128) ? (wave & 1) : 0;
     const int gx = (N + BN - 1) / BN, gy = (M + BM - 1) / BM;
-    const int bid = blockIdx.x, rest = bid >> 3;
+    const int rest = bid >> 3;
     const int bx = rest % gx, by = (rest / gx) * 8 + (bid & 7);
     if (by >= gy) return;
     const int m0 = by * BM, n0 = bx * BN;
@@ -422,6 +421,20 @@
         }
     }
 }
+template <typename T, int BN, int R, int BM = 128, int EPI = 0>
+__global__ __launch_bounds__(256) void gemm_nt_glds_kernel(const T* __restrict__ A, int lda, const T* __restrict__ W, int ldw,
+                                                             int M, int N, int K, GemmEpi epi) {
+    extern __shared__ __attribute__((aligned(16))) char smem[];
+    gemm_nt_glds_body<T, BN, R, BM, EPI>(A, lda, W, ldw, M, N, K, epi, blockIdx.x, smem);
+}
+template <typename T, int BN, int R, int BM, int EPI>
+__global__ __launch_bounds__(256) void gemm_nt_glds_pair_kernel(NtProblem p0, NtProblem p1, int blocks0) {
+    extern __shared__ __attribute__((aligned(16))) char smem[];
+    if ((int)blockIdx.x < blocks0)
+        gemm_nt_glds_body<T, BN, R, BM, EPI>((const T*)p0.A, p0.lda, (const T*)p0.W, p0.ldw, p0.M, p0.N, p0.K, p0.epi, blockIdx.x, smem);
+    else
+        gemm_nt_glds_body<T, BN, R, BM, EPI>((const T*)p1.A, p1.lda, (const T*)p1.W, p1.ldw, p1.M, p1.N, p1.K, p1.epi, blockIdx.x - blocks0, smem);
+}
 
 template <typename T> struct TnSwz;
 template <> struct TnSwz<bf16> {
@@ -609,9 +622,29 @@
     NT_ATTR5(bf16, 128); NT_ATTR5(float, 128); NT_ATTR5(bf16, 64); NT_ATTR5(float, 64);
 #undef NT_ATTR5
 #undef NT_ATTR
+#define NT_ATTR_P(T, BMv, E) M3L_HIP(hipFuncSetAttribute((const void*)gemm_nt_glds_pair_kernel<T, 64, 2, BMv, E>, hipFuncAttributeMaxDynamicSharedMemorySize, glds_lds_bytes(64, 2, BMv)))
+#define NT_ATTR_P2(T, BMv) NT_ATTR_P(T, BMv, EPI_GENERIC); NT_ATTR_P(T, BMv, EPI_PLAIN)
+    NT_ATTR_P2(bf16, 128); NT_ATTR_P2(float, 128); NT_ATTR_P2(bf16, 64); NT_ATTR_P2(float, 64);
+#undef NT_ATTR_P2
+#undef NT_ATTR_P
     M3L_HIP(hipFuncSetAttribute((const void*)gemm_tn_glds_kernel<float>, hipFuncAttributeMaxDynamicSharedMemorySize, 65536));
     g_gemm_inited = 1;
     return 0;
+}
+
+static int nt_epi_mode(const GemmEpi* epi) {
+    const bool plain_alpha = epi->alpha == 1.0f && !epi->relu_ref;
+    if (epi->drop.on) return EPI_DROP;
+    if (plain_alpha && epi->out_t && epi->out_pre && epi->act == 1 && !epi->gelu_u && !epi->res && !epi->res_t && !epi->out_f32 && !epi->colsum_part)
+        return EPI_FC1;
+    if (plain_alpha && epi->out_t && epi->gelu_u && !epi->out_pre && epi->act == 0 && !epi->res && !epi->res_t && !epi->out_f32) return EPI_DGELU;
+    if (plain_alpha && epi->out_t && !epi->gelu_u && !epi->out_pre && epi->act == 0 && !epi->res && !epi->res_t && !epi->out_f32 && !epi->colsum_part)
+        return EPI_PLAIN;
+    if (plain_alpha && !epi->out_t && !epi->gelu_u && !epi->out_pre && epi->act == 0 && epi->res && epi->out_f32 && !epi->colsum_part)
+        return EPI_RES32;
+    if (plain_alpha && epi->out_t && epi->res_t && !epi->gelu_u && !epi->out_pre && epi->act == 0 && !epi->res && !epi->out_f32 && !epi->colsum_part)
+        return EPI_RES16;
+    return EPI_GENERIC;
 }
 
 int m3l_gemm_nt(int dtype, const void* A, int lda, const void* W, int ldw, int M, int N, int K, const GemmEpi* epi_in,
@@ -634,20 +667,7 @@
     const char* kind = (K % bke != 0) ? "gemm_nt_generic" : "gemm_nt_glds64";
     ProfScope prof(kind, M, N, K, 2.0 * M * N * K, st, bytes);
     if (K % bke == 0) {
-        const bool plain_alpha = epi->alpha == 1.0f && !epi->relu_ref;
-        int mode = EPI_GENERIC;
-        if (epi->drop.on)
-            mode = EPI_DROP;
-        else if (plain_alpha && epi->out_t && epi->out_pre && epi->act == 1 && !epi->gelu_u && !epi->res && !epi->res_t && !epi->out_f32 && !epi->colsum_part)
-            mode = EPI_FC1;
-        else if (plain_alpha && epi->out_t && epi->gelu_u && !epi->out_pre && epi->act == 0 && !epi->res && !epi->res_t && !epi->out_f32)
-            mode = EPI_DGELU;
-        else if (plain_alpha && epi->out_t && !epi->gelu_u && !epi->out_pre && epi->act == 0 && !epi->res && !epi->res_t && !epi->out_f32 && !epi->colsum_part)
-            mode = EPI_PLAIN;
-        else if (plain_alpha && !epi->out_t && !epi->gelu_u && !epi->out_pre && epi->act == 0 && epi->res && epi->out_f32 && !epi->colsum_part)
-            mode = EPI_RES32;
-        else if (plain_alpha && epi->out_t && epi->res_t && !epi->gelu_u && !epi->out_pre && epi->act == 0 && !epi->res && !epi->out_f32 && !epi->colsum_part)
-            mode = EPI_RES16;
+        const int mode = nt_epi_mode(epi);
         const bool small = nt_tile_rows(M, N) == 64;
         const dim3 grid(8 * cdiv(N, 64) * cdiv(cdiv(M, small ? 64 : 128), 8));
 #define NT_LAUNCH(T, BMv, E) gemm_nt_glds_kernel<T, 64, 2, BMv, E><<<grid, 256, glds_lds_bytes(64, 2, BMv), st>>>((const T*)A, lda, (const T*)W, ldw, M, N, K, *epi)
@@ -682,6 +702,52 @@
 }
 
 int m3l_gemm_nt_colsum_rows(int M, int N) { return cdiv(M, nt_tile_rows(M, N)); }
+
+bool m3l_gemm_nt_pair_ok(int dtype, const NtProblem* p) {
+    if (dtype != 0 && dtype != 1) return false;
+    const int bke = dtype == 1 ? 64 : 32;
+    for (int i = 0; i < 2; ++i) {
+        if (p[i].M <= 0 || p[i].N <= 0 || p[i].K <= 0 || p[i].K % bke != 0) return false;
+        if (p[i].N % 8 || p[i].lda % 8 || p[i].ldw % 8 || p[i].epi.ldc % 8) return false;
+        if (p[i].epi.res_t) return false;
+    }
+    const int m0 = nt_epi_mode(&p[0].epi), m1 = nt_epi_mode(&p[1].epi);
+    if (m0 != m1 || (m0 != EPI_GENERIC && m0 != EPI_PLAIN)) return false;
+    return nt_tile_rows(p[0].M, p[0].N) == nt_tile_rows(p[1].M, p[1].N);
+}
+
+int m3l_gemm_nt_pair(int dtype, const NtProblem* p_in, hipStream_t st) {
+    if (m3l_gemm_init()) return 2;
+    NtProblem p[2] = {p_in[0], p_in[1]};
+    for (int i = 0; i < 2; ++i)
+        if (p[i].epi.n_bias <= 0) p[i].epi.n_bias = p[i].N;
+    M3L_CHECK(m3l_gemm_nt_pair_ok(dtype, p), "gemm_nt_pair: the two problems do not pair (path, tile height or epilogue kind differ)");
+    const double es = dtype ? 2.0 : 4.0;
+    double bytes = 0.0, flops = 0.0;
+    int blocks[2];
+    const int mode = nt_epi_mode(&p[0].epi);
+    const bool small = nt_tile_rows(p[0].M, p[0].N) == 64;
+    for (int i = 0; i < 2; ++i) {
+        const GemmEpi* epi = &p[i].epi;
+        bytes += (double)p[i].M * p[i].K * es + (double)p[i].N * p[i].K * es +
+                 (double)p[i].M * p[i].N * ((epi->res ? 4.0 : 0.0) + (epi->out_f32 ? 4.0 : 0.0) + (epi->out_t ? es : 0.0) + (epi->out_pre ? es : 0.0) + (epi->gelu_u ? es : 0.0));
+        flops += 2.0 * p[i].M * p[i].N * p[i].K;
+        blocks[i] = 8 * cdiv(p[i].N, 64) * cdiv(cdiv(p[i].M, small ? 64 : 128), 8);
+    }
+    ProfScope prof("gemm_nt_glds64", p[0].M + p[1].M, p[0].N, p[0].K, flops, st, bytes);
+    const dim3 grid(blocks[0] + blocks[1]);
+#define NT_PAIR(T, BMv, E) gemm_nt_glds_pair_kernel<T, 64, 2, BMv, E><<<grid, 256, glds_lds_bytes(64, 2, BMv), st>>>(p[0], p[1], blocks[0])
+#define NT_PAIR_M(T, BMv) { if (mode == EPI_PLAIN) NT_PAIR(T, BMv, EPI_PLAIN); else NT_PAIR(T, BMv, EPI_GENERIC); }
+    if (dtype == 1) {
+        if (small) NT_PAIR_M(bf16, 64) else NT_PAIR_M(bf16, 128)
+    } else {
+        if (small) NT_PAIR_M(float, 64) else NT_PAIR_M(float, 128)
+    }
+#undef NT_PAIR_M
+#undef NT_PAIR
+    M3L_LAUNCH_CHECK();
+    return 0;
+}
 
 static int tn_splits(int M, int tiles) {
     int S = cdiv(512, tiles);
diff --git a/m3l_amd/csrc/kernels.h b/m3l_amd/csrc/kernels.h
--- a/m3l_amd/csrc/kernels.h
+++ b/m3l_amd/csrc/kernels.h
@@ -130,6 +130,14 @@
                    int extra_count);
 int m3l_gemm_init();
 int m3l_gemm_nt_colsum_rows(int M, int N);
+struct NtProblem {
+    const void* A;
+    const void* W;
+    int lda, ldw, M, N, K;
+    GemmEpi epi;
+};
+bool m3l_gemm_nt_pair_ok(int dtype, const NtProblem* p);
+int m3l_gemm_nt_pair(int dtype, const NtProblem* p, hipStream_t st);
 
 int m3l_attn_block_supported(int dtype, int D, int heads, int n, int project_out, int dim_head);
 int m3l_attn_block_bwd_enabled(void);
@@ -247,6 +255,88 @@
 int m3l_embed_finalize_bwd(int dtype, const float* dtok, int L, const float* E, int D, const PatchGroup* pg, const int64_t* idx,
                            int idx_ld, int j0, int cnt, int B, const float* gamma, float eps, void* dE, float* part_ws, float* dgamma,
                            float* dbeta, float* dmod, int mod0, int accumulate, hipStream_t st);
+struct PatchLnArgs {
+    PatchGroup pg;
+    const int64_t* idx;
+    const float *gamma, *beta;
+    void* xn;
+    int idx_ld, j0, cnt, rows, pdpad, vec;
+    float eps;
+};
+struct PatchLnBwdArgs {
+    PatchGroup pg;
+    const int64_t* idx;
+    const void* dxn;
+    float* part;
+    int idx_ld, j0, cnt, rows, pdpad, vec;
+    float eps;
+};
+struct EmbedFinArgs {
+    PatchGroup pg;
+    const float* E;
+    const int64_t* idx;
+    const float *gamma, *beta, *mod, *pos;
+    float* tokens;
+    int rows, D, idx_ld, j0, cnt, mod0, L;
+    float eps;
+};
+struct EmbedFinBwdArgs {
+    PatchGroup pg;
+    const float *dtok, *E;
+    const int64_t* idx;
+    const float* gamma;
+    void* dE;
+    float* part;
+    int L, rows, D, idx_ld, j0, cnt, nslot;
+    float eps;
+};
+struct MseArgs {
+    PatchGroup pg;
+    const float* pred;
+    const int64_t* idx;
+    float* part;
+    void* dpred;
+    float* target_out;
+    int pdpad, idx_ld, j0, cnt, rows, vec;
+    float w;
+};
+struct ColsumArgs {
+    const void* Y;
+    float* part;
+    int M, N, ld, rows_per_block, vec_ok;
+};
+constexpr int M3L_REDUCE_TABLE_MAX = 12;
+struct ReduceTableItem {
+    const float* part;
+    float* out;
+    int G, stride, width;
+};
+struct ReduceTable {
+    ReduceTableItem it[M3L_REDUCE_TABLE_MAX];
+    int count;
+};
+int m3l_reduce_rows_table(const ReduceTable* t, int accumulate, hipStream_t st);
+int m3l_patch_ln_vec(int dtype, const PatchGroup* pg, int pdpad, const float* gamma, const float* beta, const void* xn);
+int m3l_patch_ln_bwd_vec(int dtype, const PatchGroup* pg, int pdpad, const void* dxn);
+int m3l_mse_vec(int dtype, const PatchGroup* pg, int pdpad, const float* pred, const void* dpred, const float* target_out);
+int m3l_part_grid(long rows);
+int m3l_patch_ln_pair(int dtype, const PatchGroup* pg, const int64_t* idx, int idx_ld, const int* j0, const int* cnt, int B,
+                      const float* const* gamma, const float* const* beta, float eps, void* const* xn, const int* pdpad, hipStream_t st);
+int m3l_patch_ln_bwd_pair(int dtype, const PatchGroup* pg, const int64_t* idx, int idx_ld, const int* j0, const int* cnt, int B, float eps,
+                          const void* const* dxn, const int* pdpad, float* const* part_ws, hipStream_t st);
+int m3l_embed_finalize_pair(const float* const* E, int D, const PatchGroup* pg, const int64_t* idx, int idx_ld, const int* j0,
+                            const int* cnt, int B, const float* const* gamma, const float* const* beta, float eps, const float* mod,
+                            const int* mod0, const float* const* pos, float* tokens, int L, hipStream_t st);
+int m3l_embed_finalize_bwd_pair(int dtype, const float* dtok, int L, const float* const* E, int D, const PatchGroup* pg,
+                                const int64_t* idx, int idx_ld, const int* j0, const int* cnt, int B, const float* const* gamma,
+                                float eps, void* const* dE, float* const* part_ws, hipStream_t st);
+int m3l_mse_pair(int dtype, const float* const* pred, const int* pdpad, const PatchGroup* pg, const int64_t* idx, int idx_ld,
+                 const int* j0, const int* cnt, int B, const float* weight, float* part_ws, int* nblocks_out, void* const* dpred,
+                 float* const* target_out, hipStream_t st);
+int m3l_colsum_pair(int dtype, const void* const* Y, const int* M, const int* N, const int* ld, float* part_ws, float* const* out,
+                    int accumulate, hipStream_t st);
+int m3l_scale_by_dev_pair(int dtype, const void* const* x, const long* count, const float* scale_dev, void* const* out, hipStream_t st);
+
 int k_unshuffle_fwd(const float* src, const float* mask_token, const int64_t* unmasked, int nvis, const int64_t* masked, int nmask,
                       int B, int dd, int n_img, int n_tac, const float* dmod, const float* pos_img, const float* pos_tac, float* dec_in,
                       hipStream_t st);
diff --git a/m3l_amd/csrc/mae_plan.hip b/m3l_amd/csrc/mae_plan.hip
--- a/m3l_amd/csrc/mae_plan.hip
+++ b/m3l_amd/csrc/mae_plan.hip
@@ -121,6 +121,11 @@
 inline bool res_bf16_mode() {
     if (g_res_bf16 < 0) g_res_bf16 = getenv("M3L_RES_BF16") ? (atoi(getenv("M3L_RES_BF16")) > 0 ? 1 : 0) : 1;
     return g_res_bf16 == 1;
+}
+int g_pair_launch = -1;
+inline bool pair_launch() {
+    if (g_pair_launch < 0) g_pair_launch = getenv("M3L_PAIR_LAUNCH") ? (atoi(getenv("M3L_PAIR_LAUNCH")) > 0 ? 1 : 0) : 1;
+    return g_pair_launch == 1;
 }
 struct RbScope {
     explicit RbScope(bool on) { m3l_set_call_rb(on ? 1 : 0); }
@@ -401,6 +406,12 @@
     return old;
 }
 
+int m3l_set_pair_launch(int on) {
+    const int old = pair_launch() ? 1 : 0;
+    g_pair_launch = on ? 1 : 0;
+    return old;
+}
+
 int m3l_set_rowln(int enable) {
     const int old = use_rowln() ? 1 : 0;
     g_rowln = enable ? 1 : 0;
@@ -450,6 +461,8 @@
     EmbGroupWs g[2];
     float* scratch;
     float* scratch_side;
+    float* part_fin[2];
+    float* part_ln1[2];
     size_t scratch_b, total;
 };
 EmbWs emb_layout(const Geo& ge, int D, int dtype, int B, void* ws) {
@@ -471,6 +484,12 @@
     w.scratch_b = scratch_bytes(std::max(Mmax, 1), shapes, std::max(D * (2 + M3L_MAX_TACTILES), std::max(ge.pdp_img, ge.pdp_tac)));
     w.scratch = reinterpret_cast<float*>(a.take(w.scratch_b));
     w.scratch_side = reinterpret_cast<float*>(a.take(w.scratch_b));
+    const int pdr[2] = {ge.pd_img, ge.pd_tac}, nslot[2] = {1, std::max(ge.k, 1)};
+    for (int i = 0; i < 2; ++i) {
+        const size_t G = (size_t)m3l_part_grid(std::max(maxrows[i], 1));
+        w.part_fin[i] = a.take_n<float>(G * (2 + nslot[i]) * D);
+        w.part_ln1[i] = a.take_n<float>(G * 2 * pdr[i]);
+    }
     w.total = a.off + 256;
     return w;
 }
@@ -510,6 +529,67 @@
         }
         if (m3l_prep_weights(dtype, &pk, st)) return 1;
         if (m3l_prep_mode() == 1) return 0;
+    }
+    if (pair_launch() && B > 0 && cnt[0] > 0 && cnt[1] > 0) {
+        const int rows[2] = {B * cnt[0], B * cnt[1]};
+        const float *ln1_w[2], *ln1_b[2], *bias[2], *ln2_w[2], *ln2_b[2];
+        const float* E[2];
+        void *xn[2], *dE[2], *dxn[2];
+        for (int i = 0; i < 2; ++i) {
+            const void* const* t = tensors + 6 * i;
+            ln1_w[i] = (const float*)t[0]; ln1_b[i] = (const float*)t[1]; bias[i] = (const float*)t[3];
+            ln2_w[i] = (const float*)t[4]; ln2_b[i] = (const float*)t[5];
+            E[i] = w.g[i].E; xn[i] = w.g[i].xn; dE[i] = w.g[i].dE; dxn[i] = w.g[i].dxn;
+        }
+        NtProblem np[2];
+        bool ok = true;
+        for (int i = 0; i < 2; ++i) {
+            if (!backward) {
+                ok = ok && m3l_patch_ln_vec(dtype, &pgs[i], pdp[i], ln1_w[i], ln1_b[i], xn[i]);
+                GemmEpi e = epi0(D);
+                e.bias = bias[i];
+                e.out_f32 = w.g[i].E;
+                np[i] = NtProblem{w.g[i].xn, w.g[i].w, pdp[i], pdp[i], rows[i], D, pdp[i], e};
+            } else {
+                ok = ok && m3l_patch_ln_bwd_vec(dtype, &pgs[i], pdp[i], dxn[i]);
+                GemmEpi e = epi0(pdp[i]);
+                e.out_t = w.g[i].dxn;
+                np[i] = NtProblem{w.g[i].dE, w.g[i].wT, D, D, rows[i], pdp[i], D, e};
+            }
+        }
+        ok = ok && m3l_gemm_nt_pair_ok(dtype, np);
+        if (ok && !backward) {
+            if (m3l_patch_ln_pair(dtype, pgs, idx, L, j0, cnt, B, ln1_w, ln1_b, LN_EPS, xn, pdp, st)) return 1;
+            if (m3l_gemm_nt_pair(dtype, np, st)) return 1;
+            return m3l_embed_finalize_pair(E, D, pgs, idx, L, j0, cnt, B, ln2_w, ln2_b, LN_EPS, mod, mod0, pos, tokens, L, st);
+        }
+        if (ok) {
+            if (m3l_embed_finalize_bwd_pair(dtype, dtokens, L, E, D, pgs, idx, L, j0, cnt, B, ln2_w, LN_EPS, dE, w.part_fin, st)) return 1;
+            hipStream_t s2;
+            if (side.fork(st, &s2)) return 2;
+            float* sc = side.on ? w.scratch_side : w.scratch;
+            for (int i = 0; i < 2; ++i)
+                if (m3l_gemm_tn(dtype, w.g[i].dE, D, w.g[i].xn, pdp[i], rows[i], D, pdp[i], sc, w.scratch_b, grads[6 * i + 2], pd[i], D, pd[i], 0, s2))
+                    return 1;
+            const int DD[2] = {D, D};
+            float* db[2] = {grads[3], grads[9]};
+            if (m3l_colsum_pair(dtype, dE, rows, DD, DD, sc, db, 0, s2)) return 1;
+            if (m3l_gemm_nt_pair(dtype, np, st)) return 1;
+            if (m3l_patch_ln_bwd_pair(dtype, pgs, idx, L, j0, cnt, B, LN_EPS, dxn, pdp, w.part_ln1, st)) return 1;
+            ReduceTable rt;
+            memset(&rt, 0, sizeof(rt));
+            for (int i = 0; i < 2; ++i) {
+                const int G = m3l_part_grid(rows[i]), ns = pgs[i].nsrc, PL = (2 + ns) * D;
+                float* const* gr = grads + 6 * i;
+                rt.it[rt.count++] = ReduceTableItem{w.part_fin[i], gr[4], G, PL, D};
+                rt.it[rt.count++] = ReduceTableItem{w.part_fin[i] + D, gr[5], G, PL, D};
+                rt.it[rt.count++] = ReduceTableItem{w.part_fin[i] + 2 * D, grads[12] ? grads[12] + (long)mod0[i] * D : nullptr, G, PL, ns * D};
+                rt.it[rt.count++] = ReduceTableItem{w.part_ln1[i], gr[0], G, 2 * pd[i], pd[i]};
+                rt.it[rt.count++] = ReduceTableItem{w.part_ln1[i] + pd[i], gr[1], G, 2 * pd[i], pd[i]};
+            }
+            if (m3l_reduce_rows_table(&rt, 0, st)) return 1;
+            return side.end();
+        }
     }
     for (int i = 0; i < 2; ++i) {
         if (cnt[i] == 0) continue;
@@ -1258,7 +1338,33 @@
         if (m3l_prep_mode() == 1) return 0;
     }
     if (m3l_gather_rows2(dtype, dec_t, N, dd, masked, nmask, cnt[0], cnt[1], B, w.g[0].dg, w.g[1].dg, st)) return 1;
-    for (int i = 0; i < 2; ++i) {
+    bool pair = pair_launch() && B > 0 && cnt[0] > 0 && cnt[1] > 0;
+    if (pair) {
+        NtProblem np[2];
+        const float* pred[2];
+        void* dpred[2];
+        for (int i = 0; i < 2; ++i) {
+            GemmEpi e = epi0(pdp[i]);
+            e.bias = (const float*)tensors[2 * i + 1];
+            e.n_bias = pd[i];
+            e.out_f32 = w.g[i].pred;
+            np[i] = NtProblem{w.g[i].dg, w.g[i].w, dd, dd, B * cnt[i], pdp[i], dd, e};
+            pred[i] = w.g[i].pred; dpred[i] = w.g[i].dpred;
+            pair = pair && m3l_mse_vec(dtype, &pgs[i], pdp[i], w.g[i].pred, w.g[i].dpred, tgt[i]);
+        }
+        pair = pair && m3l_gemm_nt_pair_ok(dtype, np);
+        if (pair) {
+            if (m3l_gemm_nt_pair(dtype, np, st)) return 1;
+            if (m3l_mse_pair(dtype, pred, pdp, pgs, masked, nmask, j0, cnt, B, weight, w.loss_part, part_cnt, dpred, tgt, st)) return 1;
+            part_beg[1] = part_cnt[0];
+            nparts = part_cnt[0] + part_cnt[1];
+            for (int i = 0; i < 2; ++i)
+                if (pred_out[i])
+                    M3L_HIP(hipMemcpy2DAsync(pred_out[i], (size_t)pd[i] * 4, w.g[i].pred, (size_t)pdp[i] * 4, (size_t)pd[i] * 4, B * cnt[i],
+                                             hipMemcpyDeviceToDevice, st));
+        }
+    }
+    for (int i = 0; i < 2 && !pair; ++i) {
         if (cnt[i] == 0) continue;
         const int rows = B * cnt[i];
         GemmEpi e = epi0(pdp[i]);
@@ -1295,7 +1401,36 @@
     const int pd[2] = {ge.pd_img, ge.pd_tac}, pdp[2] = {ge.pdp_img, ge.pdp_tac};
     M3L_HIP(hipMemsetAsync(d_dec, 0, (size_t)B * N * dd * esz(dtype), st));
     SideSection side;
-    for (int i = 0; i < 2; ++i) {
+    bool pair = pair_launch() && B > 0 && cnt[0] > 0 && cnt[1] > 0;
+    if (pair) {
+        NtProblem np[2];
+        for (int i = 0; i < 2; ++i) {
+            GemmEpi e = epi0(dd);
+            e.out_t = w.g[i].ddg;
+            np[i] = NtProblem{w.g[i].dpred, w.g[i].wT, pdp[i], pdp[i], B * cnt[i], dd, pdp[i], e};
+        }
+        pair = m3l_gemm_nt_pair_ok(dtype, np);
+        if (pair) {
+            const int rows[2] = {B * cnt[0], B * cnt[1]};
+            hipStream_t s2;
+            if (side.fork(st, &s2)) return 2;
+            const void* dpred[2] = {w.g[0].dpred, w.g[1].dpred};
+            if (dloss) {
+                const long count[2] = {(long)rows[0] * pdp[0], (long)rows[1] * pdp[1]};
+                void* scaled[2] = {w.g[0].dpred_s, w.g[1].dpred_s};
+                if (m3l_scale_by_dev_pair(dtype, dpred, count, dloss, scaled, s2)) return 1;
+                dpred[0] = w.g[0].dpred_s; dpred[1] = w.g[1].dpred_s;
+            }
+            float* sc = side.on ? w.scratch_side : w.scratch;
+            for (int i = 0; i < 2; ++i)
+                if (m3l_gemm_tn(dtype, dpred[i], pdp[i], w.g[i].dg, dd, rows[i], pdp[i], dd, sc, w.scratch_b, grads[2 * i], dd, pd[i], dd, 0, s2))
+                    return 1;
+            float* db[2] = {grads[1], grads[3]};
+            if (m3l_colsum_pair(dtype, dpred, rows, pd, pdp, sc, db, 0, s2)) return 1;
+            if (m3l_gemm_nt_pair(dtype, np, st)) return 1;
+        }
+    }
+    for (int i = 0; i < 2 && !pair; ++i) {
         if (cnt[i] == 0) continue;
         const int rows = B * cnt[i];
         hipStream_t s2;
```

Result: faster. 72560 samples/s (median of 4 runs) (+1.0%).
